# haoningwu3639/StoryGen

Measured on AMD Instinct MI355X. Metric: UNet denoising steps/sec @512x512, 3 prior-frame ctx, bs=1, higher is better.
Workload: dtype f16; 1 GPU; BASELINE configs[1]: StoryGen denoising loop, 512x512 (64x64x4 latent), R=3 prior frames, CFG batch 3, DDIM, SD-1.5 UNet + attn3 (909M params, synthetic fp16 weights); stage=multi-image-condition, samples_per_gpu=1, parallelism=dp1 (one sample per GPU, final all-gather), hipgraph=True, dedup_identical_reference_samples=True, overlap_ref_pass_of_next_step=True, ref_ahead=1, warmup_run=5, split_graphs=False, stream_priority=False, ref_pass_on_cus=0, ref_pass_eager=False, paired_gemm_launches=True, paired_text_image_attention=False, groupnorm_stats_from_epilogues=True, fp16_block_stream=False

## Files before the change

storygen_amd/csrc/gemm_conv.hip:

```cpp
#include "common.h"
#include <stdlib.h>
#include <type_traits>
#include <vector>

namespace {

constexpr int BK = 64;
constexpr int MAX_AUTO_SPLIT = 16;

struct FastDiv { unsigned mul, sh1, sh2; };

__host__ __device__ __forceinline__ unsigned fd_div(unsigned n, FastDiv f) {
#if defined(__HIP_DEVICE_COMPILE__)
    const unsigned t = __umulhi(n, f.mul);
#else
    const unsigned t = (unsigned)(((unsigned long long)n * f.mul) >> 32);
#endif
    return (t + ((n - t) >> f.sh1)) >> f.sh2;
}

FastDiv make_fastdiv(unsigned d) {
    if (d <= 1) return FastDiv{0u, 0u, 0u};
    unsigned l = 0;
    while ((1ull << l) < d) ++l;
    const unsigned long long m = (((1ull << l) - d) << 32) / d + 1;
    return FastDiv{(unsigned)m, 1u, l - 1};
}

struct MmaParams {
    const f16* A; long lda;
    const f16* W; long ldw;
    void* C; long ldc;
    f16* C2; long ldc2;
    int M, N, K, KT;
    int H, Wd, Ho, Wo, cpt , stride, ups, padded;
    int mode, flags;
    const f16* bias;
    const float* rowbias; long rowbias_ld; int rows_per_batch;
    const void* res1; long ldr1;
    const void* res2; long ldr2;
    float* ws; int splits; int kt_per_split; int tiles_m, tiles_n;
    int defer;
    float* stats; int stats_batch_rows;
    const float* ln_stats; int ln_parts; const float* ln_c; const float* ln_d; int ln_mode; float ln_eps;
    float* ln_out;
    unsigned* ln_guard;
    unsigned long long* prof;
    int group_m;
    FastDiv fd_splits, fd_group_w , fd_group_m, fd_hw, fd_wo, fd_rpb, fd_cpt;
};

__device__ __forceinline__ int lds_off(int row, int chunk) { return row * 128 + ((chunk ^ ((row >> 1) & 7)) << 4); }

__host__ __device__ __forceinline__ void tile_of_id(unsigned lid, int tiles_m, int tiles_n, int gm, FastDiv fd_w, FastDiv fd_gm,
                                                    unsigned& tm, unsigned& tn) {
    const unsigned width = (unsigned)gm * (unsigned)tiles_n;
    const unsigned group = fd_div(lid, fd_w), r = lid - group * width;
    const unsigned first = group * (unsigned)gm;
    const unsigned gsize = min((unsigned)tiles_m - first, (unsigned)gm);
    const unsigned q = gsize == (unsigned)gm ? fd_div(r, fd_gm) : r / gsize;
    tn = q;
    tm = first + (r - q * gsize);
}

__device__ __forceinline__ void decode_block(const MmaParams& p, int BM, int BN, int& m0, int& n0, int& z) {
    const unsigned lid2 = (unsigned)xcd_remap(blockIdx.x, p.tiles_m * p.tiles_n * p.splits);
    const unsigned lid = fd_div(lid2, p.fd_splits);
    z = (int)(lid2 - lid * p.splits);
    unsigned tm, tn;
    tile_of_id(lid, p.tiles_m, p.tiles_n, p.group_m, p.fd_group_w, p.fd_group_m, tm, tn);
    m0 = (int)tm * BM;
    n0 = (int)tn * BN;
}

constexpr int EPI_PITCH = 68;
constexpr int EPI_XTR = 64 * EPI_PITCH;
constexpr int EPI_WAVE_BYTES = 64 * EPI_PITCH * 4 + 1024;
constexpr int EPIQ_GROUP_BYTES = 64 * EPI_PITCH * 4 + 4 * 1024;

constexpr int LN_MAX_PARTS = 20;
typedef unsigned u32x2 __attribute__((ext_vector_type(2)));

__device__ __forceinline__ void st_stream(float* p, const f32x4& v) { *reinterpret_cast<f32x4*>(p) = v; }
__device__ __forceinline__ void st_stream(f16* p, const uint2& v) {
    const u32x2 w = {v.x, v.y};
    *reinterpret_cast<u32x2*>(p) = w;
}
__device__ __forceinline__ f32x4 ld_stream(const float* p) { return *reinterpret_cast<const f32x4*>(p); }

__device__ __forceinline__ bool epi_prefetches(const MmaParams& p) {
    return p.res1 != nullptr && (p.flags & SG_F_RES1_F32) && p.splits == 1 && p.mode == SG_EPI_LINEAR;
}

template <int NQ, int NPRE>
__device__ __forceinline__ void epi_prefetch(const MmaParams& p, int rowq, int cq, f32x4 (&pre)[NQ], u32x2& pbias) {
    static_assert(NPRE <= NQ, "prefetched row quads");
    if (p.splits > 1 || p.mode != SG_EPI_LINEAR) return;
    if (p.bias) pbias = *reinterpret_cast<const u32x2*>(p.bias + cq);
    if (NPRE == 0 || !epi_prefetches(p)) return;
    const float* r = reinterpret_cast<const float*>(p.res1) + cq;
    const int mlast = p.M - 1;
#pragma unroll
    for (int k = 0; k < NPRE; ++k) pre[k] = ld_stream(r + (long)min(rowq + 4 * k, mlast) * p.ldr1);
}

template <int NW, int WTM>
constexpr int epi_npre() { return WTM == 1 ? 4 : WTM == 4 ? 0 : NW >= 8 ? 8 : 16; }
template <int NW, int WTM>
constexpr int epi_kb() { return WTM == 1 ? 4 : (WTM == 4 || NW >= 8) ? 8 : 16; }

__device__ __forceinline__ float2 ln_token_coeffs(const MmaParams& p, int token) {
    const int pairs = (p.ln_parts + 1) >> 1;
    const f32x4* s = reinterpret_cast<const f32x4*>(p.ln_stats) + (long)token * pairs;
    f32x4 t[LN_MAX_PARTS / 2];
#pragma unroll
    for (int q = 0; q < LN_MAX_PARTS / 2; ++q) t[q] = s[min(q, pairs - 1)];
    float tot = 0.f;
#pragma unroll
    for (int q = 0; q < LN_MAX_PARTS; ++q) tot += q < p.ln_parts ? ((q & 1) ? t[q >> 1].z : t[q >> 1].x) : 0.f;
    const float n = 64.f * (float)p.ln_parts, mean = tot / n;
    float m2 = 0.f;
#pragma unroll
    for (int q = 0; q < LN_MAX_PARTS; ++q) {
        const float sq = (q & 1) ? t[q >> 1].z : t[q >> 1].x, mq = (q & 1) ? t[q >> 1].w : t[q >> 1].y;
        const float dm = sq * (1.f / 64.f) - mean;
        m2 += q < p.ln_parts ? fmaf(64.f * dm, dm, mq) : 0.f;
    }
    const float r = rsqrtf(m2 / n + p.ln_eps);
    if (p.ln_guard && fabsf(mean * r) > SG_LN_GUARD_RATIO) atomicOr(p.ln_guard, SG_LN_GUARD_OFFSET);
    return make_float2(mean * r, r);
}

union H4 { uint2 u; f16 h[4]; };


__device__ __forceinline__ void store_out4(const MmaParams& p, int gm, int gn, const float (&v)[4]) {
    const bool f32 = p.flags & SG_F_OUT_F32;
    if (f32) st_stream(reinterpret_cast<float*>(p.C) + (long)gm * p.ldc + gn, f32x4{v[0], v[1], v[2], v[3]});
    if (!f32 || p.C2) {
        H4 o;
#pragma unroll
        for (int e = 0; e < 4; ++e) o.h[e] = (f16)(f32 ? __builtin_amdgcn_fmed3f(v[e], -65504.f, 65504.f) : v[e]);
        if (!f32) st_stream(reinterpret_cast<f16*>(p.C) + (long)gm * p.ldc + gn, o.u);
        if (p.C2) st_stream(p.C2 + (long)gm * p.ldc2 + gn, o.u);
    }
}

__device__ __forceinline__ void epi_park_stats(float* xtr, int lr, int lc, float (&cs)[4], float (&cq2)[4]) {
#pragma unroll
    for (int e = 0; e < 4; ++e) {
        cs[e] += __shfl_xor(cs[e], 16, 64); cq2[e] += __shfl_xor(cq2[e], 16, 64);
        cs[e] += __shfl_xor(cs[e], 32, 64); cq2[e] += __shfl_xor(cq2[e], 32, 64);
    }
    if (lr == 0) {
#pragma unroll
        for (int e = 0; e < 4; ++e) {
            xtr[128 + (4 * lc + e) * 2 + 0] = cs[e];
            xtr[128 + (4 * lc + e) * 2 + 1] = cq2[e];
        }
    }
}

__device__ __forceinline__ void ln_out_store(const MmaParams& p, int gm, int blk, float sum, float m2) {
    const int nblk = ((p.N >> 6) + 1) & ~1;
    *reinterpret_cast<float2*>(p.ln_out + ((size_t)gm * nblk + blk) * 2) = make_float2(sum, m2);
    if (p.ln_guard && !(fabsf(sum * (1.f / 64.f)) + sqrtf(m2) < 65504.f)) atomicOr(p.ln_guard, SG_LN_GUARD_RANGE);
}

template <int WGM, int WGN, int WT = 2, int WTM = WT>
__device__ __forceinline__ void epi_finish(const MmaParams& p, char* smem, f32x16 (&acc)[WTM][WT], f32x4 (&pre)[WT == 2 ? 16 : 4], u32x2& pbias,
                                           int m0, int n0, int z, int wave, int wm0, int wn, int lane) {
    constexpr int BN = 32 * WT * WGN, NW = WGM * WGN, NT = 64 * NW, NH = WT == 2 ? WTM / 2 : 1, NQ = WT == 2 ? 16 : 4;
    const int lnm = p.ln_mode;
    const int l31 = lane & 31, hi = lane >> 5, lr = lane >> 4, lc = lane & 15;
    constexpr int GQ = WGN / 2;
    const int gmq = wm0 >> 1, gq = wn >> 1, wi = wm0 & 1, wj = wn & 1, q = wi * 2 + wj;
    char* grp = smem + (gmq * GQ + gq) * EPIQ_GROUP_BYTES;
    const int rbase = m0 + gmq * 64 + q * 16, cbase = n0 + gq * 64;
    float* stg = reinterpret_cast<float*>(WT == 2 ? smem + wave * EPI_WAVE_BYTES : grp);
    float* xtr = WT == 2 ? stg + EPI_XTR : reinterpret_cast<float*>(grp + 64 * EPI_PITCH * 4 + q * 1024);
    const int r0 = WT == 2 ? lr : q * 16 + lr;
    asm volatile("s_waitcnt lgkmcnt(0)" ::: "memory");
    __builtin_amdgcn_s_barrier();
    float cs[4] = {0, 0, 0, 0}, cq2[4] = {0, 0, 0, 0};
    const bool want_stats = p.stats != nullptr;
#pragma unroll
    for (int half = 0; half < NH; ++half) {
    const int wm = wm0 * NH + half;
    int rowq, colq;
    if constexpr (WT == 2) {
#pragma unroll
        for (int i = 0; i < 2; ++i)
#pragma unroll
            for (int j = 0; j < 2; ++j)
#pragma unroll
                for (int g = 0; g < 4; ++g)
                    *reinterpret_cast<float4*>(stg + (i * 32 + l31) * EPI_PITCH + j * 32 + 8 * g + 4 * hi) =
                        make_float4(acc[2 * half + i][j][4 * g], acc[2 * half + i][j][4 * g + 1], acc[2 * half + i][j][4 * g + 2],
                                    acc[2 * half + i][j][4 * g + 3]);
        rowq = m0 + wm * 64 + lr; colq = n0 + wn * 64 + 4 * lc;
        if (lnm) {
            *reinterpret_cast<float2*>(xtr + 2 * lane) =
                ln_token_coeffs(p, lnm == 1 ? min(m0 + wm * 64 + lane, p.M - 1) : min(n0 + wn * 64 + lane, p.N - 1));
            if (lnm == 2) {
                const int rr = min(m0 + wm * 64 + lane, p.M - 1);
                *reinterpret_cast<float2*>(xtr + 128 + 2 * lane) = make_float2(p.ln_c[rr], p.ln_d[rr]);
            }
        }
        if (p.mode == SG_EPI_GEGLU && p.splits == 1) {
            const int gr = lane >> 3, gc = (lane & 7) * 4;
            const int gv = n0 + wn * 64 + gc;
            if (gv >= p.N) continue;
            float bv[4] = {0, 0, 0, 0}, bg[4] = {0, 0, 0, 0};
            if (p.bias) {
                H4 a, b;
                a.u = *reinterpret_cast<const uint2*>(p.bias + gv); b.u = *reinterpret_cast<const uint2*>(p.bias + gv + 32);
#pragma unroll
                for (int e = 0; e < 4; ++e) { bv[e] = (float)a.h[e]; bg[e] = (float)b.h[e]; }
            }
            const int go = (gv >> 6) * 32 + (gv & 31);
            float cv[4] = {0, 0, 0, 0}, cg[4] = {0, 0, 0, 0};
            if (lnm == 1) {
                const f32x4 a = *reinterpret_cast<const f32x4*>(p.ln_c + gv), b = *reinterpret_cast<const f32x4*>(p.ln_c + gv + 32);
                const f32x4 c = *reinterpret_cast<const f32x4*>(p.ln_d + gv), d = *reinterpret_cast<const f32x4*>(p.ln_d + gv + 32);
                cv[0] = a.x; cv[1] = a.y; cv[2] = a.z; cv[3] = a.w; cg[0] = b.x; cg[1] = b.y; cg[2] = b.z; cg[3] = b.w;
                bv[0] += c.x; bv[1] += c.y; bv[2] += c.z; bv[3] += c.w; bg[0] += d.x; bg[1] += d.y; bg[2] += d.z; bg[3] += d.w;
            }
#pragma unroll
            for (int k = 0; k < 8; ++k) {
                const int row = 8 * k + gr, gm = m0 + wm * 64 + row;
                const float4 a = *reinterpret_cast<const float4*>(stg + row * EPI_PITCH + gc);
                const float4 b = *reinterpret_cast<const float4*>(stg + row * EPI_PITCH + 32 + gc);
                float2 mr = make_float2(0.f, 1.f);
                if (lnm == 1) mr = *reinterpret_cast<const float2*>(xtr + 2 * row);
                if (gm >= p.M) continue;
                const float va[4] = {a.x, a.y, a.z, a.w}, ga[4] = {b.x, b.y, b.z, b.w};
                float o[4];
#pragma unroll
                for (int e = 0; e < 4; ++e)
                    o[e] = (fmaf(mr.y, va[e], bv[e]) - mr.x * cv[e]) * gelu_erf_f(fmaf(mr.y, ga[e], bg[e]) - mr.x * cg[e]);
                store_out4(p, gm, go, o);
            }
            continue;
        }
    } else {
#pragma unroll
        for (int g = 0; g < 4; ++g)
            *reinterpret_cast<float4*>(stg + (wi * 32 + l31) * EPI_PITCH + wj * 32 + 8 * g + 4 * hi) =
                make_float4(acc[0][0][4 * g], acc[0][0][4 * g + 1], acc[0][0][4 * g + 2], acc[0][0][4 * g + 3]);
        if (lnm == 1) {
            const float2 c = ln_token_coeffs(p, min(rbase + lc, p.M - 1));
            if (lr == 0) *reinterpret_cast<float2*>(xtr + 2 * lc) = c;
        } else if (lnm == 2) {
            *reinterpret_cast<float2*>(xtr + 2 * lane) = ln_token_coeffs(p, min(cbase + lane, p.N - 1));
            const int rr = min(rbase + lc, p.M - 1);
            if (lr == 0) *reinterpret_cast<float2*>(xtr + 128 + 2 * lc) = make_float2(p.ln_c[rr], p.ln_d[rr]);
        }
        asm volatile("s_waitcnt lgkmcnt(0)" ::: "memory");
        __builtin_amdgcn_s_barrier();
        rowq = rbase + lr; colq = cbase + 4 * lc;
    }
    const bool col_ok = colq < p.N;
    if (p.splits > 1) {
        float* wsz = p.ws + (size_t)z * p.M * p.N + colq;
#pragma unroll
        for (int k = 0; k < NQ; ++k) {
            const int row = 4 * k + r0, gm = rowq + 4 * k;
            const float4 v = *reinterpret_cast<const float4*>(stg + row * EPI_PITCH + 4 * lc);
            if (gm < p.M && col_ok) st_stream(wsz + (size_t)gm * p.N, f32x4{v.x, v.y, v.z, v.w});
        }
        continue;
    }
    const bool r1f32 = p.flags & SG_F_RES1_F32, r2f32 = p.flags & SG_F_RES2_F32;
    const bool res2_same = p.res2 != nullptr && p.res2 == p.res1 && p.ldr2 == p.ldr1 && r1f32 == r2f32;
    const int cq = min(colq, p.N - 4), mlast = p.M - 1;
    float v[NQ][4];
    {
        float bias4[4] = {0, 0, 0, 0};
        if (p.bias) {
            H4 b; b.u = make_uint2(pbias.x, pbias.y);
#pragma unroll
            for (int e = 0; e < 4; ++e) bias4[e] = (float)b.h[e];
        }
        if (lnm == 1) {
            const f32x4 lc4 = *reinterpret_cast<const f32x4*>(p.ln_c + cq), ld4 = *reinterpret_cast<const f32x4*>(p.ln_d + cq);
            const float c4[4] = {lc4.x, lc4.y, lc4.z, lc4.w};
            const float d4[4] = {ld4.x + bias4[0], ld4.y + bias4[1], ld4.z + bias4[2], ld4.w + bias4[3]};
#pragma unroll
            for (int k = 0; k < NQ; ++k) {
                const float4 a = *reinterpret_cast<const float4*>(stg + (4 * k + r0) * EPI_PITCH + 4 * lc);
                const float2 mr = *reinterpret_cast<const float2*>(xtr + 2 * (4 * k + lr));
                const float av[4] = {a.x, a.y, a.z, a.w};
#pragma unroll
                for (int e = 0; e < 4; ++e) v[k][e] = fmaf(mr.y, av[e], d4[e]) - mr.x * c4[e];
            }
        } else if (lnm == 2) {
            float mrx[4], mry[4];
#pragma unroll
            for (int e = 0; e < 4; ++e) { const float2 t = *reinterpret_cast<const float2*>(xtr + 2 * (4 * lc + e)); mrx[e] = t.x; mry[e] = t.y; }
#pragma unroll
            for (int k = 0; k < NQ; ++k) {
                const float4 a = *reinterpret_cast<const float4*>(stg + (4 * k + r0) * EPI_PITCH + 4 * lc);
                const float2 cd = *reinterpret_cast<const float2*>(xtr + 128 + 2 * (4 * k + lr));
                const float av[4] = {a.x, a.y, a.z, a.w};
#pragma unroll
                for (int e = 0; e < 4; ++e) v[k][e] = fmaf(mry[e], av[e], cd.y + bias4[e]) - mrx[e] * cd.x;
            }
        } else {
#pragma unroll
            for (int k = 0; k < NQ; ++k) {
                const float4 a = *reinterpret_cast<const float4*>(stg + (4 * k + r0) * EPI_PITCH + 4 * lc);
                v[k][0] = a.x + bias4[0]; v[k][1] = a.y + bias4[1]; v[k][2] = a.z + bias4[2]; v[k][3] = a.w + bias4[3];
            }
        }
    }
    constexpr int KB = epi_kb<NW, WTM>();
    auto add_f32 = [&](const float* base, long ld) __attribute__((always_inline)) {
#pragma unroll
        for (int kb = 0; kb < NQ; kb += KB) {
            float4 t[KB];
#pragma unroll
            for (int k = 0; k < KB; ++k) t[k] = *reinterpret_cast<const float4*>(base + (long)min(rowq + 4 * (kb + k), mlast) * ld + cq);
#pragma unroll
            for (int k = 0; k < KB; ++k) { v[kb + k][0] += t[k].x; v[kb + k][1] += t[k].y; v[kb + k][2] += t[k].z; v[kb + k][3] += t[k].w; }
        }
    };
    auto add_f16 = [&](const f16* base, long ld) __attribute__((always_inline)) {
        uint2 t[NQ];
#pragma unroll
        for (int k = 0; k < NQ; ++k) t[k] = *reinterpret_cast<const uint2*>(base + (long)min(rowq + 4 * k, mlast) * ld + cq);
#pragma unroll
        for (int k = 0; k < NQ; ++k) {
            H4 h; h.u = t[k];
#pragma unroll
            for (int e = 0; e < 4; ++e) v[k][e] += (float)h.h[e];
        }
    };
    if (p.rowbias) {
#pragma unroll
        for (int kb = 0; kb < NQ; kb += KB) {
            float4 t[KB];
#pragma unroll
            for (int k = 0; k < KB; ++k)
                t[k] = *reinterpret_cast<const float4*>(p.rowbias + (long)fd_div((unsigned)min(rowq + 4 * (kb + k), mlast), p.fd_rpb) * p.rowbias_ld + cq);
#pragma unroll
            for (int k = 0; k < KB; ++k) { v[kb + k][0] += t[k].x; v[kb + k][1] += t[k].y; v[kb + k][2] += t[k].z; v[kb + k][3] += t[k].w; }
        }
    }
    if (p.res1) {
        if (r1f32) {
            const float w = res2_same ? 2.f : 1.f;
            if constexpr (NH > 1) {
                const float* r = reinterpret_cast<const float*>(p.res1) + cq;
#pragma unroll
                for (int kb = 0; kb < NQ; kb += 8) {
                    f32x4 t[8];
#pragma unroll
                    for (int k = 0; k < 8; ++k) t[k] = ld_stream(r + (long)min(rowq + 4 * (kb + k), mlast) * p.ldr1);
#pragma unroll
                    for (int k = 0; k < 8; ++k) {
                        v[kb + k][0] = fmaf(w, t[k].x, v[kb + k][0]); v[kb + k][1] = fmaf(w, t[k].y, v[kb + k][1]);
                        v[kb + k][2] = fmaf(w, t[k].z, v[kb + k][2]); v[kb + k][3] = fmaf(w, t[k].w, v[kb + k][3]);
                    }
                }
            } else {
                if constexpr (epi_npre<NW, WTM>() < NQ) {
                    const float* r = reinterpret_cast<const float*>(p.res1) + cq;
#pragma unroll
                    for (int k = epi_npre<NW, WTM>(); k < NQ; ++k) pre[k] = ld_stream(r + (long)min(rowq + 4 * k, mlast) * p.ldr1);
                }
#pragma unroll
                for (int k = 0; k < NQ; ++k) {
                    v[k][0] = fmaf(w, pre[k].x, v[k][0]); v[k][1] = fmaf(w, pre[k].y, v[k][1]);
                    v[k][2] = fmaf(w, pre[k].z, v[k][2]); v[k][3] = fmaf(w, pre[k].w, v[k][3]);
                }
            }
        } else {
            add_f16(reinterpret_cast<const f16*>(p.res1), p.ldr1);
            if (res2_same) add_f16(reinterpret_cast<const f16*>(p.res1), p.ldr1);
        }
    }
    if (p.res2 && !res2_same) {
        if (r2f32) add_f32(reinterpret_cast<const float*>(p.res2), p.ldr2);
        else add_f16(reinterpret_cast<const f16*>(p.res2), p.ldr2);
    }
#pragma unroll
    for (int k = 0; k < NQ; ++k) {
        const int gm = rowq + 4 * k;
        if (gm < p.M && col_ok) {
            store_out4(p, gm, colq, v[k]);
#pragma unroll
            for (int e = 0; e < 4; ++e) { cs[e] += v[k][e]; cq2[e] = fmaf(v[k][e], v[k][e], cq2[e]); }
        }
    }
    if (p.ln_out) {
        if constexpr (WT == 2) {
#pragma unroll
            for (int k = 0; k < 16; ++k)
                *reinterpret_cast<float4*>(stg + (4 * k + lr) * EPI_PITCH + 4 * lc) = make_float4(v[k][0], v[k][1], v[k][2], v[k][3]);
            float sum = 0.f, m2 = 0.f, mean = 0.f;
            if constexpr (NH > 1) {
#pragma unroll
                for (int pass = 0; pass < 2; ++pass) {
#pragma unroll
                    for (int qb = 0; qb < 16; qb += 8) {
                        float4 rv[8];
#pragma unroll
                        for (int q = 0; q < 8; ++q) rv[q] = *reinterpret_cast<const float4*>(stg + lane * EPI_PITCH + 4 * (qb + q));
#pragma unroll
                        for (int q = 0; q < 8; ++q) {
                            if (pass == 0) {
                                sum += (rv[q].x + rv[q].y) + (rv[q].z + rv[q].w);
                            } else {
                                const float a = rv[q].x - mean, b = rv[q].y - mean, c = rv[q].z - mean, d = rv[q].w - mean;
                                m2 = fmaf(a, a, m2); m2 = fmaf(b, b, m2); m2 = fmaf(c, c, m2); m2 = fmaf(d, d, m2);
                            }
                        }
                    }
                    if (pass == 0) mean = sum * (1.f / 64.f);
                }
            } else {
                float4 rv[16];
#pragma unroll
                for (int q = 0; q < 16; ++q) rv[q] = *reinterpret_cast<const float4*>(stg + lane * EPI_PITCH + 4 * q);
#pragma unroll
                for (int q = 0; q < 16; ++q) sum += (rv[q].x + rv[q].y) + (rv[q].z + rv[q].w);
                mean = sum * (1.f / 64.f);
#pragma unroll
                for (int q = 0; q < 16; ++q) {
                    const float a = rv[q].x - mean, b = rv[q].y - mean, c = rv[q].z - mean, d = rv[q].w - mean;
                    m2 = fmaf(a, a, m2); m2 = fmaf(b, b, m2); m2 = fmaf(c, c, m2); m2 = fmaf(d, d, m2);
                }
            }
            const int gm = m0 + wm * 64 + lane;
            if (gm < p.M && n0 + wn * 64 < p.N) {
                ln_out_store(p, gm, (n0 >> 6) + wn, sum, m2);
            }
        } else {
            float s4[4], m4[4];
#pragma unroll
            for (int k = 0; k < 4; ++k) s4[k] = (v[k][0] + v[k][1]) + (v[k][2] + v[k][3]);
#pragma unroll
            for (int o = 1; o < 16; o <<= 1)
#pragma unroll
                for (int k = 0; k < 4; ++k) s4[k] += __shfl_xor(s4[k], o, 64);
#pragma unroll
            for (int k = 0; k < 4; ++k) {
                const float mean = s4[k] * (1.f / 64.f);
                const float a = v[k][0] - mean, b = v[k][1] - mean, c = v[k][2] - mean, d = v[k][3] - mean;
                m4[k] = fmaf(a, a, fmaf(b, b, fmaf(c, c, d * d)));
            }
#pragma unroll
            for (int o = 1; o < 16; o <<= 1)
#pragma unroll
                for (int k = 0; k < 4; ++k) m4[k] += __shfl_xor(m4[k], o, 64);
            if (lc == 0 && cbase < p.N) {
#pragma unroll
                for (int k = 0; k < 4; ++k)
                    if (rowq + 4 * k < p.M) ln_out_store(p, rowq + 4 * k, (n0 >> 6) + gq, s4[k], m4[k]);
            }
        }
    }
    }
    if (want_stats && (WT == 1 || p.mode == SG_EPI_LINEAR) && p.splits == 1) {
        epi_park_stats(xtr, lr, lc, cs, cq2);
        __syncthreads();
        for (int idx = threadIdx.x; idx < BN * 2; idx += NT) {
            const int plane = idx / BN, col = idx - plane * BN;
            const int gn = n0 + col;
            if (gn < p.N) {
                float s = 0.f;
                if constexpr (WT == 2) {
#pragma unroll
                    for (int w = 0; w < WGM; ++w)
                        s += reinterpret_cast<const float*>(smem + (w * WGN + (col >> 6)) * EPI_WAVE_BYTES)[EPI_XTR + 128 + (col & 63) * 2 + plane];
                } else {
#pragma unroll
                    for (int g = 0; g < WGM / 2; ++g)
#pragma unroll
                        for (int w = 0; w < 4; ++w)
                            s += reinterpret_cast<const float*>(smem + (g * GQ + (col >> 6)) * EPIQ_GROUP_BYTES + 64 * EPI_PITCH * 4 + w * 1024)[128 + (col & 63) * 2 + plane];
                }
                p.stats[((size_t)(m0 / (32 * WTM * WGM)) * 2 + plane) * p.N + gn] = s;
            }
        }
    }
}

template <int BM, int BN, bool CONV>
__global__ __launch_bounds__(256) void mma_kernel(const MmaParams p) {
    constexpr int WM = BM / 2, WN = BN / 2, TM = WM / 32, TN = WN / 32;
    static_assert(TM == 2 && TN == 2, "epi_finish works on 64x64 wave tiles");
    constexpr int A_IT = BM / 32, B_IT = BN / 32;
    constexpr int A_BYTES = BM * 128, B_BYTES = BN * 128, STAGE = A_BYTES + B_BYTES;
    constexpr int EPI_BYTES = 4 * EPI_WAVE_BYTES;
    constexpr int SMEM = (2 * STAGE > EPI_BYTES) ? 2 * STAGE : EPI_BYTES;
    __shared__ __attribute__((aligned(16))) char smem[SMEM];

    const int t = threadIdx.x, lane = t & 63, wave = t >> 6;
    const int wm = wave >> 1, wn = wave & 1, l31 = lane & 31, hi = lane >> 5;
    int m0, n0, z;
    decode_block(p, BM, BN, m0, n0, z);
    const int kt0 = z * p.kt_per_split;
    const int kt1 = min(p.KT, kt0 + p.kt_per_split);

    const int c = t & 7, r0 = t >> 3;
    const f16* a_ptr[A_IT];
    int a_oy[A_IT], a_ox[A_IT];
    bool a_ok[A_IT];
    const int pad = p.padded ? 1 : 0;
    const int wrow = p.Wd + 2 * pad;
#pragma unroll
    for (int i = 0; i < A_IT; ++i) {
        const int gm = m0 + r0 + 32 * i;
        a_ok[i] = gm < p.M;
        if constexpr (CONV) {
            const int hw = p.Ho * p.Wo;
            const int b = gm / hw, rem = gm - b * hw;
            const int oy = rem / p.Wo, ox = rem - oy * p.Wo;
            a_oy[i] = a_ok[i] ? oy * p.stride - 1 : -(1 << 20);
            a_ox[i] = ox * p.stride - 1;
            a_ptr[i] = p.A + (long)b * (p.H + 2 * pad) * wrow * p.lda + c * 8;
        } else {
            a_oy[i] = a_ox[i] = 0;
            a_ptr[i] = p.A + (long)gm * p.lda + c * 8;
        }
    }
    const f16* w_ptr[B_IT];
    bool w_ok[B_IT];
#pragma unroll
    for (int i = 0; i < B_IT; ++i) {
        const int gn = n0 + r0 + 32 * i;
        w_ok[i] = gn < p.N;
        w_ptr[i] = p.W + (long)gn * p.ldw + c * 8;
    }
    const int hin = p.H << p.ups, win = p.Wd << p.ups;

    uint4 areg[A_IT], breg[B_IT];
    auto load_regs = [&](int kt) {
        const bool kok = kt * BK + c * 8 < p.K;
        if constexpr (CONV) {
            const int tap = kt / p.cpt, cc = kt - tap * p.cpt;
            const int ky = tap / 3, kx = tap - ky * 3;
#pragma unroll
            for (int i = 0; i < A_IT; ++i) {
                const int iy = a_oy[i] + ky, ix = a_ox[i] + kx;
                const bool ok = (unsigned)iy < (unsigned)hin && (unsigned)ix < (unsigned)win;
                const long pix = (long)((iy >> p.ups) + pad) * wrow + ((ix >> p.ups) + pad);
                areg[i] = ok ? ldg16(a_ptr[i] + pix * p.lda + cc * BK) : make_uint4(0, 0, 0, 0);
            }
        } else {
#pragma unroll
            for (int i = 0; i < A_IT; ++i)
                areg[i] = (a_ok[i] && kok) ? ldg16(a_ptr[i] + kt * BK) : make_uint4(0, 0, 0, 0);
        }
#pragma unroll
        for (int i = 0; i < B_IT; ++i)
            breg[i] = (w_ok[i] && kok) ? ldg16(w_ptr[i] + kt * BK) : make_uint4(0, 0, 0, 0);
    };
    auto store_lds = [&](int buf) {
        char* sA = smem + buf * STAGE;
        char* sB = sA + A_BYTES;
#pragma unroll
        for (int i = 0; i < A_IT; ++i) *reinterpret_cast<uint4*>(sA + lds_off(r0 + 32 * i, c)) = areg[i];
#pragma unroll
        for (int i = 0; i < B_IT; ++i) *reinterpret_cast<uint4*>(sB + lds_off(r0 + 32 * i, c)) = breg[i];
    };

    f32x16 acc[TM][TN];
#pragma unroll
    for (int i = 0; i < TM; ++i)
#pragma unroll
        for (int j = 0; j < TN; ++j)
#pragma unroll
            for (int r = 0; r < 16; ++r) acc[i][j][r] = 0.f;

    if (kt0 < kt1) {
        load_regs(kt0);
        store_lds(0);
    }
    __syncthreads();
    for (int kt = kt0; kt < kt1; ++kt) {
        const int buf = (kt - kt0) & 1;
        const bool more = kt + 1 < kt1;
        if (more) load_regs(kt + 1);
        const char* sA = smem + buf * STAGE;
        const char* sB = sA + A_BYTES;
#pragma unroll
        for (int ks = 0; ks < 4; ++ks) {
            f16x8 af[TM], bf[TN];
#pragma unroll
            for (int i = 0; i < TM; ++i)
                af[i] = *reinterpret_cast<const f16x8*>(sA + lds_off(wm * WM + i * 32 + l31, ks * 2 + hi));
#pragma unroll
            for (int j = 0; j < TN; ++j)
                bf[j] = *reinterpret_cast<const f16x8*>(sB + lds_off(wn * WN + j * 32 + l31, ks * 2 + hi));
#pragma unroll
            for (int i = 0; i < TM; ++i)
#pragma unroll
                for (int j = 0; j < TN; ++j)
                    acc[i][j] = __builtin_amdgcn_mfma_f32_32x32x16_f16(bf[j], af[i], acc[i][j], 0, 0, 0);
        }
        if (more) store_lds(buf ^ 1);
        __syncthreads();
    }
    f32x4 pre_f[16]; u32x2 pre_bias;
    epi_prefetch<16, 16>(p, m0 + wm * 64 + (lane >> 4), min(n0 + wn * 64 + 4 * (lane & 15), p.N - 4), pre_f, pre_bias);
    __syncthreads();
    epi_finish<2, 2>(p, smem, acc, pre_f, pre_bias, m0, n0, z, wave, wm, wn, lane);
}

struct LdsRef { char* p; unsigned a; };
__device__ __forceinline__ LdsRef operator+(LdsRef r, int d) { return LdsRef{r.p + d, r.a + (unsigned)d}; }
__device__ __forceinline__ LdsRef lds_ref(char* smem) {
    return LdsRef{smem, (unsigned)__builtin_amdgcn_readfirstlane((int)(unsigned long)((__attribute__((address_space(3))) char*)smem))};
}
__device__ __forceinline__ void glds16(const f16* base, unsigned offb, LdsRef dst) {
    __builtin_amdgcn_global_load_lds((const __attribute__((address_space(1))) void*)(reinterpret_cast<const char*>(base) + offb),
                                     (__attribute__((address_space(3))) void*)dst.p, 16, 0, 0);
}

template <int N>
__device__ __forceinline__ void wait_vmcnt() {
    asm volatile("s_waitcnt vmcnt(%0)" ::"n"(N) : "memory");
}

template <int WGM, int WGN, int S, int WT = 2, int WTM = WT>
constexpr int pipe_smem_bytes() {
    constexpr int ring = S * (32 * WTM * WGM + 32 * WT * WGN) * 128;
    constexpr int epi = WT == 2 ? WGM * WGN * EPI_WAVE_BYTES : (WGM / 2) * (WGN / 2) * EPIQ_GROUP_BYTES;
    return ring > epi ? ring : epi;
}

template <int ST, int S, int YS, class F>
__device__ __forceinline__ void slab_seq(F& slab, int it, int nsteady) {
    if constexpr (ST < S) {
        if (it + ST < nsteady) {
            slab(it + ST, std::false_type{}, std::integral_constant<int, YS>{}, std::integral_constant<int, ST>{});
            slab_seq<ST + 1, S, YS>(slab, it, nsteady);
        }
    }
}
template <int Y, int S, class F>
__device__ __forceinline__ void slab_tail(F& slab, int nt) {
    if (nt > Y) slab(nt - 1 - Y, std::integral_constant<bool, Y == 0>{}, std::integral_constant<int, Y>{}, (nt - 1 - Y) % S);
    if constexpr (Y > 0) slab_tail<Y - 1, S>(slab, nt);
}

template <int WGM, int WGN, bool CONV, bool PROF = false, int S = 3, int WT = 2, int WTMX = WT>
__device__ __forceinline__ void mma_pipe_body(const MmaParams& p, char* smem) {
    unsigned long long pf_acc[9] = {0, 0, 0, 0, 0, 0, 0, 0, 0};
    unsigned long long pf_t = 0, pf_entry = 0;
    auto stamp = [&](int slot) __attribute__((always_inline)) {
        if constexpr (PROF) {
            const unsigned long long now = __builtin_readcyclecounter();
            pf_acc[slot] += now - pf_t;
            pf_t = now;
        }
    };
    if constexpr (PROF) pf_entry = pf_t = __builtin_readcyclecounter();
    constexpr int WTM = WTMX, WTN = WT;
    static_assert(WTM == WT || (WT == 2 && WTM == 4), "wave tiles: 32x32, 64x64 or 128x64");
    constexpr int NW = WGM * WGN, WM = 32 * WTM, WN = 32 * WTN, BM = WM * WGM, BN = WN * WGN;
    constexpr int A_IT = BM / (8 * NW), B_IT = BN / (8 * NW), LPT = A_IT + B_IT;
    constexpr int A_BYTES = BM * 128, B_BYTES = BN * 128, STAGE = A_BYTES + B_BYTES;
    constexpr int ISTR = NW * 1024;
    constexpr bool SPREAD = (NW <= 4 || WT == 1) && !PROF, STAGGER = NW == 8 && WT == 2 && !PROF;
    static_assert(S >= 2 && S <= 8, "ring depth");
    static_assert(WT == 2 || (WGM % 2 == 0 && WGN % 2 == 0), "32x32 waves come in 2x2 groups (epi_finish, WT = 1)");
    static_assert((S - 1) * LPT < 64, "vmcnt is a 6-bit counter");
    static_assert(S * STAGE <= 160 * 1024, "the ring must fit the 160 KB of LDS");
    static_assert(S * STAGE <= pipe_smem_bytes<WGM, WGN, S, WT, WTM>(), "the LDS block covers the ring and the epilogue's staging regions");

    const int t = threadIdx.x, lane = t & 63;
    const int wave = __builtin_amdgcn_readfirstlane(t >> 6);
    const int wm = wave / WGN, wn = wave % WGN, l31 = lane & 31, hi = lane >> 5;
    int m0, n0, z;
    decode_block(p, BM, BN, m0, n0, z);
    const int kt0 = z * p.kt_per_split;
    const int nt = min(p.KT, kt0 + p.kt_per_split) - kt0;

    const int srow = wave * 8 + (lane >> 3);
    const int wp = p.Wd + 2;
    unsigned w_off[B_IT];
#pragma unroll
    for (int i = 0; i < B_IT; ++i) {
        const int row = srow + 8 * NW * i;
        const int lc = (lane & 7) ^ ((row >> 1) & 7);
        w_off[i] = 2u * (unsigned)((long)min(n0 + row, p.N - 1) * p.ldw + lc * 8);
    }
    auto w_koff = [&](int kt) __attribute__((always_inline)) -> long {
        if constexpr (CONV) {
            const int cc = (kt * 7282) >> 16, tap = kt - 9 * cc;
            return (long)tap * p.cpt * BK + (long)cc * BK;
        } else {
            return (long)kt * BK;
        }
    };
    const LdsRef lds = lds_ref(smem);
    auto issue_w = [&](long koff, int stage, int sel = -1) __attribute__((always_inline)) {
        const LdsRef sB = lds + (stage * STAGE + A_BYTES + wave * 1024);
        const f16* Wt = p.W + koff;
#pragma unroll
        for (int i = 0; i < B_IT; ++i)
            if (sel < 0 || ((A_IT + i) & 3) == sel) glds16(Wt, w_off[i], sB + i * ISTR);
    };
    if (nt > 0) issue_w(w_koff(kt0), 0);

    unsigned a_off[A_IT];
    unsigned a_par[A_IT];
#pragma unroll
    for (int i = 0; i < A_IT; ++i) {
        const int row = srow + 8 * NW * i;
        const int lc = (lane & 7) ^ ((row >> 1) & 7);
        const int gm = min(m0 + row, p.M - 1);
        if constexpr (CONV) {
            const int hw = p.Ho * p.Wo;
            const int b = (int)fd_div((unsigned)gm, p.fd_hw), rem = gm - b * hw;
            const int oy = (int)fd_div((unsigned)rem, p.fd_wo), ox = rem - oy * p.Wo;
            const long img = (long)b * (p.H + 2) * wp;
            if (!p.ups) {
                a_off[i] = 2u * (unsigned)((img + (long)(oy * p.stride) * wp + ox * p.stride) * p.lda + lc * 8);
                a_par[i] = 0;
            } else {
                a_off[i] = 2u * (unsigned)((img + (long)(((oy - 1) >> 1) + 1) * wp + ((ox - 1) >> 1) + 1) * p.lda + lc * 8);
                a_par[i] = (unsigned)(((oy - 1) & 1) | (((ox - 1) & 1) << 1));
            }
        } else {
            a_off[i] = 2u * (unsigned)((long)gm * p.lda + lc * 8);
            a_par[i] = 0;
        }
    }

    struct ABase { const f16* At; int ky, kx; long wk; };
    auto a_base = [&](int kt) __attribute__((always_inline)) {
        ABase r;
        r.ky = r.kx = 0;
        r.wk = w_koff(kt);
        if constexpr (CONV) {
            const int cc = (kt * 7282) >> 16, tap = kt - 9 * cc;
            const int ky = (tap * 11) >> 5, kx = tap - ky * 3;
            r.ky = ky; r.kx = kx;
            r.At = !p.ups ? p.A + ((long)(ky * wp + kx) * p.lda + cc * BK) : p.A + cc * BK;
        } else {
            r.At = p.A + kt * BK;
        }
        return r;
    };
    auto a_emit = [&](const ABase& ab, int stage, int sel) __attribute__((always_inline)) {
        const LdsRef sA = lds + (stage * STAGE + wave * 1024);
        if constexpr (CONV) {
            if (!p.ups) {
#pragma unroll
                for (int i = 0; i < A_IT; ++i)
                    if (sel < 0 || (i & 3) == sel) glds16(ab.At, a_off[i], sA + i * ISTR);
            } else {
                const unsigned rs = (unsigned)(wp * (int)p.lda), cs = (unsigned)p.lda;
#pragma unroll
                for (int i = 0; i < A_IT; ++i) {
                    if (!(sel < 0 || (i & 3) == sel)) continue;
                    const unsigned dy = ((unsigned)ab.ky + (a_par[i] & 1u)) >> 1, dx = ((unsigned)ab.kx + (a_par[i] >> 1)) >> 1;
                    glds16(ab.At, a_off[i] + 2u * (__umul24(dy, rs) + __umul24(dx, cs)), sA + i * ISTR);
                }
            }
        } else {
#pragma unroll
            for (int i = 0; i < A_IT; ++i)
                if (sel < 0 || (i & 3) == sel) glds16(ab.At, a_off[i], sA + i * ISTR);
        }
    };
    long it_off, it_wk;
    int it_kx = 0, it_ky = 0;
    {
        const ABase b0 = a_base(kt0);
        it_off = b0.At - p.A;
        it_wk = b0.wk;
        if constexpr (CONV) { it_ky = b0.ky; it_kx = b0.kx; }
    }
    const long it_px = CONV && !p.ups ? (long)p.lda : 0;
    const long it_dy = CONV && !p.ups ? (long)(wp - 3) * p.lda : 0;
    const long it_dc = CONV ? (p.ups ? 0 : -3L * wp * p.lda) + BK : 0;
    const long it_wtap = CONV ? (long)p.cpt * BK : BK, it_wdc = CONV ? BK - 9L * p.cpt * BK : 0;
    auto a_next = [&]() __attribute__((always_inline)) {
        ABase r;
        r.At = p.A + it_off; r.ky = it_ky; r.kx = it_kx; r.wk = it_wk;
        it_wk += it_wtap;
        if constexpr (CONV) {
            it_off += it_px;
            if (++it_kx == 3) {
                it_kx = 0; it_off += it_dy;
                if (++it_ky == 3) { it_ky = 0; it_off += it_dc; it_wk += it_wdc; }
            }
        } else {
            it_off += BK;
        }
        return r;
    };
    auto issue_aw = [&](int stage, bool with_w) __attribute__((always_inline)) {
        const ABase ab = a_next();
        a_emit(ab, stage, -1);
        if (with_w) issue_w(ab.wk, stage);
    };
    if (nt > 0) issue_aw(0, false);
#pragma unroll
    for (int st = 1; st < S - 1; ++st)
        if (nt > st) issue_aw(st, true);

    f32x16 acc[WTM][WTN];
#pragma unroll
    for (int i = 0; i < WTM; ++i)
#pragma unroll
        for (int j = 0; j < WTN; ++j)
#pragma unroll
            for (int r = 0; r < 16; ++r) acc[i][j][r] = 0.f;
    constexpr int NQ = WT == 2 ? 16 : 4;
    f32x4 pre_f[NQ]; u32x2 pre_bias;
    auto prefetch = [&]() __attribute__((always_inline)) {
        const int rowq = (WT == 2 ? m0 + wm * WM : m0 + (wm >> 1) * 64 + ((wm & 1) * 2 + (wn & 1)) * 16) + (lane >> 4);
        const int colq = n0 + (WT == 2 ? wn : wn >> 1) * 64 + 4 * (lane & 15);
        epi_prefetch<NQ, epi_npre<NW, WTM>()>(p, rowq, min(colq, p.N - 4), pre_f, pre_bias);
    };

    constexpr int SPB = WT == 2 ? 1 : ((65536 - 8192) / STAGE > 0 ? (65536 - 8192) / STAGE : 1);
    constexpr int NBASE = (S + SPB - 1) / SPB;
    unsigned fa_off[NBASE][4], fb_off[NBASE][4];
#pragma unroll
    for (int st = 0; st < NBASE; ++st)
#pragma unroll
        for (int ks = 0; ks < 4; ++ks) {
            fa_off[st][ks] = (unsigned)(st * SPB * STAGE + lds_off(wm * WM + l31, ks * 2 + hi));
            fb_off[st][ks] = (unsigned)(st * SPB * STAGE + A_BYTES + lds_off(wn * WN + l31, ks * 2 + hi));
            asm volatile("" : "+v"(fa_off[st][ks]), "+v"(fb_off[st][ks]));
        }
    stamp(7);
    auto slab = [&](int it, auto last_tag, auto young_tag, auto stage_c) __attribute__((always_inline)) {
        constexpr bool LAST = decltype(last_tag)::value;
        constexpr int YOUNG = decltype(young_tag)::value;
        const int stage = stage_c;
        wait_vmcnt<YOUNG * LPT>();
        stamp(1);
        __builtin_amdgcn_s_barrier();
        stamp(2);
        const char* sA = smem + stage * STAGE;
        const char* sB = sA + A_BYTES;
        f16x8 af[2][WTM], bf[2][WTN];
        auto load_frags = [&](int buf, int ks) __attribute__((always_inline)) {
            if constexpr (std::is_same<decltype(stage_c), int>::value) {
#pragma unroll
                for (int i = 0; i < WTM; ++i)
                    af[buf][i] = *reinterpret_cast<const f16x8*>(sA + lds_off(wm * WM + i * 32 + l31, ks * 2 + hi));
#pragma unroll
                for (int j = 0; j < WTN; ++j)
                    bf[buf][j] = *reinterpret_cast<const f16x8*>(sB + lds_off(wn * WN + j * 32 + l31, ks * 2 + hi));
            } else {
                constexpr int ST = decltype(stage_c)::value;
#pragma unroll
                for (int i = 0; i < WTM; ++i)
                    af[buf][i] = *reinterpret_cast<const f16x8*>(smem + fa_off[ST / SPB][ks] + (ST % SPB) * STAGE + i * 4096);
#pragma unroll
                for (int j = 0; j < WTN; ++j)
                    bf[buf][j] = *reinterpret_cast<const f16x8*>(smem + fb_off[ST / SPB][ks] + (ST % SPB) * STAGE + j * 4096);
            }
        };
        load_frags(0, 0);
        const bool refill = SPREAD && !LAST && it + S - 1 < nt;
        int rst = stage + S - 1;
        if (rst >= S) rst -= S;
        ABase ab = {nullptr, 0, 0, 0};
        if (refill) ab = a_next();
#pragma unroll
        for (int ks = 0; ks < 4; ++ks) {
            if (ks + 1 < 4) load_frags((ks + 1) & 1, ks + 1);
            if constexpr (SPREAD) {
                if constexpr (!LAST) {
                    if (refill) {
                        a_emit(ab, rst, ks);
                        issue_w(ab.wk, rst, ks);
                    }
                } else if (ks == 1) {
                    prefetch();
                }
            } else if (LAST || !STAGGER ? ks == 1 : ks == (wave < 4 ? 1 : 3)) {
                stamp(4);
                if constexpr (LAST) {
                    prefetch();
                } else if (it + S - 1 < nt) {
                    issue_aw(rst, true);
                }
                stamp(5);
            }
#pragma unroll
            for (int i = 0; i < WTM; ++i)
#pragma unroll
                for (int j = 0; j < WTN; ++j)
                    acc[i][j] = __builtin_amdgcn_mfma_f32_32x32x16_f16(bf[ks & 1][j], af[ks & 1][i], acc[i][j], 0, 0, 0);
            if (ks == 0) stamp(3);
        }
        stamp(6);
        if constexpr (PROF) pf_acc[0] += 1;
    };
    constexpr int TAIL = S > 2 ? S - 2 : 1, YS = S - 2;
    const int nsteady = nt > TAIL ? nt - TAIL : 0;
    for (int it = 0; it < nsteady; it += S) slab_seq<0, S, YS>(slab, it, nsteady);
    slab_tail<TAIL - 1, S>(slab, nt);
    if (nt <= 0) prefetch();
    epi_finish<WGM, WGN, WT, WTM>(p, smem, acc, pre_f, pre_bias, m0, n0, z, wave, wm, wn, lane);
    if constexpr (PROF) {
        asm volatile("s_waitcnt vmcnt(0)" ::: "memory");
        stamp(8);
        if (lane == 0 && p.prof) {
            unsigned long long* dst = p.prof + ((size_t)blockIdx.x * NW + wave) * 10;
#pragma unroll
            for (int k = 0; k < 9; ++k) dst[k] = pf_acc[k];
            dst[9] = pf_t - pf_entry;
        }
    }
}

template <int WGM, int WGN, bool CONV, int S = 3>
__global__ __launch_bounds__(64 * WGM * WGN) void mma_pipe_kernel(const MmaParams p) {
    __shared__ __attribute__((aligned(16))) char smem[pipe_smem_bytes<WGM, WGN, S>()];
    mma_pipe_body<WGM, WGN, CONV, false, S>(p, smem);
}

template <int WGM, int WGN, bool CONV>
__global__ __launch_bounds__(64 * WGM * WGN) void mma_fat_kernel(const MmaParams p) {
    __shared__ __attribute__((aligned(16))) char smem[pipe_smem_bytes<WGM, WGN, 2, 2, 4>()];
    mma_pipe_body<WGM, WGN, CONV, false, 2, 2, 4>(p, smem);
}

template <int WGM, int WGN, bool CONV, int S>
__global__ __launch_bounds__(64 * WGM * WGN) void mma_lat_kernel(const MmaParams p) {
    __shared__ __attribute__((aligned(16))) char smem[pipe_smem_bytes<WGM, WGN, S, 1>()];
    mma_pipe_body<WGM, WGN, CONV, false, S, 1>(p, smem);
}

#ifdef SG_BUILD_EXPERIMENTS
template <int WGM, int WGN, bool CONV>
__global__ __launch_bounds__(64 * WGM * WGN) void mma_pipe_prof_kernel(const MmaParams p) {
    __shared__ __attribute__((aligned(16))) char smem[pipe_smem_bytes<WGM, WGN, 3>()];
    mma_pipe_body<WGM, WGN, CONV, true>(p, smem);
}
#endif

struct MmaPair { MmaParams p0, p1; };

template <int WGM, int WGN>
__global__ __launch_bounds__(64 * WGM * WGN) void mma_pipe_pair_kernel(const MmaPair pp) {
    __shared__ __attribute__((aligned(16))) char smem[pipe_smem_bytes<WGM, WGN, 3>()];
    if (blockIdx.y == 0) {
        if ((int)blockIdx.x < pp.p0.tiles_m * pp.p0.tiles_n * pp.p0.splits) mma_pipe_body<WGM, WGN, false>(pp.p0, smem);
    } else {
        if ((int)blockIdx.x < pp.p1.tiles_m * pp.p1.tiles_n * pp.p1.splits) mma_pipe_body<WGM, WGN, false>(pp.p1, smem);
    }
}

template <int S>
__global__ __launch_bounds__(256) void mma_lat_pair_kernel(const MmaPair pp) {
    __shared__ __attribute__((aligned(16))) char smem[pipe_smem_bytes<2, 2, S, 1>()];
    if (blockIdx.y == 0) {
        if ((int)blockIdx.x < pp.p0.tiles_m * pp.p0.tiles_n * pp.p0.splits) mma_pipe_body<2, 2, false, false, S, 1>(pp.p0, smem);
    } else {
        if ((int)blockIdx.x < pp.p1.tiles_m * pp.p1.tiles_n * pp.p1.splits) mma_pipe_body<2, 2, false, false, S, 1>(pp.p1, smem);
    }
}

__device__ __forceinline__ void add8(float (&v)[8], const uint4& a, const uint4& b, bool f32) {
    if (f32) {
        v[0] += __uint_as_float(a.x); v[1] += __uint_as_float(a.y); v[2] += __uint_as_float(a.z); v[3] += __uint_as_float(a.w);
        v[4] += __uint_as_float(b.x); v[5] += __uint_as_float(b.y); v[6] += __uint_as_float(b.z); v[7] += __uint_as_float(b.w);
    } else {
        H8 h; h.u = a;
#pragma unroll
        for (int e = 0; e < 8; ++e) v[e] += (float)h.h[e];
    }
}

__device__ __forceinline__ void store_out8(const MmaParams& p, int gm, int gn, const float (&v)[8]) {
    const bool f32 = p.flags & SG_F_OUT_F32;
    if (f32) {
        float* o = reinterpret_cast<float*>(p.C) + (long)gm * p.ldc + gn;
        *reinterpret_cast<float4*>(o) = make_float4(v[0], v[1], v[2], v[3]);
        *reinterpret_cast<float4*>(o + 4) = make_float4(v[4], v[5], v[6], v[7]);
    }
    if (!f32 || p.C2) {
        H8 o;
#pragma unroll
        for (int e = 0; e < 8; ++e) o.h[e] = (f16)(f32 ? __builtin_amdgcn_fmed3f(v[e], -65504.f, 65504.f) : v[e]);
        if (!f32) stg16(reinterpret_cast<f16*>(p.C) + (long)gm * p.ldc + gn, o.u);
        if (p.C2) stg16(p.C2 + (long)gm * p.ldc2 + gn, o.u);
    }
}

__device__ __forceinline__ void add_res8(const void* res, long ld, bool f32, int gm, int gn, float (&v)[8]) {
    if (f32) {
        const float* r = reinterpret_cast<const float*>(res) + (long)gm * ld + gn;
        add8(v, ldg16(r), ldg16(r + 4), true);
    } else {
        add8(v, ldg16(reinterpret_cast<const f16*>(res) + (long)gm * ld + gn), make_uint4(0, 0, 0, 0), false);
    }
}

__device__ __forceinline__ void epi_linear8(const MmaParams& p, int gm, int gn, float (&v)[8]) {
    if (p.bias) {
        H8 b; b.u = ldg16(p.bias + gn);
#pragma unroll
        for (int j = 0; j < 8; ++j) v[j] += (float)b.h[j];
    }
    if (p.rowbias) {
        const float* rb = p.rowbias + (long)fd_div((unsigned)gm, p.fd_rpb) * p.rowbias_ld + gn;
        add8(v, ldg16(rb), ldg16(rb + 4), true);
    }
    if (p.res1) add_res8(p.res1, p.ldr1, p.flags & SG_F_RES1_F32, gm, gn, v);
    if (p.res2) add_res8(p.res2, p.ldr2, p.flags & SG_F_RES2_F32, gm, gn, v);
    store_out8(p, gm, gn, v);
    if (p.ln_out) {
        float s = ((v[0] + v[1]) + (v[2] + v[3])) + ((v[4] + v[5]) + (v[6] + v[7]));
        s += __shfl_xor(s, 1, 64); s += __shfl_xor(s, 2, 64); s += __shfl_xor(s, 4, 64);
        const float mean = s * (1.f / 64.f);
        float m2 = 0.f;
#pragma unroll
        for (int j = 0; j < 8; ++j) { const float d = v[j] - mean; m2 = fmaf(d, d, m2); }
        m2 += __shfl_xor(m2, 1, 64); m2 += __shfl_xor(m2, 2, 64); m2 += __shfl_xor(m2, 4, 64);
        if ((gn & 63) == 0) ln_out_store(p, gm, gn >> 6, s, m2);
    }
}

__device__ __forceinline__ void epi_geglu8(const MmaParams& p, int gm, int gv, float (&val)[8], float (&gate)[8]) {
    if (p.bias) {
        H8 bv, bg; bv.u = ldg16(p.bias + gv); bg.u = ldg16(p.bias + gv + 32);
#pragma unroll
        for (int j = 0; j < 8; ++j) { val[j] += (float)bv.h[j]; gate[j] += (float)bg.h[j]; }
    }
    float o[8];
#pragma unroll
    for (int j = 0; j < 8; ++j) o[j] = val[j] * gelu_erf_f(gate[j]);
    store_out8(p, gm, (gv >> 6) * 32 + (gv & 31), o);
}

__global__ __launch_bounds__(256) void splitk_reduce_kernel(const MmaParams p) {
    const size_t MN = (size_t)p.M * p.N;
    if (p.mode == SG_EPI_LINEAR) {
        const int nch = p.N / 8;
        const long total = (long)p.M * nch;
        for (long idx = (long)blockIdx.x * 256 + threadIdx.x; idx < total; idx += (long)gridDim.x * 256) {
            const int gm = (int)(idx / nch), gn = (int)(idx - (long)gm * nch) * 8;
            float v[8] = {0, 0, 0, 0, 0, 0, 0, 0};
            const float* s = p.ws + (size_t)gm * p.N + gn;
            for (int z0 = 0; z0 < p.splits; z0 += 4) {
                float4 a[4], b[4];
#pragma unroll
                for (int u = 0; u < 4; ++u) {
                    a[u] = b[u] = make_float4(0.f, 0.f, 0.f, 0.f);
                    if (z0 + u < p.splits) {
                        a[u] = *reinterpret_cast<const float4*>(s + (z0 + u) * MN);
                        b[u] = *reinterpret_cast<const float4*>(s + (z0 + u) * MN + 4);
                    }
                }
#pragma unroll
                for (int u = 0; u < 4; ++u) {
                    v[0] += a[u].x; v[1] += a[u].y; v[2] += a[u].z; v[3] += a[u].w;
                    v[4] += b[u].x; v[5] += b[u].y; v[6] += b[u].z; v[7] += b[u].w;
                }
            }
            epi_linear8(p, gm, gn, v);
        }
    } else {
        const int och = p.N / 16;
        const long total = (long)p.M * och;
        for (long idx = (long)blockIdx.x * 256 + threadIdx.x; idx < total; idx += (long)gridDim.x * 256) {
            const int gm = (int)(idx / och), j = (int)(idx - (long)gm * och);
            const int gv = (j >> 2) * 64 + (j & 3) * 8;
            float val[8] = {0, 0, 0, 0, 0, 0, 0, 0}, gate[8] = {0, 0, 0, 0, 0, 0, 0, 0};
            const float* s = p.ws + (size_t)gm * p.N + gv;
            for (int z0 = 0; z0 < p.splits; z0 += 2) {
                float4 q[2][4];
#pragma unroll
                for (int u = 0; u < 2; ++u) {
#pragma unroll
                    for (int k = 0; k < 4; ++k) q[u][k] = make_float4(0.f, 0.f, 0.f, 0.f);
                    if (z0 + u < p.splits) {
                        const float* src = s + (z0 + u) * MN;
                        q[u][0] = *reinterpret_cast<const float4*>(src);
                        q[u][1] = *reinterpret_cast<const float4*>(src + 4);
                        q[u][2] = *reinterpret_cast<const float4*>(src + 32);
                        q[u][3] = *reinterpret_cast<const float4*>(src + 36);
                    }
                }
#pragma unroll
                for (int u = 0; u < 2; ++u) {
                    val[0] += q[u][0].x; val[1] += q[u][0].y; val[2] += q[u][0].z; val[3] += q[u][0].w;
                    val[4] += q[u][1].x; val[5] += q[u][1].y; val[6] += q[u][1].z; val[7] += q[u][1].w;
                    gate[0] += q[u][2].x; gate[1] += q[u][2].y; gate[2] += q[u][2].z; gate[3] += q[u][2].w;
                    gate[4] += q[u][3].x; gate[5] += q[u][3].y; gate[6] += q[u][3].z; gate[7] += q[u][3].w;
                }
            }
            epi_geglu8(p, gm, gv, val, gate);
        }
    }
}

template <int RPT>
__global__ __launch_bounds__(256) void splitk_reduce_stats_kernel(const MmaParams p) {
    constexpr int RB = RPT < 4 ? RPT : 4;
    static_assert(RPT % RB == 0, "whole steps");
    __shared__ float s_acc[32][2][64];
    const int t = threadIdx.x, vc = t & 7, tr = t >> 3;
    const int nb = p.N >> 6;
    const int mt = blockIdx.x / nb, nt = blockIdx.x - mt * nb;
    const int gn = nt * 64 + vc * 8, gm0 = mt * (32 * RPT) + tr;
    const size_t MN = (size_t)p.M * p.N;
    const size_t hstep = (size_t)32 * p.N;
    float s1[8], s2[8];
#pragma unroll
    for (int j = 0; j < 8; ++j) s1[j] = s2[j] = 0.f;
#pragma unroll 1
    for (int h0 = 0; h0 < RPT; h0 += RB) {
        float v[RB][8];
#pragma unroll
        for (int h = 0; h < RB; ++h)
#pragma unroll
            for (int j = 0; j < 8; ++j) v[h][j] = 0.f;
        const float* s = p.ws + (size_t)(gm0 + 32 * h0) * p.N + gn;
        for (int z0 = 0; z0 < p.splits; z0 += 2) {
            float4 a[2][RB], b[2][RB];
#pragma unroll
            for (int u = 0; u < 2; ++u)
#pragma unroll
                for (int h = 0; h < RB; ++h) {
                    a[u][h] = b[u][h] = make_float4(0.f, 0.f, 0.f, 0.f);
                    if (z0 + u < p.splits) {
                        const float* src = s + (z0 + u) * MN + h * hstep;
                        a[u][h] = *reinterpret_cast<const float4*>(src);
                        b[u][h] = *reinterpret_cast<const float4*>(src + 4);
                    }
                }
#pragma unroll
            for (int u = 0; u < 2; ++u)
#pragma unroll
                for (int h = 0; h < RB; ++h) {
                    v[h][0] += a[u][h].x; v[h][1] += a[u][h].y; v[h][2] += a[u][h].z; v[h][3] += a[u][h].w;
                    v[h][4] += b[u][h].x; v[h][5] += b[u][h].y; v[h][6] += b[u][h].z; v[h][7] += b[u][h].w;
                }
        }
#pragma unroll
        for (int h = 0; h < RB; ++h) {
            epi_linear8(p, gm0 + 32 * (h0 + h), gn, v[h]);
#pragma unroll
            for (int j = 0; j < 8; ++j) { s1[j] += v[h][j]; s2[j] = fmaf(v[h][j], v[h][j], s2[j]); }
        }
    }
    *reinterpret_cast<float4*>(&s_acc[tr][0][vc * 8]) = make_float4(s1[0], s1[1], s1[2], s1[3]);
    *reinterpret_cast<float4*>(&s_acc[tr][0][vc * 8 + 4]) = make_float4(s1[4], s1[5], s1[6], s1[7]);
    *reinterpret_cast<float4*>(&s_acc[tr][1][vc * 8]) = make_float4(s2[0], s2[1], s2[2], s2[3]);
    *reinterpret_cast<float4*>(&s_acc[tr][1][vc * 8 + 4]) = make_float4(s2[4], s2[5], s2[6], s2[7]);
    __syncthreads();
    if (t < 128) {
        const int plane = t >> 6, ch = t & 63;
        float acc = 0.f;
#pragma unroll 8
        for (int r = 0; r < 32; ++r) acc += s_acc[r][plane][ch];
        p.stats[((size_t)mt * 2 + plane) * p.N + nt * 64 + ch] = acc;
    }
}

int reduce_stats_rows(const MmaParams& p) {
    if (p.mode != SG_EPI_LINEAR || p.N % 64 != 0 || p.stats_batch_rows <= 0 || p.M % p.stats_batch_rows != 0) return 0;
    int best = 0;
    for (int rows = 64; rows <= 256; rows *= 2)
        if (p.stats_batch_rows % rows == 0 && (best == 0 || (long)(p.M / rows) * (p.N / 64) >= 192)) best = rows;
    return best;
}

enum { FAM_GENERIC = 0, FAM_PIPE = 1, FAM_FAT = 2, FAM_LAT = 16 };

struct TileHint { int bm = 0, bn = 0, waves = 0; };
struct PlanRequest {
    int force_split = 0;
    TileHint hint;
    void* ws = nullptr;
    size_t ws_bytes = 0;
    const char* name = "";
    bool in_pair = false;
    bool stats_optional = false;
    unsigned long long* prof = nullptr;
};

struct Plan {
    int bm = 0, bn = 0, splits = 1;
    int family = FAM_GENERIC;
    int threads = 0, grid = 0;
    int stats_rows = 0;
    bool lat() const { return family >= FAM_LAT; }
    int ring() const { return family - FAM_LAT; }
};


Plan choose_plan(int M, int N, int KT, int force_split, int max_ws_split, bool pipe, int hint_bm, int hint_bn) {
    static const int cand_pipe[6][2] = {{256, 128}, {128, 128}, {256, 64}, {128, 64}, {64, 128}, {64, 64}};
    static const int cand_gen[1][2] = {{128, 128}};
    static const int split_opts[] = {1, 2, 3, 4, 5, 6, 8, 10, 12, 16};
    const SgOptions& o = sg_options();
    const int ncand = pipe ? 6 : 1, family = pipe ? FAM_PIPE : FAM_GENERIC;
    const double CUS = 256.0, BW = pipe ? 18.5 : 12.0;
    const int forced = force_split > 0 ? (force_split > KT ? KT : force_split) : 0;
    const int gen_bm = cand_gen[0][0], gen_bn = cand_gen[0][1];
    Plan best{pipe ? 64 : gen_bm, pipe ? 64 : gen_bn, forced ? forced : 1, family};
    double best_cost = 1e300;
    for (int ci = 0; ci < ncand; ++ci) {
        const int bm = pipe ? cand_pipe[ci][0] : cand_gen[ci][0], bn = pipe ? cand_pipe[ci][1] : cand_gen[ci][1];
        if (pipe && o.tile_m && (bm != o.tile_m || bn != o.tile_n)) continue;
        if (pipe && !o.tile_m && hint_bm && (bm != hint_bm || bn != hint_bn)) continue;
        const long tiles = (long)sg_cdiv(M, bm) * sg_cdiv(N, bn);
        const double waves_per_block = pipe ? (bm / 64) * (bn / 64) : 4.0;
        const double mfma_per_slab = pipe ? 512.0 : 512.0 * (bm / 64.0) * (bn / 64.0) / 4.0;
        for (int s : split_opts) {
            if (forced) s = forced;
            else if (s > 1 && (s > max_ws_split || KT / s < 2 || o.no_split)) continue;
            if (s > KT) continue;
            const double blocks = (double)tiles * s;
            const double slabs = sg_cdiv(KT, s);
            const double blocks_per_cu = sg_cdiv((long)blocks, (long)CUS);
            const double t_bw = blocks_per_cu * slabs * (bm + bn) * 128.0 / BW;
            const double waves_per_simd = sg_cdiv((long)(blocks * waves_per_block), (long)(CUS * 4));
            const double t_mfma = waves_per_simd * slabs * mfma_per_slab;
            double cost = (t_bw > t_mfma ? t_bw : t_mfma) + 2500.0 + blocks_per_cu * (bm * bn / 16.0);
            if (s > 1) cost += 5000.0 + (double)M * N * 4.0 * (s + 1) / 1500.0;
            if (cost < best_cost) { best_cost = cost; best = Plan{bm, bn, s, family}; }
            if (forced) break;
        }
    }
    return best;
}

int check_stats(MmaParams& p, Plan& pl, const PlanRequest& rq) {
    pl.stats_rows = 0;
    if (!p.stats) return SG_OK;
    const int rows = p.splits == 1 ? pl.bm : reduce_stats_rows(p);
    const bool ok = p.mode == SG_EPI_LINEAR && rows > 0 && p.stats_batch_rows > 0 && p.stats_batch_rows % rows == 0 &&
                    p.M % p.stats_batch_rows == 0;
    if (ok) { pl.stats_rows = rows; return SG_OK; }
    if (rq.stats_optional) { p.stats = nullptr; return SG_OK; }
    return sg_set_error(SG_EINVAL, "%s: epilogue statistics need the linear epilogue, a %d-row tile that divides the %d rows of an image "
                        "and, under split-K (here %d), N %% 64 == 0: query sg_*_stats_tile_rows first", rq.name, rows, p.stats_batch_rows,
                        p.splits);
}

template <bool CONV>
bool lat_plan(const MmaParams& p, bool pipe, int force_split, int max_ws_split, TileHint hint, bool in_pair, Plan& pl) {
    const SgOptions& o = sg_options();
    if (!pipe || p.mode != SG_EPI_LINEAR || p.prof || hint.waves < 0 || o.tile_m) return false;
    if (hint.waves == 0) {
        const int kind = (in_pair || p.ln_mode == 2) ? 1 : p.ln_mode ? 2 : p.stats ? 4 : p.ln_out ? 16 : 32;
        if (!(o.lat_mask & kind)) return false;
    }
    const bool hinted = hint.bm != 0 || hint.bn != 0 || hint.waves != 0;
    const bool ask_sq = hint.bm == 64 && hint.bn == 64 && hint.waves == 4, ask_wide = hint.bm == 64 && hint.bn == 128 && hint.waves == 8;
    if (hinted && !ask_sq && !ask_wide) return false;
    const long tiles_sq = (long)sg_cdiv(p.M, 64) * sg_cdiv(p.N, 64), tiles_wide = (long)sg_cdiv(p.M, 64) * sg_cdiv(p.N, 128);
    const bool wide = ask_wide || (!hinted && o.lat_wide && p.M <= o.lat_wide_m && p.N >= 256 && p.KT >= 40);
    const bool sq = !wide && (ask_sq || (!hinted && !CONV && tiles_sq <= o.lat_tiles && p.KT >= o.lat_min_kt &&
                                         (p.KT <= o.lat_max_kt || tiles_sq <= 128)));
    if (!wide && !sq) return false;
    const long tiles = wide ? tiles_wide : tiles_sq;
    const int min_slabs = wide ? 8 : 16;
    int sp = 1;
    if (force_split > 0) sp = force_split > p.KT ? p.KT : force_split;
    else if (tiles <= 128 && !o.no_split && (o.lat_mask & 8)) {
        sp = (int)(256 / tiles);
        if (sp > p.KT / min_slabs) sp = p.KT / min_slabs;
        if (sp > max_ws_split) sp = max_ws_split;
        if (sp > MAX_AUTO_SPLIT) sp = MAX_AUTO_SPLIT;
        if (sp < 1) sp = 1;
    }
    pl = Plan{64, wide ? 128 : 64, sp, FAM_LAT + (wide ? 6 : (o.lat_stages == 8 ? 8 : 4))};
    return true;
}

TileHint apply_big_m(TileHint hint, int M, bool pipe) {
    const SgOptions& o = sg_options();
    if (o.big_m > 0 && M >= o.big_m && hint.bm == 0 && hint.bn == 0 && hint.waves == 0 && pipe) { hint.bm = o.big_bm; hint.bn = o.big_bn; }
    return hint;
}

bool asks_fat(TileHint h) { return h.waves == 8 && ((h.bm == 512 && h.bn == 128) || (h.bm == 256 && h.bn == 256)); }
bool asks_lat(TileHint h) { return (h.waves == 4 && h.bm == 64 && h.bn == 64) || (h.waves == 8 && h.bm == 64 && h.bn == 128); }

template <bool CONV>
Plan choose_family(const MmaParams& p, const PlanRequest& rq, TileHint hint, bool pipe, int max_ws_split) {
    const SgOptions& o = sg_options();
    const bool fat_ok = pipe && !p.prof && !o.tile_m && rq.force_split <= 1 && (p.mode == SG_EPI_LINEAR || p.mode == SG_EPI_GEGLU);
    if (asks_fat(hint)) {
        if (fat_ok) return Plan{hint.bm, hint.bn, 1, FAM_FAT};
        hint = TileHint{};
    }
    else if (CONV && fat_ok && o.fat_m > 0 && p.M >= o.fat_m && hint.bm == 0 && hint.bn == 0 && hint.waves == 0) {
        const int rows = p.stats ? p.stats_batch_rows : 512;
        if (rows % 512 == 0) return Plan{512, 128, 1, FAM_FAT};
    }
    Plan pl;
    if (lat_plan<CONV>(p, pipe, rq.force_split, max_ws_split, hint, rq.in_pair, pl)) return pl;
    if (asks_lat(hint)) hint.bm = hint.bn = 0;
    return choose_plan(p.M, p.N, p.KT, rq.force_split, max_ws_split, pipe, hint.bm, hint.bn);
}

template <bool CONV>
int choose_group_m(const MmaParams& p, int splits) {
    const double a_bytes = CONV ? 2.0 * p.M * (p.K / 9) * (p.stride == 1 && !p.ups ? 1.0 : (p.ups ? 0.25 : 4.0)) : 2.0 * p.M * p.K;
    const double w_bytes = 2.0 * p.N * p.K;
    const double a_panel = a_bytes / p.tiles_m, w_panel = w_bytes / p.tiles_n;
    const int wave_tiles = splits >= 32 ? 1 : 32 / splits;
    int best = 1;
    double best_bytes = 1e300;
    const int cands[6] = {1, 2, 4, 8, 16, p.tiles_m};
    for (int c : cands) {
        const int gm = c < p.tiles_m ? c : p.tiles_m;
        const int width = gm * p.tiles_n;
        int rows, cols;
        if (width >= wave_tiles) {
            rows = gm < wave_tiles ? gm : wave_tiles;
            cols = (wave_tiles + rows - 1) / rows;
        } else {
            rows = gm * ((wave_tiles + width - 1) / width);
            if (rows > p.tiles_m) rows = p.tiles_m;
            cols = p.tiles_n;
        }
        const double bytes = rows * a_panel + cols * w_panel;
        if (bytes <= best_bytes) { best_bytes = bytes; best = gm; }
    }
    return sg_options().no_nmajor ? 1 : best;
}

template <bool CONV>
void fill_fastdiv(MmaParams& p) {
    p.fd_splits = make_fastdiv((unsigned)p.splits);
    p.fd_group_w = make_fastdiv((unsigned)(p.group_m * p.tiles_n));
    p.fd_group_m = make_fastdiv((unsigned)p.group_m);
    p.fd_rpb = make_fastdiv((unsigned)(p.rows_per_batch > 0 ? p.rows_per_batch : 1));
    if (CONV) {
        p.fd_hw = make_fastdiv((unsigned)(p.Ho * p.Wo));
        p.fd_wo = make_fastdiv((unsigned)p.Wo);
        p.fd_cpt = make_fastdiv((unsigned)p.cpt);
    }
}

int threads_of(const Plan& pl) {
    return pl.family == FAM_FAT ? 512 : pl.lat() ? 64 * (pl.bm / 32) * (pl.bn / 32) : pl.family == FAM_PIPE ? 64 * (pl.bm / 64) * (pl.bn / 64) : 256;
}

template <bool CONV>
int plan_mma(MmaParams& p, const PlanRequest& rq, Plan& pl) {
    p.KT = sg_cdiv(p.K, BK);
    p.prof = rq.prof;
    const bool pipe = (p.K % BK == 0) && (!CONV || p.padded) && !sg_options().no_pipe;
    const size_t per_split = (size_t)p.M * p.N * 4;
    const int max_ws_split = rq.ws ? (int)(rq.ws_bytes / per_split > 64 ? 64 : rq.ws_bytes / per_split) : 1;
    pl = choose_family<CONV>(p, rq, apply_big_m(rq.hint, p.M, pipe), pipe, max_ws_split);
    if (pl.splits > 1 && (rq.ws == nullptr || rq.ws_bytes < per_split * pl.splits))
        return sg_set_error(SG_EINVAL, "%s: split_k=%d needs %zu workspace bytes, got %zu", rq.name, pl.splits, per_split * pl.splits,
                            rq.ws_bytes);
    p.ws = reinterpret_cast<float*>(rq.ws);
    p.splits = pl.splits;
    p.kt_per_split = sg_cdiv(p.KT, pl.splits);
    p.tiles_m = sg_cdiv(p.M, pl.bm);
    p.tiles_n = sg_cdiv(p.N, pl.bn);
    p.group_m = choose_group_m<CONV>(p, pl.splits);
    fill_fastdiv<CONV>(p);
    pl.threads = threads_of(pl);
    pl.grid = p.tiles_m * p.tiles_n * pl.splits;
    return check_stats(p, pl, rq);
}

template <int WGM, int WGN, bool CONV>
void launch_pipe(const MmaParams& p, dim3 grid, dim3 block, hipStream_t st) {
#ifdef SG_BUILD_EXPERIMENTS
    if (p.prof) {
        hipLaunchKernelGGL((mma_pipe_prof_kernel<WGM, WGN, CONV>), grid, block, 0, st, p);
        return;
    }
#endif
    if constexpr ((WGM == 2 && WGN == 2) || (WGM == 4 && WGN == 1)) {
        if (sg_options().pipe_stages == 2) {
            hipLaunchKernelGGL((mma_pipe_kernel<WGM, WGN, CONV, 2>), grid, block, 0, st, p);
            return;
        }
    }
    hipLaunchKernelGGL((mma_pipe_kernel<WGM, WGN, CONV>), grid, block, 0, st, p);
}

int launch_reduce(const MmaParams& p, hipStream_t st) {
    if (p.splits <= 1) return SG_OK;
    if (p.stats) {
        const int rows = reduce_stats_rows(p);
        const dim3 grid((p.M / rows) * (p.N / 64));
        if (rows == 256) hipLaunchKernelGGL(splitk_reduce_stats_kernel<8>, grid, dim3(256), 0, st, p);
        else if (rows == 128) hipLaunchKernelGGL(splitk_reduce_stats_kernel<4>, grid, dim3(256), 0, st, p);
        else hipLaunchKernelGGL(splitk_reduce_stats_kernel<2>, grid, dim3(256), 0, st, p);
        SG_CHECK_LAUNCH("splitk_reduce_stats");
        return SG_OK;
    }
    const long items = (long)p.M * (p.N / (p.mode == SG_EPI_GEGLU ? 16 : 8));
    const int blocks = (int)min((long)4096, (items + 255) / 256);
    hipLaunchKernelGGL(splitk_reduce_kernel, dim3(blocks), dim3(256), 0, st, p);
    SG_CHECK_LAUNCH("splitk_reduce");
    return SG_OK;
}

template <bool CONV>
int launch_plan(const MmaParams& p, const Plan& pl, hipStream_t st, const char* name) {
    if (p.defer && pl.splits <= 1)
        return sg_set_error(SG_EINVAL, "%s: defer_reduce needs a split-K launch (query sg_conv3x3_planned_splits first)", name);
    const dim3 grid(pl.grid), block(pl.threads);
    if (pl.family == FAM_FAT) {
        if (pl.bm == 512) hipLaunchKernelGGL((mma_fat_kernel<4, 2, CONV>), grid, block, 0, st, p);
        else hipLaunchKernelGGL((mma_fat_kernel<2, 4, CONV>), grid, block, 0, st, p);
    } else if (pl.lat()) {
        if (pl.bn == 128) hipLaunchKernelGGL((mma_lat_kernel<2, 4, CONV, 6>), grid, block, 0, st, p);
        else if (pl.ring() == 8) hipLaunchKernelGGL((mma_lat_kernel<2, 2, CONV, 8>), grid, block, 0, st, p);
        else hipLaunchKernelGGL((mma_lat_kernel<2, 2, CONV, 4>), grid, block, 0, st, p);
    } else if (pl.family == FAM_PIPE) {
        if (pl.bm == 256 && pl.bn == 128) launch_pipe<4, 2, CONV>(p, grid, block, st);
        else if (pl.bm == 128 && pl.bn == 128) launch_pipe<2, 2, CONV>(p, grid, block, st);
        else if (pl.bm == 256 && pl.bn == 64) launch_pipe<4, 1, CONV>(p, grid, block, st);
        else if (pl.bm == 128 && pl.bn == 64) launch_pipe<2, 1, CONV>(p, grid, block, st);
        else if (pl.bm == 64 && pl.bn == 128) launch_pipe<1, 2, CONV>(p, grid, block, st);
        else launch_pipe<1, 1, CONV>(p, grid, block, st);
    } else {
        if (p.ln_mode) return sg_set_error(SG_EINVAL, "%s: a folded LayerNorm needs the LDS-DMA kernel (K %% 64 == 0)", name);
        if (pl.bm == 128 && pl.bn == 128) hipLaunchKernelGGL((mma_kernel<128, 128, CONV>), grid, block, 0, st, p);
        else return sg_set_error(SG_EINVAL, "%s: internal: the register-staged kernel has only the 128x128 tile", name);
    }
    SG_CHECK_LAUNCH(name);
    if (p.defer) return SG_OK;
    return launch_reduce(p, st);
}

void report_plan(const Plan& pl, int32_t* out) {
    out[0] = pl.bm; out[1] = pl.bn; out[2] = pl.splits; out[3] = pl.grid; out[4] = pl.threads; out[5] = pl.family;
}

int check_out_res(const char* who, int flags, const void* C, int64_t ldc, const void* C2, int64_t ldc2, const void* res1,
                  int64_t ldr1, const void* res2, int64_t ldr2, int n_out) {
    SG_REQUIRE((flags & ~(SG_F_OUT_F32 | SG_F_RES1_F32 | SG_F_RES2_F32)) == 0, "%s: unknown flag bits 0x%x", who, flags);
    SG_REQUIRE(sg_aligned16(C) && ldc % 8 == 0 && ldc >= n_out, "%s: output alignment / ld", who);
    SG_REQUIRE(!C2 || (sg_aligned16(C2) && ldc2 % 8 == 0 && ldc2 >= n_out), "%s: second output alignment / ld", who);
    SG_REQUIRE(!res1 || (sg_aligned16(res1) && ldr1 % 8 == 0), "%s: res1 alignment", who);
    SG_REQUIRE(!res2 || (sg_aligned16(res2) && ldr2 % 8 == 0), "%s: res2 alignment", who);
    return SG_OK;
}

int check_tile_hint(const char* who, int bm, int bn, int waves) {
    if ((bm == 64 && bn == 64 && waves == 4) || (bm == 64 && bn == 128 && waves == 8)) return SG_OK;
    if (bm == 0 && bn == 0 && waves == -1) return SG_OK;
    if (waves == 8 && ((bm == 512 && bn == 128) || (bm == 256 && bn == 256))) return SG_OK;
    if (waves != 0 && waves != (bm / 64) * (bn / 64))
        return sg_set_error(SG_EINVAL, "%s: tile_waves=%d is not available for tile %dx%d (64x64 per wave; 64x64 with 4 waves of 32x32)", who, waves, bm, bn);
    if (bm == 0 && bn == 0) return SG_OK;
    static const int ok[6][2] = {{256, 128}, {128, 128}, {256, 64}, {128, 64}, {64, 128}, {64, 64}};
    for (auto& t : ok)
        if (t[0] == bm && t[1] == bn) return SG_OK;
    return sg_set_error(SG_EINVAL, "%s: unsupported tile hint %dx%d", who, bm, bn);
}

}

extern "C" size_t sg_gemm_workspace_bytes(int32_t M, int32_t N, int32_t split_k) {
    const int s = split_k > 0 ? split_k : MAX_AUTO_SPLIT;
    return s > 1 ? (size_t)M * (size_t)N * 4u * (size_t)s : 0;
}

namespace {
int gemm_params(const sg_gemm_desc* d, MmaParams& p, const char* who) {
    SG_REQUIRE(d != nullptr, "%s: null descriptor", who);
    SG_REQUIRE(d->A && d->W && d->C, "%s: null A/W/C", who);
    SG_REQUIRE(d->M > 0 && d->N > 0 && d->K > 0, "%s: bad shape M=%d N=%d K=%d", who, d->M, d->N, d->K);
    SG_REQUIRE(d->K % 8 == 0 && d->N % 8 == 0, "%s: K (%d) and N (%d) must be multiples of 8", who, d->K, d->N);
    SG_REQUIRE(d->lda % 8 == 0 && d->ldw % 8 == 0, "%s: lda/ldw must be multiples of 8", who);
    SG_REQUIRE(d->lda >= d->K && d->ldw >= d->K, "%s: lda/ldw smaller than K", who);
    SG_REQUIRE(sg_aligned16(d->A) && sg_aligned16(d->W), "%s: A/W must be 16-byte aligned", who);
    SG_REQUIRE(d->epilogue == SG_EPI_LINEAR || d->epilogue == SG_EPI_GEGLU, "%s: unknown epilogue %d", who, d->epilogue);
    int n_out = d->N;
    if (d->epilogue == SG_EPI_GEGLU) {
        SG_REQUIRE(d->N % 64 == 0, "%s: GEGLU needs N %% 64 == 0 (got %d)", who, d->N);
        SG_REQUIRE(!d->rowbias && !d->res1 && !d->res2, "%s: GEGLU epilogue takes bias only", who);
        n_out = d->N / 2;
    }
    if (int rc = check_out_res(who, d->flags, d->C, d->ldc, d->C2, d->ldc2, d->res1, d->ldr1, d->res2, d->ldr2, n_out))
        return rc;
    SG_REQUIRE(!d->bias || sg_aligned16(d->bias), "%s: bias must be 16-byte aligned", who);
    SG_REQUIRE(!d->rowbias || (sg_aligned16(d->rowbias) && d->rowbias_ld % 4 == 0 && d->rows_per_batch >= 1),
               "%s: rowbias alignment / rows_per_batch", who);
    SG_REQUIRE(d->split_k >= 0 && d->split_k <= 64, "%s: split_k %d is outside the supported range [0, 64] (0 = auto, 1 = none)", who, d->split_k);
    SG_REQUIRE(!d->workspace || (sg_aligned16(d->workspace)), "%s: workspace alignment", who);
    const long long lim = 1ll << 31;
    const long long a_span = (long long)(d->M - 1) * d->lda + d->K, w_span = (long long)(d->N - 1) * d->ldw + d->K;
    SG_REQUIRE(d->lda <= lim && a_span <= lim,
               "%s: operand A spans %lld elements ((M - 1) * lda + K); the bound is 2^31 elements (4 GiB: 32-bit LDS-DMA byte offsets)", who, a_span);
    SG_REQUIRE(d->ldw <= lim && w_span <= lim,
               "%s: operand W spans %lld elements ((N - 1) * ldw + K); the bound is 2^31 elements (4 GiB: 32-bit LDS-DMA byte offsets)", who, w_span);
    p = MmaParams{};
    p.A = reinterpret_cast<const f16*>(d->A); p.lda = d->lda;
    p.W = reinterpret_cast<const f16*>(d->W); p.ldw = d->ldw;
    p.C = d->C; p.ldc = d->ldc;
    p.C2 = reinterpret_cast<f16*>(d->C2); p.ldc2 = d->ldc2;
    p.M = d->M; p.N = d->N; p.K = d->K;
    p.mode = d->epilogue; p.flags = d->flags;
    p.bias = reinterpret_cast<const f16*>(d->bias);
    p.rowbias = d->rowbias; p.rowbias_ld = d->rowbias_ld; p.rows_per_batch = d->rows_per_batch > 0 ? d->rows_per_batch : 1;
    p.res1 = d->res1; p.ldr1 = d->ldr1;
    p.res2 = d->res2; p.ldr2 = d->ldr2;
    SG_REQUIRE(!d->stats || (sg_aligned16(d->stats) && d->stats_batch_rows > 0), "%s: stats alignment / stats_batch_rows", who);
    p.stats = d->stats; p.stats_batch_rows = d->stats_batch_rows;
    SG_REQUIRE(d->ln_mode >= 0 && d->ln_mode <= 2, "%s: ln_mode must be 0, 1 or 2", who);
    if (d->ln_mode) {
        SG_REQUIRE(d->ln_stats && d->ln_c && d->ln_d, "%s: ln_mode needs ln_stats, ln_c and ln_d", who);
        SG_REQUIRE(d->ln_parts >= 1 && d->ln_parts <= LN_MAX_PARTS && d->K == 64 * d->ln_parts,
                   "%s: ln_parts (%d) must be K / 64 (K = %d) and at most %d", who, d->ln_parts, d->K, LN_MAX_PARTS);
        SG_REQUIRE(sg_aligned16(d->ln_c) && sg_aligned16(d->ln_d) && sg_aligned16(d->ln_stats), "%s: ln_c / ln_d / ln_stats alignment", who);
        SG_REQUIRE(d->split_k <= 1, "%s: a GEMM with a folded LayerNorm does not split K (its epilogue is not linear in the partials)", who);
        SG_REQUIRE(!d->stats && !d->rowbias && !d->res1 && !d->res2, "%s: ln_mode excludes stats, rowbias and residuals", who);
        SG_REQUIRE(d->ln_mode == 1 || d->epilogue == SG_EPI_LINEAR, "%s: ln_mode 2 needs the linear epilogue", who);
        SG_REQUIRE(d->ln_eps > 0.f, "%s: ln_eps must be positive", who);
    }
    if (d->ln_stats_out) {
        SG_REQUIRE(d->epilogue == SG_EPI_LINEAR && d->N % 64 == 0 && sg_aligned16(d->ln_stats_out),
                   "%s: ln_stats_out needs the linear epilogue, N %% 64 == 0 and a 16-byte aligned buffer", who);
    }
    p.ln_stats = d->ln_stats; p.ln_parts = d->ln_parts; p.ln_c = d->ln_c; p.ln_d = d->ln_d; p.ln_mode = d->ln_mode; p.ln_eps = d->ln_eps;
    p.ln_out = d->ln_stats_out;
    SG_REQUIRE(!d->ln_guard || (reinterpret_cast<uintptr_t>(d->ln_guard) & 3u) == 0, "%s: ln_guard must be 4-byte aligned", who);
    p.ln_guard = (d->ln_mode || d->ln_stats_out) ? reinterpret_cast<unsigned*>(d->ln_guard) : nullptr;
    return check_tile_hint(who, d->tile_m, d->tile_n, d->tile_waves);
}

int conv_params(const sg_conv3x3_desc* d, MmaParams& p, const char* who) {
    SG_REQUIRE(d != nullptr, "%s: null descriptor", who);
    SG_REQUIRE(d->x && d->w && d->y, "%s: null x/w/y", who);
    SG_REQUIRE(d->B > 0 && d->H > 0 && d->W > 0 && d->Cin > 0 && d->Cout > 0, "%s: bad shape", who);
    SG_REQUIRE(d->Cin % 64 == 0, "%s: Cin (%d) must be a multiple of 64", who, d->Cin);
    SG_REQUIRE(d->Cout % 8 == 0, "%s: Cout (%d) must be a multiple of 8", who, d->Cout);
    SG_REQUIRE(d->stride == 1 || d->stride == 2, "%s: stride must be 1 or 2", who);
    SG_REQUIRE(d->upsample2x == 0 || (d->upsample2x == 1 && d->stride == 1), "%s: upsample2x needs stride 1", who);
    SG_REQUIRE(d->x_padded == 0 || d->x_padded == 1, "%s: x_padded must be 0 or 1", who);
    SG_REQUIRE(d->ldx % 8 == 0 && d->ldx >= d->Cin, "%s: bad ldx", who);
    SG_REQUIRE(sg_aligned16(d->x) && sg_aligned16(d->w), "%s: x/w must be 16-byte aligned", who);
    if (int rc = check_out_res(who, d->flags, d->y, d->ldy, nullptr, 0, d->res1, d->ldr1, nullptr, 0, d->Cout)) return rc;
    SG_REQUIRE(!d->bias || sg_aligned16(d->bias), "%s: bias alignment", who);
    SG_REQUIRE(!d->rowbias || (sg_aligned16(d->rowbias) && d->rowbias_ld % 4 == 0), "%s: rowbias alignment", who);
    SG_REQUIRE(d->split_k >= 0 && d->split_k <= 64, "%s: split_k %d is outside the supported range [0, 64] (0 = auto, 1 = none)", who, d->split_k);
    SG_REQUIRE(!d->workspace || sg_aligned16(d->workspace), "%s: workspace alignment", who);
    SG_REQUIRE((int64_t)(d->W + 2) * d->ldx < (1 << 24), "%s: input row pitch must be below 2^24 elements", who);
    {
        const long long lim = 1ll << 31;
        const int bord = d->x_padded ? 2 : 0;
        const long long rows = (long long)d->B * (d->H + bord), pixels = rows <= lim ? rows * (d->W + bord) : lim + 1;
        const long long x_span = pixels <= lim ? (pixels - 1) * (long long)d->ldx + d->Cin : lim + 1;
        const long long w_span = (long long)d->Cout * 9 * d->Cin;
        SG_REQUIRE(x_span <= lim,
                   "%s: input x spans %s%lld elements ((pixels - 1) * ldx + Cin%s); the bound is 2^31 elements (4 GiB: 32-bit LDS-DMA byte offsets)",
                   who, pixels <= lim ? "" : "more than ", x_span, d->x_padded ? ", zero border included" : "");
        SG_REQUIRE(w_span <= lim,
                   "%s: weights w span %lld elements (Cout * 9 * Cin); the bound is 2^31 elements (4 GiB: 32-bit LDS-DMA byte offsets)", who, w_span);
    }
    SG_REQUIRE(9 * (d->Cin / 64) < 3000, "%s: Cin (%d) too large for the slab decode (kt / 9 by multiply-shift, kt < 3000)", who, d->Cin);
    const int hin = d->H << d->upsample2x, win = d->W << d->upsample2x;
    const int Ho = (hin + 2 - 3) / d->stride + 1, Wo = (win + 2 - 3) / d->stride + 1;
    p = MmaParams{};
    p.A = reinterpret_cast<const f16*>(d->x); p.lda = d->ldx;
    p.W = reinterpret_cast<const f16*>(d->w); p.ldw = 9L * d->Cin;
    p.C = d->y; p.ldc = d->ldy;
    p.M = d->B * Ho * Wo; p.N = d->Cout; p.K = 9 * d->Cin;
    p.H = d->H; p.Wd = d->W; p.Ho = Ho; p.Wo = Wo; p.cpt = d->Cin / 64; p.stride = d->stride; p.ups = d->upsample2x;
    p.padded = d->x_padded;
    p.mode = SG_EPI_LINEAR; p.flags = d->flags;
    p.bias = reinterpret_cast<const f16*>(d->bias);
    p.rowbias = d->rowbias; p.rowbias_ld = d->rowbias_ld; p.rows_per_batch = Ho * Wo;
    p.res1 = d->res1; p.ldr1 = d->ldr1;
    SG_REQUIRE(!d->stats || sg_aligned16(d->stats), "%s: stats alignment", who);
    p.stats = d->stats; p.stats_batch_rows = Ho * Wo;
    SG_REQUIRE(d->defer_reduce == 0 || (d->defer_reduce == 1 && !d->stats), "%s: defer_reduce is 0 or 1 and excludes stats", who);
    p.defer = d->defer_reduce;
    return check_tile_hint(who, d->tile_m, d->tile_n, d->tile_waves);
}

PlanRequest gemm_request(const sg_gemm_desc* d, const char* name) {
    return PlanRequest{d->ln_mode ? 1 : d->split_k, TileHint{d->tile_m, d->tile_n, d->tile_waves}, d->workspace, d->workspace_bytes, name};
}

int plan_gemm(const sg_gemm_desc* d, MmaParams& p, Plan& pl, bool stats_optional = false, void* prof = nullptr) {
    if (int rc = gemm_params(d, p, "sg_gemm_f16")) return rc;
    PlanRequest rq = gemm_request(d, "sg_gemm_f16");
    rq.stats_optional = stats_optional;
    rq.prof = reinterpret_cast<unsigned long long*>(prof);
    return plan_mma<false>(p, rq, pl);
}

int plan_conv(const sg_conv3x3_desc* d, MmaParams& p, Plan& pl, bool stats_optional = false, void* prof = nullptr) {
    if (int rc = conv_params(d, p, "sg_conv3x3")) return rc;
    PlanRequest rq{d->split_k, TileHint{d->tile_m, d->tile_n, d->tile_waves}, d->workspace, d->workspace_bytes, "sg_conv3x3_nhwc_f16"};
    rq.stats_optional = stats_optional;
    rq.prof = reinterpret_cast<unsigned long long*>(prof);
    return plan_mma<true>(p, rq, pl);
}

int plan_conv_undeferred(const sg_conv3x3_desc* d, Plan& pl) {
    sg_conv3x3_desc q = *d;
    q.defer_reduce = 0;
    MmaParams p;
    return plan_conv(&q, p, pl);
}

struct PairPlan {
    Plan pl0, pl1;
    bool paired = false;
    int grid = 0;
};

int plan_pair(const sg_gemm_desc* d0, const sg_gemm_desc* d1, MmaPair& pp, PairPlan& out) {
    if (int rc = gemm_params(d0, pp.p0, "sg_gemm_pair_f16[0]")) return rc;
    if (int rc = gemm_params(d1, pp.p1, "sg_gemm_pair_f16[1]")) return rc;
    SG_REQUIRE(!(d0->workspace && d1->workspace) ||
               (reinterpret_cast<char*>(d0->workspace) + d0->workspace_bytes <= reinterpret_cast<char*>(d1->workspace) ||
                reinterpret_cast<char*>(d1->workspace) + d1->workspace_bytes <= reinterpret_cast<char*>(d0->workspace)),
               "sg_gemm_pair_f16: the two problems run concurrently and need disjoint workspaces");
    PlanRequest rq0 = gemm_request(d0, "sg_gemm_pair_f16[0]"), rq1 = gemm_request(d1, "sg_gemm_pair_f16[1]");
    rq0.in_pair = rq1.in_pair = true;
    Plan &pl0 = out.pl0, &pl1 = out.pl1;
    if (int rc = plan_mma<false>(pp.p0, rq0, pl0)) return rc;
    PlanRequest on_tile0 = rq1;
    on_tile0.hint = TileHint{pl0.bm, pl0.bn, pl0.lat() ? (pl0.bn == 128 ? 8 : 4) : -1};
    if (int rc = plan_mma<false>(pp.p1, on_tile0, pl1)) return rc;
    out.paired = pl0.family != FAM_GENERIC && pl1.family != FAM_GENERIC && pl1.bm == pl0.bm && pl1.bn == pl0.bn && pl0.lat() == pl1.lat() &&
                 !(pl0.lat() && pl0.bn == 128);
    if (!out.paired) {
        out.grid = 0;
        return plan_mma<false>(pp.p1, rq1, pl1);
    }
    out.grid = (((pl0.grid > pl1.grid ? pl0.grid : pl1.grid) + 7) & ~7) * 2;
    return SG_OK;
}

template <int WGM, int WGN>
void launch_pair(const MmaPair& pp, dim3 grid, dim3 block, hipStream_t st) {
    hipLaunchKernelGGL((mma_pipe_pair_kernel<WGM, WGN>), grid, block, 0, st, pp);
}

int launch_pair_plan(const MmaPair& pp, const PairPlan& pr, hipStream_t st) {
    const Plan& pl0 = pr.pl0;
    const dim3 grid(pr.grid / 2, 2), block(pl0.threads);
    if (pl0.lat()) {
        if (pl0.ring() == 8) hipLaunchKernelGGL(mma_lat_pair_kernel<8>, grid, block, 0, st, pp);
        else hipLaunchKernelGGL(mma_lat_pair_kernel<4>, grid, block, 0, st, pp);
    }
    else if (pl0.bm == 256 && pl0.bn == 128) launch_pair<4, 2>(pp, grid, block, st);
    else if (pl0.bm == 128 && pl0.bn == 128) launch_pair<2, 2>(pp, grid, block, st);
    else if (pl0.bm == 256 && pl0.bn == 64) launch_pair<4, 1>(pp, grid, block, st);
    else if (pl0.bm == 128 && pl0.bn == 64) launch_pair<2, 1>(pp, grid, block, st);
    else if (pl0.bm == 64 && pl0.bn == 128) launch_pair<1, 2>(pp, grid, block, st);
    else launch_pair<1, 1>(pp, grid, block, st);
    SG_CHECK_LAUNCH("sg_gemm_pair_f16");
    if (int rc = launch_reduce(pp.p0, st)) return rc;
    return launch_reduce(pp.p1, st);
}
}

extern "C" int sg_gemm_f16(const sg_gemm_desc* d, sg_stream_t stream) {
    MmaParams p;
    Plan pl;
    if (int rc = plan_gemm(d, p, pl)) return rc;
    return launch_plan<false>(p, pl, (hipStream_t)stream, "sg_gemm_f16");
}

extern "C" int sg_gemm_pair_f16(const sg_gemm_desc* d0, const sg_gemm_desc* d1, sg_stream_t stream) {
    MmaPair pp;
    PairPlan pr;
    if (int rc = plan_pair(d0, d1, pp, pr)) return rc;
    hipStream_t st = (hipStream_t)stream;
    if (pr.paired) return launch_pair_plan(pp, pr, st);
    if (int rc = launch_plan<false>(pp.p0, pr.pl0, st, "sg_gemm_pair_f16[0]")) return rc;
    return launch_plan<false>(pp.p1, pr.pl1, st, "sg_gemm_pair_f16[1]");
}

extern "C" int sg_conv3x3_nhwc_f16(const sg_conv3x3_desc* d, sg_stream_t stream) {
    MmaParams p;
    Plan pl;
    if (int rc = plan_conv(d, p, pl)) return rc;
    return launch_plan<true>(p, pl, (hipStream_t)stream, "sg_conv3x3_nhwc_f16");
}

extern "C" int sg_gemm_stats_tile_rows(const sg_gemm_desc* d) {
    SG_REQUIRE(d && d->stats, "sg_gemm_stats_tile_rows: descriptor with a stats buffer required");
    MmaParams p;
    Plan pl;
    const int rc = plan_gemm(d, p, pl, true);
    return rc ? rc : pl.stats_rows;
}

extern "C" int sg_conv3x3_stats_tile_rows(const sg_conv3x3_desc* d) {
    SG_REQUIRE(d && d->stats, "sg_conv3x3_stats_tile_rows: descriptor with a stats buffer required");
    MmaParams p;
    Plan pl;
    const int rc = plan_conv(d, p, pl, true);
    return rc ? rc : pl.stats_rows;
}

extern "C" int sg_conv3x3_planned_splits(const sg_conv3x3_desc* d) {
    SG_REQUIRE(d != nullptr, "sg_conv3x3_planned_splits: null descriptor");
    Plan pl;
    const int rc = plan_conv_undeferred(d, pl);
    return rc ? rc : pl.splits;
}

extern "C" int sg_gemm_launch_plan(const sg_gemm_desc* d, int32_t* out) {
    SG_REQUIRE(d && out, "sg_gemm_launch_plan: null argument");
    MmaParams p;
    Plan pl;
    if (int rc = plan_gemm(d, p, pl)) return rc;
    report_plan(pl, out);
    return SG_OK;
}

extern "C" int sg_conv3x3_launch_plan(const sg_conv3x3_desc* d, int32_t* out) {
    SG_REQUIRE(d && out, "sg_conv3x3_launch_plan: null argument");
    Plan pl;
    if (int rc = plan_conv_undeferred(d, pl)) return rc;
    report_plan(pl, out);
    return SG_OK;
}

extern "C" int sg_gemm_pair_launch_plan(const sg_gemm_desc* d0, const sg_gemm_desc* d1, int32_t* out) {
    SG_REQUIRE(out, "sg_gemm_pair_launch_plan: null argument");
    MmaPair pp;
// ... 115 lines not shown
```

storygen_amd/engine.py:

```python
from __future__ import annotations

import math
from typing import Dict, List, NamedTuple, Optional

import torch

from . import ops
from .arch import BlockSpec, ResnetSpec, UNetArch, XfSpec, feature_shapes
from .repack import conv1x1_nk, conv3x3_krsc, conv_in_kn, ff_fused_pack, fold_layernorm, interleave_geglu

F16 = torch.float16
GN_EPILOGUE_STATS = True
FP16_BLOCK_STREAM = False
FP16_RESNET_STREAM = False
PAIR_GEMMS = True
LN_FOLD = True
ATTN_PAIR = False
SPLITK_IN_GN = True
FF_FUSED = True
FF_SPLIT_MAX_TOKENS = 16384
FF_PROJ_MERGE = True
LN_EPS = 1e-5


def _pair(first, second):
    if PAIR_GEMMS:
        ops.gemm_pair(first, second)
    else:
        for args, kw in (first, second):
            ops.gemm(*args, **{**kw, "tile": (0, 0, -1)})


class _Resnet:
    __slots__ = ("spec", "n1g", "n1b", "w1", "n2g", "n2b", "w2", "b2", "wsc", "bsc", "temb_off")


class _Xf:
    __slots__ = ("spec", "ng", "nb", "w_in", "b_in", "w_out", "b_out", "ln", "w_qk1", "w_v1", "w_o1", "b_o1", "w_q2", "w_k2",
                 "w_v2", "w_o2", "b_o2", "w_q3", "w_k3", "w_v3", "w_o3", "b_o3", "w_o23", "b_o23", "w_ff1", "b_ff1", "w_ff2", "b_ff2",
                 "w_qk1f", "c_qk1", "d_qk1", "w_v1f", "c_v1", "d_v1", "w_q2f", "c_q2", "d_q2", "w_q3f", "c_q3", "d_q3",
                 "w_ff1f", "c_ff1", "d_ff1",
                 "ff_pack",
                 "w_out2",
                 "w_ffo", "b_ffo")


class EngineWeights:

    def __init__(self, arch: UNetArch, state_dict: Dict[str, torch.Tensor], device):
        self.arch, self.dev, self.cfg = arch, torch.device(device), arch.config
        self.version = 0
        self._load_weights(state_dict)

    def _w(self, sd, key) -> torch.Tensor:
        return sd[key].detach().to(device=self.dev, dtype=F16).contiguous()

    def _load_weights(self, sd):
        dev, arch = self.dev, self.arch
        g = lambda k: self._w(sd, k)
        self.w_conv_in = conv_in_kn(g("conv_in.weight"))
        self.b_conv_in = g("conv_in.bias")
        self.w_t1, self.b_t1 = g("time_embedding.linear_1.weight"), g("time_embedding.linear_1.bias")
        self.w_t2, self.b_t2 = g("time_embedding.linear_2.weight"), g("time_embedding.linear_2.bias")
        half = cfg_half = self.cfg["block_out_channels"][0] // 2
        self.freqs = torch.exp(-math.log(10000.0) * torch.arange(half, dtype=torch.float32)
                               / (cfg_half - self.cfg["freq_shift"])).to(dev)
        self.resnets: Dict[str, _Resnet] = {}
        temb_w, temb_b, off = [], [], 0
        for r in arch.resnets:
            p = r.prefix
            o = _Resnet()
            o.spec = r
            o.n1g, o.n1b = g(f"{p}.norm1.weight"), g(f"{p}.norm1.bias")
            o.w1 = conv3x3_krsc(g(f"{p}.conv1.weight"))
            o.n2g, o.n2b = g(f"{p}.norm2.weight"), g(f"{p}.norm2.bias")
            o.w2, o.b2 = conv3x3_krsc(g(f"{p}.conv2.weight")), g(f"{p}.conv2.bias")
            if r.has_shortcut:
                o.wsc, o.bsc = conv1x1_nk(g(f"{p}.conv_shortcut.weight")), g(f"{p}.conv_shortcut.bias")
            else:
                o.wsc = o.bsc = None
            temb_w.append(g(f"{p}.time_emb_proj.weight"))
            temb_b.append((sd[f"{p}.time_emb_proj.bias"].float() + sd[f"{p}.conv1.bias"].float()).to(dev, F16))
            o.temb_off = off
            off += r.cout
            self.resnets[p] = o
        self.w_temb = torch.cat(temb_w, 0).contiguous()
        self.b_temb = torch.cat(temb_b, 0).contiguous()
        self.temb_total = off
        self.xfs: Dict[str, _Xf] = {}
        for blk in arch.blocks:
            for a in blk.attns:
                if a is None:
                    continue
                p, t = a.prefix, f"{a.prefix}.transformer_blocks.0"
                o = _Xf()
                o.spec = a
                o.ng, o.nb = g(f"{p}.norm.weight"), g(f"{p}.norm.bias")
                o.w_in, o.b_in = conv1x1_nk(g(f"{p}.proj_in.weight")), g(f"{p}.proj_in.bias")
                o.w_out, o.b_out = conv1x1_nk(g(f"{p}.proj_out.weight")), g(f"{p}.proj_out.bias")
                o.ln = {n: (g(f"{t}.{n}.weight"), g(f"{t}.{n}.bias")) for n in ("norm1", "norm2", "norm3", "norm4")}
                o.w_qk1 = torch.cat([g(f"{t}.attn1.to_q.weight"), g(f"{t}.attn1.to_k.weight")], 0).contiguous()
                o.w_v1 = g(f"{t}.attn1.to_v.weight")
                o.w_o1, o.b_o1 = g(f"{t}.attn1.to_out.0.weight"), g(f"{t}.attn1.to_out.0.bias")
                o.w_q2 = g(f"{t}.attn2.to_q.weight")
                o.w_k2, o.w_v2 = g(f"{t}.attn2.to_k.weight"), g(f"{t}.attn2.to_v.weight")
                o.w_o2, o.b_o2 = g(f"{t}.attn2.to_out.0.weight"), g(f"{t}.attn2.to_out.0.bias")
                o.w_q3 = g(f"{t}.attn3.to_q.weight")
                o.w_k3, o.w_v3 = g(f"{t}.attn3.to_k.weight"), g(f"{t}.attn3.to_v.weight")
                o.w_o3, o.b_o3 = g(f"{t}.attn3.to_out.0.weight"), g(f"{t}.attn3.to_out.0.bias")
                o.w_o23 = torch.cat([o.w_o2, o.w_o3], dim=1).contiguous()
                o.b_o23 = (sd[f"{t}.attn2.to_out.0.bias"].float() + sd[f"{t}.attn3.to_out.0.bias"].float()).to(dev, F16)
                o.w_ff1, o.b_ff1 = interleave_geglu(g(f"{t}.ff.net.0.proj.weight"), g(f"{t}.ff.net.0.proj.bias"))
                o.w_ff2, o.b_ff2 = g(f"{t}.ff.net.2.weight"), g(f"{t}.ff.net.2.bias")
                for name, val in self._pack_folds(o).items():
                    setattr(o, name, val)
                o.ff_pack = ff_fused_pack(o.w_ff1f, o.d_ff1, o.w_ff2) if (ops.ff_fused_supported(a.channels) and dev.type == "cuda") else None
                o.w_out2 = torch.cat([o.w_out, o.w_out], dim=1).contiguous() if o.ff_pack is not None else None
                if o.ff_pack is None:
                    wo32 = o.w_out.float()
                    o.w_ffo = torch.cat([(wo32 @ o.w_ff2.float()).to(F16), o.w_out], dim=1).contiguous()
                    o.b_ffo = (wo32 @ o.b_ff2.float() + o.b_out.float()).to(F16).contiguous()
                else:
                    o.w_ffo = o.b_ffo = None
                self.xfs[p] = o
        self.samplers = {}
        for blk in arch.down + arch.up:
            if blk.sampler_prefix:
                self.samplers[blk.sampler_prefix] = (conv3x3_krsc(g(f"{blk.sampler_prefix}.weight")),
                                                     g(f"{blk.sampler_prefix}.bias"))
        self.gn_out = (g("conv_norm_out.weight"), g("conv_norm_out.bias"))
        self.w_conv_out = conv3x3_krsc(g("conv_out.weight"))
        self.b_conv_out = g("conv_out.bias")

    @staticmethod
    def _pack_folds(xf: "_Xf", which=("qk1", "v1", "q2", "q3", "ff1")) -> Dict[str, torch.Tensor]:
        src = {"qk1": (xf.w_qk1, None, "norm1"), "v1": (xf.w_v1, None, "norm1"), "q2": (xf.w_q2, None, "norm2"),
               "q3": (xf.w_q3, None, "norm4"), "ff1": (xf.w_ff1, xf.b_ff1, "norm3")}
        out = {}
        for k in which:
            w, b, n = src[k]
            wf, c, d = fold_layernorm(w, b, *xf.ln[n])
            out[f"w_{k}f"], out[f"c_{k}"], out[f"d_{k}"] = wf.contiguous(), c.contiguous(), d.contiguous()
        return out

    def _pack_attn3(self, sd, xf: "_Xf") -> Dict[str, torch.Tensor]:
        t = f"{xf.spec.prefix}.transformer_blocks.0"
        g = lambda k: self._w(sd, k)
        w_o3 = g(f"{t}.attn3.to_out.0.weight")
        return {"w_q3": g(f"{t}.attn3.to_q.weight"), "w_k3": g(f"{t}.attn3.to_k.weight"), "w_v3": g(f"{t}.attn3.to_v.weight"),
                "w_o3": w_o3, "b_o3": g(f"{t}.attn3.to_out.0.bias"), "w_o23": torch.cat([xf.w_o2, w_o3], dim=1),
                "b_o23": (sd[f"{t}.attn2.to_out.0.bias"].float() + sd[f"{t}.attn3.to_out.0.bias"].float()).to(self.dev, F16)}

    def refresh_attn3_(self, sd, prefixes=None):
        for p, xf in self.xfs.items():
            if prefixes is None or p in prefixes:
                for name, val in self._pack_attn3(sd, xf).items():
                    getattr(xf, name).copy_(val)
                for name, val in self._pack_folds(xf, ("q3",)).items():
                    getattr(xf, name).copy_(val)

    def _pack_attn1(self, sd, xf: "_Xf") -> Dict[str, torch.Tensor]:
        t = f"{xf.spec.prefix}.transformer_blocks.0"
        g = lambda k: self._w(sd, k)
        return {"w_qk1": torch.cat([g(f"{t}.attn1.to_q.weight"), g(f"{t}.attn1.to_k.weight")], 0), "w_v1": g(f"{t}.attn1.to_v.weight"),
                "w_o1": g(f"{t}.attn1.to_out.0.weight"), "b_o1": g(f"{t}.attn1.to_out.0.bias")}

    def refresh_attn1_(self, sd, prefixes=None):
        for p, xf in self.xfs.items():
            if prefixes is None or p in prefixes:
                for name, val in self._pack_attn1(sd, xf).items():
                    getattr(xf, name).copy_(val)
                for name, val in self._pack_folds(xf, ("qk1", "v1")).items():
                    getattr(xf, name).copy_(val)

    def reload_(self, sd):
        fresh = EngineWeights.__new__(EngineWeights)
        fresh.arch, fresh.dev, fresh.cfg = self.arch, self.dev, self.cfg
        fresh._load_weights(sd)

        def walk(old, new):
            if torch.is_tensor(old):
                old.copy_(new)
            elif isinstance(old, dict):
                for k in old:
                    walk(old[k], new[k])
            elif isinstance(old, (tuple, list)):
                for a, b in zip(old, new):
                    walk(a, b)
            elif isinstance(old, (_Resnet, _Xf)):
                for k in old.__slots__:
                    if k != "spec" and getattr(old, k, None) is not None:
                        walk(getattr(old, k), getattr(new, k))
        for k, v in self.__dict__.items():
            if k not in ("arch", "dev", "cfg", "version"):
                walk(v, getattr(fresh, k))
        self.version += 1


class HarvestPlan:

    def __init__(self, ctx: Dict[str, torch.Tensor], ops_: List[tuple], kv: Optional[Dict[str, tuple]] = None,
                 src_offset: int = 0, short: int = 0, slots_per_row: Optional[int] = None, direct: bool = False,
                 identity: bool = False):
        self.ctx, self.ops, self.kv, self.src_offset = ctx, list(ops_), kv, int(src_offset)
        self.short, self.slots_per_row, self.direct = int(short), slots_per_row, bool(direct) or bool(identity)
        self.identity = bool(identity)
        if self.identity and (self.ops or self.src_offset):
            raise ValueError("an identity harvest plan has no copy ops and no source offset")

    def flat_slot(self, row: int, slot: int, R: int) -> int:
        return row if row < self.short else self.short + (row - self.short) * R + slot

    def is_direct(self, n_samples: int, R: int) -> bool:
        if self.identity:
            return all(c.dim() == 2 and c.shape[0] % n_samples == 0 for c in self.ctx.values())
        if not self.direct or self.src_offset:
            return False
        seen = {}
        for src, step, row, slot, cnt in self.ops:
            for j in range(cnt):
                seen[self.flat_slot(row, slot + j, R)] = src + j * step
        return seen == {u: u for u in range(n_samples)}


class _GnFeed(NamedTuple):
    pstats: Optional[list] = None
    split: Optional[dict] = None

    @staticmethod
    def concat(h: "_GnFeed", skip: "_GnFeed", channels: int) -> "_GnFeed":
        if h.pstats and skip.pstats and h.pstats[0][2] + skip.pstats[0][2] == channels:
            return _GnFeed(pstats=h.pstats + skip.pstats)
        return _NO_FEED


_NO_FEED = _GnFeed()


class _XfPass:

    def __init__(self, eng: "UNetEngine", xf: _Xf, x: torch.Tensor, x_gn: _GnFeed, out: Optional[torch.Tensor], lvl: int, consume: bool):
        L = self.L = eng.lv[lvl]
        self.xf, self.x, self.x_gn, self.out, self.lvl, self.consume, self.guard = xf, x, x_gn, out, lvl, consume, eng.ln_guard
        self.B, self.hw, self.M, self.C, self.heads = eng.B, eng.hw[lvl], x.shape[0], xf.spec.channels, xf.spec.heads
        self.scale = xf.spec.dim_head ** -0.5
        self.fold = LN_FOLD and self.C % 64 == 0 and self.C // 64 <= 20
        self.ff1 = FF_FUSED and xf.ff_pack is not None and L["h3"].dtype != F16
        self.merge = FF_PROJ_MERGE and self.fold and not self.ff1 and xf.w_ffo is not None and L["h3"].dtype != F16 and out is not None
        self.h0r, self.h1r = self.raw(L["h0"], L["ln"]), self.raw(L["h1"], L["ln4"])
        self.h3raw = L["ffo"][:self.M, 4 * self.C:5 * self.C] if self.merge else L["ln"]

    @staticmethod
    def raw(t: torch.Tensor, buf: torch.Tensor) -> torch.Tensor:
        return t if t.dtype == F16 else buf

    def prod(self, t: torch.Tensor, buf: torch.Tensor, st: torch.Tensor) -> dict:
        return dict(out2=None if t.dtype == F16 else buf, ln_out=st, guard=self.guard) if self.fold else {}

    def prod3(self, h3: torch.Tensor) -> dict:
        return {} if self.ff1 else self.prod(h3, self.h3raw, self.L["lnst3"])


class UNetEngine:
    def __init__(self, arch: UNetArch, state_dict: Optional[Dict[str, torch.Tensor]], device, batch: int, height: int,
                 width: int, n_ref: int = 0, seq_len: int = 77, splitk_workspace_mb: int = 96,
                 weights: Optional[EngineWeights] = None, ctx_rows: Optional[int] = None,
                 attn3_groups: Optional[List[tuple]] = None, fp8_attention: bool = False, ctx_short: int = 0,
                 cfg_shared_head: bool = False, fp16_stream: Optional[tuple] = None):
        self.arch, self.dev = arch, torch.device(device)
        self.B, self.H, self.W, self.R, self.S = batch, height, width, n_ref, seq_len
        cfg = arch.config
        self.cfg = cfg
        nlev = len(cfg["block_out_channels"])
        if height % (1 << (nlev - 1)) or width % (1 << (nlev - 1)):
            raise ValueError(f"latent size {height}x{width} must be divisible by {1 << (nlev - 1)}")
        self.groups, self.eps = cfg["norm_num_groups"], cfg["norm_eps"]
        self.cad = cfg["cross_attention_dim"]
        self.hw = [(height >> l) * (width >> l) for l in range(nlev)]
        self.Sp = (seq_len + 7) & ~7
        for k, lv in arch.feature_level.items():
            if self.hw[lv] % 8:
                raise ValueError(f"latent {height}x{width} leaves {self.hw[lv]} tokens at attention block {k}; the V^T layout "
# ... 261 lines not shown
        plans = () if harvest is None else (tuple(harvest) if isinstance(harvest, (list, tuple)) else (harvest,))
        self._xf_entry(st)
        self._self_projections(st, st.L["h0"], st.h0r, st.L["qk"], st.L["vt"])
        self._xf_harvest(st, plans, self._xf_self_attention(st, plans))

    def _xf_back(self, st: _XfPass, text_cache: bool, shared: bool = False) -> _GnFeed:
        h3 = self._xf_cross_consume(st, text_cache, shared) if st.consume else self._xf_cross_text(st, text_cache)
        return self._xf_feed_forward(st, h3)

    def _xf_entry(self, st: _XfPass):
        L, xf, x = st.L, st.xf, st.x
        ops.groupnorm(x.unflatten(0, (st.B, st.hw)), xf.ng, xf.nb, L["gn"].unflatten(0, (st.B, st.hw)), self.groups, 1e-6, False,
                      self.ws_gn, pstats=st.x_gn.pstats, split=st.x_gn.split)
        ops.gemm(L["gn"], xf.w_in, L["h0"], bias=xf.b_in, workspace=self.ws_split, **st.prod(L["h0"], L["ln"], L["lnst0"]))

    def _self_projections(self, st: _XfPass, h0: torch.Tensor, h0r: torch.Tensor, qk: torch.Tensor, vt: torch.Tensor):
        xf, L = st.xf, st.L
        if st.fold:
            _pair(((h0r, xf.w_qk1f, qk), dict(ln=(1, L["lnst0"], xf.c_qk1, xf.d_qk1, LN_EPS), guard=st.guard)),
                  ((xf.w_v1f, h0r, vt), dict(ln=(2, L["lnst0"], xf.c_v1, xf.d_v1, LN_EPS), guard=st.guard)))
        else:
            ops.layernorm(h0, *xf.ln["norm1"], L["ln"])
            _pair(((L["ln"], xf.w_qk1, qk), dict(workspace=self.ws_split)), ((xf.w_v1, L["ln"], vt), dict(workspace=self.ws_pair)))

    def _xf_self_attention(self, st: _XfPass, plans: tuple) -> Optional[torch.Tensor]:
        xf, L, B, hw, C = st.xf, st.L, st.B, st.hw, st.C
        qk3 = L["qk"].view(B, hw, 2 * C)
        self._attention(qk3[:, :, :C], qk3[:, :, C:], L["vt"].view(C, B, hw).permute(1, 0, 2), L["att"].view(B, hw, C), st.heads, st.scale)
        direct = None
        if len(plans) == 1 and plans[0].is_direct(B, plans[0].slots_per_row or self.R):
            c = plans[0].ctx[xf.spec.feature_key]
            direct = c if c.dim() == 2 else c.view(-1, C)
            assert direct.shape[0] == st.M, (direct.shape, st.M)
        kw1 = st.prod(L["h1"], L["ln4"], L["lnst1"])
        if direct is not None:
            kw1["out2"] = st.h1r = direct
        ops.gemm(L["att"], xf.w_o1, L["h1"], bias=xf.b_o1, res1=L["h0"], workspace=self.ws_split, **kw1)
        return direct

    def _xf_harvest(self, st: _XfPass, plans: tuple, direct: Optional[torch.Tensor]):
        xf, hw, C = st.xf, st.hw, st.C
        h1b = st.L["h1"].view(st.B, hw, C)
        for plan in plans:
            ctx = plan.ctx[xf.spec.feature_key]
            c2d = ctx if ctx.dim() == 2 else ctx.view(-1, C)
            if direct is None:
                Rp = plan.slots_per_row or (ctx.shape[1] // hw)
                for src, step, row, slot, cnt in plan.ops:
                    t0 = plan.flat_slot(row, slot, Rp) * hw
                    dst = c2d[t0:t0 + cnt * hw].view(cnt, hw, C)
                    ops.copy_rows(dst, h1b[plan.src_offset + src:].as_strided((cnt, hw, C), (step * hw * C, C, 1)))
            if plan.kv is not None:
                ki, vti = plan.kv[xf.spec.feature_key]
                _pair(((c2d, xf.w_k3, ki), dict(workspace=self.ws_split)), ((xf.w_v3, c2d, vti), dict(workspace=self.ws_pair)))

    def _xf_queries(self, st: _XfPass):
        xf, L, h1, h1r, gd, ws = st.xf, st.L, st.L["h1"], st.h1r, st.guard, self.ws_split
        if st.consume and st.fold:
            _pair(((h1r, xf.w_q2f, L["q2"]), dict(ln=(1, L["lnst1"], xf.c_q2, xf.d_q2, LN_EPS), guard=gd)),
                  ((h1r, xf.w_q3f, L["q"]), dict(ln=(1, L["lnst1"], xf.c_q3, xf.d_q3, LN_EPS), guard=gd)))
        elif st.consume:
            ops.layernorm(h1, *xf.ln["norm2"], L["ln"], 1e-5, *xf.ln["norm4"], L["ln4"])
            _pair(((L["ln"], xf.w_q2, L["q2"]), dict(workspace=ws)), ((L["ln4"], xf.w_q3, L["q"]), dict(workspace=self.ws_pair)))
        elif st.fold:
            ops.gemm(h1r, xf.w_q2f, L["q"], ln=(1, L["lnst1"], xf.c_q2, xf.d_q2, LN_EPS), guard=gd)
        else:
            ops.layernorm(h1, *xf.ln["norm2"], L["ln"])
            ops.gemm(L["ln"], xf.w_q2, L["q"], workspace=ws)

    def _ctx_kv(self, st: _XfPass):
        xf, L, hw, C = st.xf, st.L, st.hw, st.C
        if self.kv_ext is not None:
            ki, vti = self.kv_ext[xf.spec.feature_key]
        else:
            ctx = self.ctx[xf.spec.feature_key]
            c2d = ctx if ctx.dim() == 2 else ctx.view(-1, C)
            ki, vti = L["ki"], L["vti"]
            _pair(((c2d, xf.w_k3, ki), dict(workspace=self.ws_split)), ((xf.w_v3, c2d, vti), dict(workspace=self.ws_pair)))
        ns, rows, nk = self.ctx_short, self.ctx_rows, self.R * hw
        short = (ki[: ns * hw].view(ns, hw, C), vti[:, : ns * hw].unflatten(1, (ns, hw)).permute(1, 0, 2)) if ns else None
        return ki[ns * hw:].view(rows - ns, nk, C), vti[:, ns * hw:].unflatten(1, (rows - ns, nk)).permute(1, 0, 2), short

    def _xf_cross_consume(self, st: _XfPass, text_cache: bool, shared: bool) -> torch.Tensor:
        xf, L, B, hw, C, heads, scale, S = st.xf, st.L, st.B, st.hw, st.C, st.heads, st.scale, self.S
        kt3, vtt3 = self._text_kv(xf, st.lvl, text_cache)
        att23, h1, h3 = L["att23"], L["h1"], L["h3"]
        a2v, a3v = att23[:, :C].unflatten(0, (B, hw)), att23[:, C:].unflatten(0, (B, hw))
        if shared:
            q2q = L["q2"][:hw].view(1, hw, C).expand(2, hw, C)
            q3 = L["q"][:hw].view(1, hw, C).expand(2, hw, C)
            kt3, vtt3, a2o, a3o = kt3[::2], vtt3[::2], a2v[::2], a3v[:2]
        else:
            q2q, q3, a2o, a3o = L["q2"].view(B, hw, C), L["q"].view(B, hw, C), a2v, a3v
        paired = (ATTN_PAIR and self.attn3_share is not None and not self.ctx_short and not shared
                  and not (self.fp8_attention and C == heads * 40))
        forked = False if paired else self._fork()
        if forked:
            with torch.cuda.stream(self.side):
                ops.attention(q2q, kt3, vtt3, a2o, heads, scale, nk=S)
        elif not paired:
            ops.attention(q2q, kt3, vtt3, a2o, heads, scale, nk=S)
        ki3, vti3, short = self._ctx_kv(st)
        if paired:
            ops.attention_pair((q3, ki3, vti3, a3v, None), (q2q, kt3, vtt3, a2v, S), heads, scale)
        elif self.attn3_share is not None:
            self._attention(q3, ki3, vti3, a3o, heads, scale, short=short)
        else:
            for q0, n, c0 in self.attn3_groups:
                self._attention(q3[q0:q0 + n], ki3[c0:c0 + n], vti3[c0:c0 + n], a3v[q0:q0 + n], heads, scale)
        if forked:
            self._join()
        if shared:
            ops.copy_rows(a2v[1:2], a2v[0:1])
            ops.copy_rows(a3v[2:3], a3v[1:2])
        ops.gemm(att23, xf.w_o23, h3, bias=xf.b_o23, res1=h1, res2=h1, workspace=self.ws_split, **st.prod3(h3))
        return h3

    def _xf_cross_text(self, st: _XfPass, text_cache: bool) -> torch.Tensor:
        xf, L, B, hw, C = st.xf, st.L, st.B, st.hw, st.C
        kt3, vtt3 = self._text_kv(xf, st.lvl, text_cache)
        ops.attention(L["q"].view(B, hw, C), kt3, vtt3, L["att"].view(B, hw, C), st.heads, st.scale, nk=self.S)
        h3 = L["h2"]
        ops.gemm(L["att"], xf.w_o2, h3, bias=xf.b_o2, res1=L["h1"], workspace=self.ws_split, **st.prod3(h3))
        return h3

    def _xf_feed_forward(self, st: _XfPass, h3: torch.Tensor) -> _GnFeed:
        xf, L, M, C, gd, ws, x, out = st.xf, st.L, st.M, st.C, st.guard, self.ws_split, st.x, st.out
        h4, w_out = L["h4"], xf.w_out
        if st.ff1 and M <= FF_SPLIT_MAX_TOKENS:
            h4, w_out = L["att23"], xf.w_out2
            ops.ff_fused(h3, xf.ff_pack, xf.b_ff2, h4, LN_EPS, split=True)
        elif st.ff1:
            ops.ff_fused(h3, xf.ff_pack, xf.b_ff2, L["h4"], LN_EPS)
        elif st.merge:
            ops.gemm(st.h3raw, xf.w_ff1f, L["ffo"][:M, :4 * C], epilogue=ops.EPI_GEGLU, ln=(1, L["lnst3"], xf.c_ff1, xf.d_ff1, LN_EPS), guard=gd)
            h4, w_out = L["ffo"][:M], xf.w_ffo
        elif st.fold:
            ops.gemm(st.raw(h3, L["ln"]), xf.w_ff1f, L["ffi"], epilogue=ops.EPI_GEGLU, ln=(1, L["lnst3"], xf.c_ff1, xf.d_ff1, LN_EPS), guard=gd)
        else:
            ops.layernorm(h3, *xf.ln["norm3"], L["ln"])
            ops.gemm(L["ln"], xf.w_ff1, L["ffi"], bias=xf.b_ff1, epilogue=ops.EPI_GEGLU, workspace=ws)
        if not st.ff1 and not st.merge:
            ops.gemm(L["ffi"], xf.w_ff2, L["h4"], bias=xf.b_ff2, res1=h3, workspace=ws)
        kwo = dict(bias=xf.b_ffo if st.merge else xf.b_out, res1=x, workspace=ws)
        return self._produce(xf.spec.prefix + ".proj_out", st.lvl, C,
                             lambda s: ops.gemm(h4, w_out, out, stats=None if s is None else (s, st.hw), **kwo),
                             lambda buf: ops.gemm_stats_rows(h4, w_out, out, stats=(buf, st.hw), **kwo))

    def _sampler_conv(self, prefix: str, h: torch.Tensor, out: torch.Tensor, lvl: int, out_lvl: int, down: bool) -> _GnFeed:
        w, b = self.samplers[prefix]
        pbuf = self.padded[(lvl, h.shape[1])]
        ops.pad_cast(self._img(h, lvl), pbuf)
        kw = dict(stride=2 if down else 1, upsample2x=not down, bias=b, workspace=self.ws_split, x_padded=True)
        return self._produce(prefix, out_lvl, out.shape[1], lambda s: ops.conv3x3(pbuf, w, self._img(out, out_lvl), stats=s, **kw),
                             lambda buf: ops.conv3x3_stats_rows(pbuf, w, self._img(out, out_lvl), stats=buf, **kw))

    def forward(self, harvest_slot: Optional[int] = None, consume: bool = False, harvest: Optional[HarvestPlan] = None,
                harvest_only: bool = False, text_cache: bool = False,
                side: Optional[torch.cuda.Stream] = None) -> Optional[torch.Tensor]:
        if harvest_slot is not None:
            if harvest is not None or self.ctx_rows != self.B:
                raise ValueError("harvest_slot needs one context row per sample and no explicit plan")
            if not self.R:
                raise ValueError("engine was built without context buffers (n_ref=0)")
            if self.ctx_short:
                raise ValueError("harvest_slot: this engine's context rows have different slot counts (ctx_short); pass a HarvestPlan")
            harvest = HarvestPlan(self.ctx, [(b, 0, b, harvest_slot, 1) for b in range(self.B)])
        if harvest is not None and consume:
            raise ValueError("a pass either harvests features or consumes them")
        if consume and not self.R:
            raise ValueError("engine was built without context buffers (n_ref=0)")
        if harvest_only and harvest is None:
            raise ValueError("harvest_only needs a harvest plan")
        self.side = side
        arch, text, skips = self.arch, self.text_in, self.skips
        steps = list(zip(arch.schedule, arch.schedule[1:] + [None]))
        last_xf = [s.xf for s in arch.schedule if s.xf is not None][-1].prefix if harvest_only else None
        tk = dict(text_cache=text_cache)
        skip_gn: List[_GnFeed] = [_NO_FEED]
        if self.time_table is not None and self.time_table_on:
            ops.lookup_rows(self.t_in, self.time_table[0], self.time_table[1], self.tproj)
        else:
            self._time_chain(self.t_in, self.temb0, self.temb1, self.temb2, self.tproj)
        shared = self.cfg_shared_head and consume
        if shared and not self._head_checked and not torch.cuda.is_current_stream_capturing():
            self._head_checked = True
            if not (torch.equal(self.x_in[0], self.x_in[1]) and torch.equal(self.x_in[0], self.x_in[2])
                    and bool((self.t_in == self.t_in[0]).all()) and torch.equal(self.text_in[0], self.text_in[1])):
                raise ValueError("cfg_shared_head: the three samples must be the same latent at the same timestep with text rows "
                                 "[uncond, uncond, text] (the CFG main pass of one story frame, pipeline.py:448-453)")
        if shared:
            blk0 = arch.down[0]
            r0, xf0 = self.resnets[blk0.resnets[0].prefix], self.xfs[blk0.attns[0].prefix]
            ops.conv_in(self.x_in, self.w_conv_in, self.b_conv_in, self._img(skips[0], 0))
            saved = self._enter_head(1)
            try:
                sk0 = skips[0][: self.hw[0]]
                r_gn = self._resnet(r0, sk0, _NO_FEED, self.lv[0]["r"], 0, defer_out=True)
                st = _XfPass(self, xf0, self.lv[0]["r"], r_gn, None, 0, True)
                self._xf_to_harvest(st, None)
                self._xf_queries(st)
            finally:
                self._leave_head(saved)
            for t2d in (self.lv[0]["r"], self.lv[0]["h1"]):
                self._spread(t2d, 1, 2)
            h_gn = self._xf_back(_XfPass(self, xf0, self.lv[0]["r"], r_gn, skips[1], 0, True), text_cache, shared=True)
            skip_gn.append(h_gn)
            h, steps = skips[1], steps[1:]
        else:
            ops.conv_in(self.x_in, self.w_conv_in, self.b_conv_in, self._img(skips[0], 0))
            h, h_gn = skips[0], _NO_FEED
        for s, nxt in steps:
            lvl, L = s.level, self.lv[s.level]
            if s.push is not None:
                out = skips[s.push]
            elif nxt is not None and nxt.pop is not None:
                out = self.up_cats[-1 - nxt.pop][:, : nxt.resnet.cin - nxt.skip]
            else:
                out = L["t_out"]
            if s.resnet is None:
                h_gn = self._sampler_conv(s.sampler, h, out, lvl, s.out_level, down=s.out_level > lvl)
            else:
                rn = self.resnets[s.resnet.prefix]
                if s.pop is not None:
                    h, h_gn = self.up_cats[-1 - s.pop], _GnFeed.concat(h_gn, skip_gn[s.pop], s.resnet.cin)
                if s.xf is None:
                    h_gn = self._resnet(rn, h, h_gn, out, lvl)
                else:
                    r_gn = self._resnet(rn, h, h_gn, L["r"], lvl, defer_out=True)
                    if s.xf.prefix == last_xf:
                        self._xf_to_harvest(_XfPass(self, self.xfs[s.xf.prefix], L["r"], r_gn, None, lvl, consume), harvest)
                        return None
                    h_gn = self._transformer(self.xfs[s.xf.prefix], L["r"], r_gn, out, lvl, text, harvest, consume, **tk)
            if s.push is not None:
                skip_gn.append(h_gn)
            h = out
        L = self.lv[0]
        ops.groupnorm(h.unflatten(0, (self.B, self.hw[0])), *self.gn_out, L["gn"].unflatten(0, (self.B, self.hw[0])),
                      self.groups, self.eps, True, self.ws_gn, pstats=h_gn.pstats)
        ops.conv_out(self._img(L["gn"], 0), self.w_conv_out, self.b_conv_out, self.eps_out)
        return self.eps_out

    def check_ln_guard(self, clear: bool = True) -> int:
        flags = int(self.ln_guard.item())
        if clear and flags:
            self.ln_guard.zero_()
        if flags:
            why = []
            if flags & ops.LN_GUARD_RANGE:
                why.append("a stream tensor reached |x| >= 65504 (its fp16 copy was saturated)")
            if flags & ops.LN_GUARD_OFFSET:
                why.append(f"a token had |mean| / sigma > {ops.LN_GUARD_RATIO:g} (fp16 rounding of the raw copy no longer negligible)")
            raise FloatingPointError("LayerNorm fold outside its range: " + "; ".join(why) + " — rerun with storygen_amd.engine.LN_FOLD = False")
        return flags

    def _time_chain(self, t, e0, e1, e2, out):
        ops.timestep_embed(t, self.freqs, e0, self.cfg["flip_sin_to_cos"])
        ops.linear_rows(e0, self.w_t1, self.b_t1, e1, act_out=True)
        ops.linear_rows(e1, self.w_t2, self.b_t2, e2, act_out=True)
        ops.linear_rows(e2, self.w_temb, self.b_temb, out)

    def build_time_table(self, timesteps, capacity: int = 256) -> bool:
        self.time_table_on = True
        if timesteps is None:
            had = self.time_table is not None
            self.time_table = None
            self._time_keys = None
            return had
        keys = sorted({float(t) for t in timesteps})
        if not keys:
            raise ValueError("build_time_table: no timesteps")
        tag = (keys, getattr(self.wts, "version", 0))
        if self.time_table is not None and getattr(self, "_time_keys", None) == tag:
            return False
        F32, dev, T = torch.float32, self.dev, len(keys)
        fresh = self.time_table is None or self.time_table[0].numel() < T
        if fresh:
            cap = max(int(capacity), T)
            self.time_table = (torch.empty(cap, dtype=F32, device=dev), torch.empty(cap, self.temb_total, dtype=F32, device=dev))
        tk, tab = self.time_table
        tk.fill_(float("nan"))
        tk[:T].copy_(torch.tensor(keys, dtype=F32))
        e0 = torch.empty(4, self.temb0.shape[1], dtype=F32, device=dev)
        e1, e2 = (torch.empty(4, self.arch.temb_dim, dtype=F32, device=dev) for _ in range(2))
        for i in range(0, T, 4):
            n = min(4, T - i)
            self._time_chain(tk[i:i + n], e0[:n], e1[:n], e2[:n], tab[i:i + n])
        self._time_keys = tag
        return fresh

    def set_inputs(self, sample: torch.Tensor, timestep, text: torch.Tensor):
        self.x_in.copy_(sample.to(self.dev, torch.float32))
        self.time_table_on = False
        t = timestep if torch.is_tensor(timestep) else torch.tensor([float(timestep)])
        self.t_in.copy_(t.to(self.dev, torch.float32).reshape(-1).expand(self.B))
        self.text_in.copy_(text.to(self.dev, F16))

    def features(self, slot: int = 0) -> Dict[str, torch.Tensor]:
        if self.ctx_short:
            raise ValueError("features(): this engine's context rows have different slot counts (ctx_short)")
        out = {}
        for k, (n, _) in feature_shapes(self.arch, self.H, self.W).items():
            out[k] = self.ctx[k][:, slot * n:(slot + 1) * n, :]
        return out
```

storygen_amd/ops.py:

```python
from __future__ import annotations

import ctypes as C
from typing import Optional

import torch

from . import _lib
from ._lib import AttnDesc, AttnPairPlan, AttnPlan, ConvDesc, FfDesc, GemmDesc, GnPlan, GroupNormDesc, check

lib = _lib.load()

EPI_LINEAR = 0
EPI_GEGLU = 1
F_OUT_F32, F_RES1_F32, F_RES2_F32 = 1, 2, 4

TILE_TABLE = {}
TUNE_SINK = None


def _apply_tile(d, tile, split_k, sig, mn):
    if tile is not None:
        d.tile_m, d.tile_n = tile[0], tile[1]
        if len(tile) > 2:
            d.tile_waves = tile[2]
    elif split_k == 0 and sig in TILE_TABLE:
        e = TILE_TABLE[sig]
        d.tile_m, d.tile_n = e[0], e[1]
        d.split_k = e[2] if e[2] <= 1 or d.workspace_bytes >= e[2] * mn * 4 else 0
        if len(e) > 3:
            d.tile_waves = e[3]


def load_tile_table(path: Optional[str] = None) -> int:
    import json
    import os
    path = path or os.path.join(os.path.dirname(os.path.abspath(__file__)), "tuning", "mi355x_tiles.json")
    TILE_TABLE.clear()
    if os.path.exists(path) and path != "none":
        with open(path) as f:
            TILE_TABLE.update({k: tuple(v) for k, v in json.load(f)["tiles"].items()})
    return len(TILE_TABLE)


PROFILE_SINK = None
LN_GUARD_RANGE, LN_GUARD_OFFSET, LN_GUARD_RATIO = 1, 2, 16.0
PLAN_SINK = None
AUX_SINK = None


class _timed:
    __slots__ = ("family", "flops", "start", "shape", "aux")

    def __init__(self, family: str, flops: float, shape: str = "", aux: bool = False):
        self.family, self.flops, self.shape, self.aux = family, flops, shape, aux

    def __enter__(self):
        if (AUX_SINK if self.aux else PROFILE_SINK) is not None:
            self.start = torch.cuda.Event(enable_timing=True)
            self.start.record(torch.cuda.current_stream())
        return self

    def __exit__(self, *exc):
        sink = AUX_SINK if self.aux else PROFILE_SINK
        if sink is not None and exc[0] is None:
            end = torch.cuda.Event(enable_timing=True)
            end.record(torch.cuda.current_stream())
            sink.append((self.family, self.flops, self.start, end, self.shape))
        return False


load_tile_table()


def _stream() -> int:
    return torch.cuda.current_stream().cuda_stream


def _p(t: Optional[torch.Tensor]):
    return None if t is None else t.data_ptr()


def _f16(t: torch.Tensor, name: str):
    if t.dtype != torch.float16 or not t.is_cuda:
        raise TypeError(f"{name}: expected a CUDA/HIP float16 tensor, got {t.dtype} on {t.device}")


def _act(t: torch.Tensor, name: str) -> bool:
    if t.dtype not in (torch.float16, torch.float32) or not t.is_cuda:
        raise TypeError(f"{name}: expected a CUDA/HIP float16/float32 tensor, got {t.dtype} on {t.device}")
    return t.dtype == torch.float32


def _f32(t: torch.Tensor, name: str):
    if t.dtype != torch.float32 or not t.is_cuda:
        raise TypeError(f"{name}: expected a CUDA/HIP float32 tensor, got {t.dtype} on {t.device}")


def _row_stride(t: torch.Tensor, name: str) -> int:
    if t.stride(-1) != 1:
        raise ValueError(f"{name}: innermost dimension must be contiguous")
    return t.stride(-2)


def _view3(t: torch.Tensor) -> tuple:
    return t.data_ptr(), t.stride(1), t.stride(0)


def device_arch() -> int:
    return lib.sg_device_arch()


def gemm_workspace_bytes(M: int, N: int, split_k: int = 0) -> int:
    return lib.sg_gemm_workspace_bytes(M, N, split_k)


ANATOMY: Optional[torch.Tensor] = None


def new_workspace(nbytes: int, device) -> torch.Tensor:
    return torch.empty((int(nbytes) + 15) & ~15, dtype=torch.uint8, device=device)


DEFAULT_WORKSPACE: Optional[torch.Tensor] = None


class default_workspace:
    def __init__(self, ws: Optional[torch.Tensor]):
        self.ws, self.prev = ws, None

    def __enter__(self):
        global DEFAULT_WORKSPACE
        self.prev, DEFAULT_WORKSPACE = DEFAULT_WORKSPACE, self.ws
        return self.ws

    def __exit__(self, *exc):
        global DEFAULT_WORKSPACE
        DEFAULT_WORKSPACE = self.prev
        return False


def _ws(workspace: Optional[torch.Tensor], d):
    if workspace is None:
        workspace = DEFAULT_WORKSPACE
    if workspace is not None:
        d.workspace, d.workspace_bytes = workspace.data_ptr(), workspace.numel() * workspace.element_size()


def _gemm_desc(a: torch.Tensor, w: torch.Tensor, out: torch.Tensor, *, bias: Optional[torch.Tensor] = None,
               rowbias: Optional[torch.Tensor] = None, rows_per_batch: int = 1, res1: Optional[torch.Tensor] = None,
               res2: Optional[torch.Tensor] = None, epilogue: int = EPI_LINEAR, split_k: int = 0,
               workspace: Optional[torch.Tensor] = None, out2: Optional[torch.Tensor] = None,
               tile: Optional[tuple] = None, use_table: bool = True, stats: Optional[tuple] = None,
               ln: Optional[tuple] = None, ln_out: Optional[torch.Tensor] = None, guard: Optional[torch.Tensor] = None):
    _f16(a, "a"), _f16(w, "w")
    flags = F_OUT_F32 if _act(out, "out") else 0
    M, K = a.shape
    N = w.shape[0]
    if w.shape[1] != K:
        raise ValueError(f"gemm: a is [{M},{K}] but w is {tuple(w.shape)}")
    n_out = N // 2 if epilogue == EPI_GEGLU else N
    if tuple(out.shape) != (M, n_out):
        raise ValueError(f"gemm: out must be [{M},{n_out}], got {tuple(out.shape)}")
    d = GemmDesc()
    d.A, d.lda = a.data_ptr(), _row_stride(a, "a")
    d.W, d.ldw = w.data_ptr(), _row_stride(w, "w")
    d.C, d.ldc = out.data_ptr(), _row_stride(out, "out")
    d.M, d.N, d.K = M, N, K
    d.epilogue = epilogue
    d.bias = _p(bias)
    if bias is not None:
        _f16(bias, "bias")
    if rowbias is not None:
        _f32(rowbias, "rowbias")
        d.rowbias, d.rowbias_ld = rowbias.data_ptr(), _row_stride(rowbias, "rowbias")
    d.rows_per_batch = rows_per_batch
    d.split_k = split_k
    if res1 is not None:
        flags |= F_RES1_F32 if _act(res1, "res1") else 0
        d.res1, d.ldr1 = res1.data_ptr(), _row_stride(res1, "res1")
    if res2 is not None:
        flags |= F_RES2_F32 if _act(res2, "res2") else 0
        d.res2, d.ldr2 = res2.data_ptr(), _row_stride(res2, "res2")
    if out2 is not None:
        _f16(out2, "out2")
        d.C2, d.ldc2 = out2.data_ptr(), _row_stride(out2, "out2")
    d.flags = flags
    _ws(workspace, d)
    if stats is not None:
        _f32(stats[0], "stats")
        d.stats, d.stats_batch_rows = stats[0].data_ptr(), int(stats[1])
    if ln is not None:
        mode, lst, lc, ld_, eps = ln
        _f32(lst, "ln stats"), _f32(lc, "ln c"), _f32(ld_, "ln d")
        tokens = M if mode == 1 else N
        if tuple(lst.shape) != (tokens, (K // 64 + 1) & ~1, 2) or not lst.is_contiguous() or lc.numel() != (N if mode == 1 else M) or ld_.numel() != lc.numel():
            raise ValueError(f"gemm: ln operands do not match mode {mode}, {tokens} tokens, K = {K}")
        d.ln_mode, d.ln_parts, d.ln_eps = int(mode), K // 64, float(eps)
        d.ln_stats, d.ln_c, d.ln_d = lst.data_ptr(), lc.data_ptr(), ld_.data_ptr()
    if ln_out is not None:
        _f32(ln_out, "ln_out")
        if ln_out.numel() != M * ((N // 64 + 1) & ~1) * 2 or not ln_out.is_contiguous():
            raise ValueError(f"gemm: ln_out must hold [{M}, {(N // 64 + 1) & ~1}, 2] floats (N / 64 blocks rounded up to even)")
        d.ln_stats_out = ln_out.data_ptr()
    if guard is not None:
        if guard.dtype != torch.int32 or not guard.is_cuda or guard.numel() < 1:
            raise TypeError("gemm: guard must be a CUDA int32 tensor")
        d.ln_guard = guard.data_ptr()
    sig = f"g:{M}:{N}:{K}:{epilogue}:{flags}:{int(bias is not None)}{int(rowbias is not None)}{int(res1 is not None)}{int(res2 is not None)}{int(out2 is not None)}"
    if ln is not None:
        sig += f":ln{ln[0]}"
    if ln_out is not None:
        sig += ":lo"
    if use_table or tile is not None:
        _apply_tile(d, tile, split_k, sig, M * N)
    if TUNE_SINK is not None and use_table:
        TUNE_SINK.append((sig, dict(kind="gemm", M=M, N=N, K=K, epilogue=epilogue, out_f32=bool(flags & F_OUT_F32), bias=bias is not None,
                                    rowbias=rowbias is not None, rows_per_batch=rows_per_batch, out2=out2 is not None,
                                    res1=None if res1 is None else str(res1.dtype), res2=None if res2 is None else str(res2.dtype),
                                    ln=0 if ln is None else int(ln[0]), ln_out=ln_out is not None)))
    return d, 2.0 * M * N * K, f"M{M} N{N} K{K}{' geglu' if epilogue else ''}"


def _gemm_bytes(d) -> float:
    n_out = d.N // 2 if d.epilogue == EPI_GEGLU else d.N
    osz = 4 if d.flags & F_OUT_F32 else 2
    b = 2.0 * d.M * d.K + 2.0 * d.N * d.K + osz * d.M * n_out
    if d.res1:
        b += (4 if d.flags & F_RES1_F32 else 2) * d.M * n_out
    if d.res2:
        b += (4 if d.flags & F_RES2_F32 else 2) * d.M * n_out
    if d.C2:
        b += 2.0 * d.M * n_out
    return b


def _plan_of(fn, d):
    out = (C.c_int32 * 6)()
    check(fn(C.byref(d), out), "launch plan")
    return list(out)


def _kernel_name(bm: int, bn: int, pipe: int, conv: bool) -> str:
    c = "true" if conv else "false"
    if pipe == 2:
        return f"mma_fat_kernel<{bm // 128}, {bn // 64}, {c}>"
    if pipe >= 16:
        return f"mma_lat_kernel<{bm // 32}, {bn // 32}, {c}, {pipe - 16}>"
    return f"mma_pipe_kernel<{bm // 64}, {bn // 64}, {c}, 3>" if pipe else f"mma_kernel<{bm}, {bn}, {c}>"


def _report_plan(kind: str, d, nbytes: float, family: str, shape: str, second=None):
    if second is not None:
        d1, b1 = second
        out = (C.c_int32 * 14)()
        check(lib.sg_gemm_pair_launch_plan(C.byref(d), C.byref(d1), out), "launch plan")
        (bm, bn, _, wgs, threads, pipe), (bm1, bn1, _, wgs1, threads1, pipe1) = out[1:7], out[7:13]
        if out[0]:
            name = f"mma_lat_pair_kernel<{pipe - 16}>" if pipe >= 16 else f"mma_pipe_pair_kernel<{bm // 64}, {bn // 64}>"
            PLAN_SINK.append((name, out[13] * threads, nbytes + b1, family, shape))
            return
        PLAN_SINK.append((_kernel_name(bm1, bn1, pipe1, False), wgs1 * threads1, b1, family, shape + " [2nd]"))
    else:
        bm, bn, _, wgs, threads, pipe = _plan_of(lib.sg_conv3x3_launch_plan if kind == "conv" else lib.sg_gemm_launch_plan, d)
    PLAN_SINK.append((_kernel_name(bm, bn, pipe, kind == "conv"), wgs * threads, nbytes, family, shape))


def gemm(a: torch.Tensor, w: torch.Tensor, out: torch.Tensor, **kw) -> torch.Tensor:
    d, flops, shape = _gemm_desc(a, w, out, **kw)
    if PLAN_SINK is not None:
        _report_plan("gemm", d, _gemm_bytes(d), "gemm", shape)
    with _timed("gemm", flops, shape):
        if ANATOMY is not None:
            check(lib.sg_debug_gemm_anatomy(C.byref(d), ANATOMY.data_ptr(), ANATOMY.numel() * ANATOMY.element_size(), _stream()),
                  "sg_debug_gemm_anatomy")
        else:
            check(lib.sg_gemm_f16(C.byref(d), _stream()), "sg_gemm_f16")
    return out


def ff_fused_supported(Cc: int) -> bool:
    return lib.sg_ff_fused_pack_bytes(int(Cc)) != 0


def ff_fused(x: torch.Tensor, wpack: torch.Tensor, b2: torch.Tensor, out: torch.Tensor, eps: float = 1e-5, split: bool = False) -> torch.Tensor:
    _f32(x, "x"), _f16(b2, "b2"), _f16(out, "out")
    M, Cc = x.shape
    if tuple(out.shape) != (M, 2 * Cc if split else Cc) or b2.numel() != Cc or wpack.dtype != torch.uint8 or not wpack.is_cuda or not wpack.is_contiguous():
        raise ValueError("ff_fused: out must be [M, C] fp16 ([M, 2C] with split), b2 [C], wpack a contiguous CUDA uint8 tensor")
    d = FfDesc()
    d.x, d.ldx = x.data_ptr(), _row_stride(x, "x")
    d.wpack, d.wpack_bytes = wpack.data_ptr(), wpack.numel()
    d.b2 = b2.data_ptr()
    d.y, d.ldy = out.data_ptr(), _row_stride(out, "out")
    d.M, d.C, d.eps = M, Cc, float(eps)
    d.hidden_split = 2 if split else 0
    with _timed("ff_fused", 24.0 * M * Cc * Cc, f"M{M} C{Cc}" + (" split" if split else "")):
        if ANATOMY is not None:
            check(lib.sg_debug_ff_anatomy(C.byref(d), ANATOMY.data_ptr(), ANATOMY.numel() * ANATOMY.element_size(), _stream()), "sg_debug_ff_anatomy")
        else:
            check(lib.sg_ff_geglu_fused_f16(C.byref(d), _stream()), "sg_ff_geglu_fused_f16")
    return out


def gemm_stats_rows(a: torch.Tensor, w: torch.Tensor, out: torch.Tensor, **kw) -> int:
    d, _, _ = _gemm_desc(a, w, out, **kw)
    rc = lib.sg_gemm_stats_tile_rows(C.byref(d))
    if rc < 0:
        check(rc, "sg_gemm_stats_tile_rows")
    return rc


def gemm_launch_plan(a: torch.Tensor, w: torch.Tensor, out: torch.Tensor, **kw) -> tuple:
    d, _, _ = _gemm_desc(a, w, out, **kw)
    return tuple(_plan_of(lib.sg_gemm_launch_plan, d))


def gemm_pair(first: tuple, second: tuple) -> None:
    (a0, kw0), (a1, kw1) = first, second
    d0, f0, s0 = _gemm_desc(*a0, use_table=False, **kw0)
    d1, f1, s1 = _gemm_desc(*a1, use_table=False, **kw1)
    if PLAN_SINK is not None:
        _report_plan("gemm", d0, _gemm_bytes(d0), "gemm", f"{s0} + {s1}", second=(d1, _gemm_bytes(d1)))
    with _timed("gemm", f0 + f1, f"{s0} + {s1}"):
        check(lib.sg_gemm_pair_f16(C.byref(d0), C.byref(d1), _stream()), "sg_gemm_pair_f16")


def gemm_pair_launch_plan(first: tuple, second: tuple) -> tuple:
    (a0, kw0), (a1, kw1) = first, second
    d0, _, _ = _gemm_desc(*a0, use_table=False, **kw0)
    d1, _, _ = _gemm_desc(*a1, use_table=False, **kw1)
    out = (C.c_int32 * 14)()
    check(lib.sg_gemm_pair_launch_plan(C.byref(d0), C.byref(d1), out), "sg_gemm_pair_launch_plan")
    return tuple(out)


def _conv_desc(x: torch.Tensor, w_krsc: torch.Tensor, out: torch.Tensor, *, stride: int = 1, upsample2x: bool = False,
               bias: Optional[torch.Tensor] = None, rowbias: Optional[torch.Tensor] = None,
               res1: Optional[torch.Tensor] = None, split_k: int = 0, workspace: Optional[torch.Tensor] = None,
               x_padded: bool = False, tile: Optional[tuple] = None, stats: Optional[torch.Tensor] = None,
               defer_reduce: bool = False):
    _f16(x, "x"), _f16(w_krsc, "w")
    flags = F_OUT_F32 if _act(out, "out") else 0
    B, H, W, Cin = x.shape
    if x_padded:
        H, W = H - 2, W - 2
    Cout = w_krsc.shape[0]
    if tuple(w_krsc.shape) != (Cout, 3, 3, Cin) or not w_krsc.is_contiguous():
        raise ValueError(f"conv3x3: w must be contiguous [Cout,3,3,{Cin}], got {tuple(w_krsc.shape)}")
    hin, win = (H * 2, W * 2) if upsample2x else (H, W)
    Ho, Wo = (hin - 1) // stride + 1, (win - 1) // stride + 1
    if tuple(out.shape) != (B, Ho, Wo, Cout):
        raise ValueError(f"conv3x3: out must be {(B, Ho, Wo, Cout)}, got {tuple(out.shape)}")

    def pix_stride(t, name):
        if t.stride(-1) != 1 or t.stride(1) != t.shape[2] * t.stride(2) or t.stride(0) != t.shape[1] * t.stride(1):
            raise ValueError(f"{name}: must be [B,H,W,C] with a single pixel stride")
        return t.stride(2)

    d = ConvDesc()
    d.x, d.ldx = x.data_ptr(), pix_stride(x, "x")
    d.w = w_krsc.data_ptr()
    d.y, d.ldy = out.data_ptr(), pix_stride(out, "out")
    d.B, d.H, d.W, d.Cin, d.Cout = B, H, W, Cin, Cout
    d.stride, d.upsample2x, d.x_padded = stride, int(upsample2x), int(x_padded)
    if bias is not None:
        _f16(bias, "bias")
        d.bias = bias.data_ptr()
    if rowbias is not None:
        _f32(rowbias, "rowbias")
        d.rowbias, d.rowbias_ld = rowbias.data_ptr(), _row_stride(rowbias, "rowbias")
    if res1 is not None:
        flags |= F_RES1_F32 if _act(res1, "res1") else 0
        d.res1, d.ldr1 = res1.data_ptr(), pix_stride(res1, "res1")
    d.flags = flags
    d.split_k = split_k
    _ws(workspace, d)
    if stats is not None:
        _f32(stats, "stats")
        d.stats = stats.data_ptr()
    d.defer_reduce = int(bool(defer_reduce))
    sig = f"c:{B}:{H}:{W}:{Cin}:{Cout}:{stride}:{int(upsample2x)}:{int(x_padded)}:{flags}:{int(bias is not None)}{int(rowbias is not None)}{int(res1 is not None)}"
    _apply_tile(d, tile, split_k, sig, B * Ho * Wo * Cout)
    if TUNE_SINK is not None:
        TUNE_SINK.append((sig, dict(kind="conv", B=B, H=H, W=W, Cin=Cin, Cout=Cout, stride=stride, ups=bool(upsample2x), padded=bool(x_padded),
                                    out_f32=bool(flags & F_OUT_F32), bias=bias is not None, rowbias=rowbias is not None,
                                    res1=None if res1 is None else str(res1.dtype))))
    return d, 2.0 * B * Ho * Wo * Cout * 9 * Cin, f"B{B} {Ho}x{Wo} {Cin}->{Cout} s{stride}{' up' if upsample2x else ''}"


def conv3x3(x: torch.Tensor, w_krsc: torch.Tensor, out: torch.Tensor, **kw) -> torch.Tensor:
    d, flops, shape = _conv_desc(x, w_krsc, out, **kw)
    if PLAN_SINK is not None:
        Ho, Wo = out.shape[1], out.shape[2]
        nb = 2.0 * d.B * d.H * d.W * d.Cin + 2.0 * d.Cout * 9 * d.Cin + (4 if d.flags & F_OUT_F32 else 2) * d.B * Ho * Wo * d.Cout
        if d.res1:
            nb += (4 if d.flags & F_RES1_F32 else 2) * d.B * Ho * Wo * d.Cout
        _report_plan("conv", d, nb, "conv3x3", shape)
    with _timed("conv3x3", flops, shape):
        if ANATOMY is not None:
            check(lib.sg_debug_conv_anatomy(C.byref(d), ANATOMY.data_ptr(), ANATOMY.numel() * ANATOMY.element_size(), _stream()),
                  "sg_debug_conv_anatomy")
        else:
            check(lib.sg_conv3x3_nhwc_f16(C.byref(d), _stream()), "sg_conv3x3_nhwc_f16")
    return out


def conv3x3_planned_splits(x: torch.Tensor, w_krsc: torch.Tensor, out: torch.Tensor, **kw) -> int:
    d, _, _ = _conv_desc(x, w_krsc, out, **kw)
    rc = lib.sg_conv3x3_planned_splits(C.byref(d))
    if rc < 0:
        check(rc, "sg_conv3x3_planned_splits")
    return rc


def conv3x3_launch_plan(x: torch.Tensor, w_krsc: torch.Tensor, out: torch.Tensor, **kw) -> tuple:
    d, _, _ = _conv_desc(x, w_krsc, out, **kw)
    return tuple(_plan_of(lib.sg_conv3x3_launch_plan, d))


def conv3x3_stats_rows(x: torch.Tensor, w_krsc: torch.Tensor, out: torch.Tensor, **kw) -> int:
    d, _, _ = _conv_desc(x, w_krsc, out, **kw)
    rc = lib.sg_conv3x3_stats_tile_rows(C.byref(d))
    if rc < 0:
        check(rc, "sg_conv3x3_stats_tile_rows")
    return rc


def conv_in(x_nchw: torch.Tensor, w_kn: torch.Tensor, bias: torch.Tensor, out: torch.Tensor) -> torch.Tensor:
    _f32(x_nchw, "x"), _f16(w_kn, "w"), _f16(bias, "bias")
    y_f32 = _act(out, "out")
    B, Cin, H, W = x_nchw.shape
    Cout = w_kn.shape[1]
    if not x_nchw.is_contiguous() or tuple(w_kn.shape) != (9 * Cin, Cout) or tuple(out.shape) != (B, H, W, Cout):
        raise ValueError("conv_in: bad shapes")
    check(lib.sg_conv_in_f16(x_nchw.data_ptr(), w_kn.data_ptr(), bias.data_ptr(), out.data_ptr(), out.stride(2), int(y_f32),
                             B, H, W, Cin, Cout, _stream()), "sg_conv_in_f16")
    return out


def conv_out(x: torch.Tensor, w_krsc: torch.Tensor, bias: torch.Tensor, out_nchw: torch.Tensor) -> torch.Tensor:
    _f16(x, "x"), _f16(w_krsc, "w"), _f16(bias, "bias"), _f32(out_nchw, "out")
    B, H, W, Cin = x.shape
    Cout = w_krsc.shape[0]
    if tuple(out_nchw.shape) != (B, Cout, H, W) or not out_nchw.is_contiguous() or not w_krsc.is_contiguous():
        raise ValueError("conv_out: bad shapes")
    check(lib.sg_conv_out_f16(x.data_ptr(), x.stride(2), w_krsc.data_ptr(), bias.data_ptr(), out_nchw.data_ptr(), B, H, W,
                              Cin, Cout, _stream()), "sg_conv_out_f16")
    return out_nchw


def _attn_fwd_desc(q: torch.Tensor, k: torch.Tensor, vt: torch.Tensor, out: torch.Tensor, heads: int, scale: float, nk: Optional[int],
                   short: Optional[tuple] = None):
    for n, t in (("q", q), ("k", k), ("vt", vt), ("out", out)):
        _f16(t, n)
        if t.dim() != 3 or t.stride(-1) != 1:
            raise ValueError(f"attention: {n} must be 3-D with a contiguous last dimension")
    B, Nq, Cq = q.shape
    Bk = k.shape[0]
    Nk = k.shape[1] if nk is None else nk
    D = Cq // heads
    if vt.shape[0] != Bk or vt.shape[1] != Cq or k.shape[2] != Cq or Nk > k.shape[1] or vt.shape[2] < ((Nk + 7) & ~7):
        raise ValueError(f"attention: k {tuple(k.shape)} / vt {tuple(vt.shape)} do not match q {tuple(q.shape)}, nk={Nk}")
    d = AttnDesc()
    d.q, d.ldq, d.bsq = q.data_ptr(), q.stride(1), q.stride(0)
    d.k, d.ldk, d.bsk = k.data_ptr(), k.stride(1), k.stride(0)
    d.vt, d.ldvt, d.bsvt = vt.data_ptr(), vt.stride(1), vt.stride(0)
    d.o, d.ldo, d.bso = out.data_ptr(), out.stride(1), out.stride(0)
    d.B, d.H, d.Nq, d.Nk, d.D = B, heads, Nq, Nk, D
    d.kv_batches = Bk
    d.scale = scale
    keys = [Nk] * B
    if short is not None:
        k2, vt2 = short
        _f16(k2, "k2"), _f16(vt2, "vt2")
        n2, Nk2 = k2.shape[0], k2.shape[1]
        if (k2.dim() != 3 or vt2.dim() != 3 or k2.shape[2] != Cq or tuple(vt2.shape[:2]) != (n2, Cq) or vt2.shape[2] < ((Nk2 + 7) & ~7)
                or k2.stride(-1) != 1 or vt2.stride(-1) != 1 or k2.stride(1) != k.stride(1) or vt2.stride(1) != vt.stride(1)):
            raise ValueError("attention: short rows must be [n, Nk2, H*D] / [n, H*D, Nk2] views with the token / row strides of k / vt")
        d.k2, d.bsk2, d.vt2, d.bsvt2 = k2.data_ptr(), k2.stride(0), vt2.data_ptr(), vt2.stride(0)
        d.Nk2, d.kv2_batches = Nk2, n2
        d.kv_batches = Bk = Bk + n2
        keys = [Nk2 if (b if b < Bk else b - (B - Bk)) < n2 else Nk for b in range(B)]
    if d.kv_batches > B:
        raise ValueError(f"attention: {d.kv_batches} K/V rows for {B} query batches")
    shape = f"B{B} H{heads} Nq{Nq} Nk{Nk}" + (f" ({d.kv2_batches}x Nk{d.Nk2})" if short is not None else "")
    return d, 4.0 * heads * Nq * D * float(sum(keys)), shape


def attention(q: torch.Tensor, k: torch.Tensor, vt: torch.Tensor, out: torch.Tensor, heads: int, scale: float,
              nk: Optional[int] = None, short: Optional[tuple] = None) -> torch.Tensor:
    d, flops, shape = _attn_fwd_desc(q, k, vt, out, heads, scale, nk, short)
    with _timed(f"attention_d{d.D}", flops, shape):
        check(lib.sg_attn_fwd_f16(C.byref(d), _stream()), "sg_attn_fwd_f16")
    return out


def attention_pair(a: tuple, b: tuple, heads: int, scale: float) -> None:
    da, fa, sa = _attn_fwd_desc(*a[:4], heads, scale, *a[4:])
    db, fb, sb = _attn_fwd_desc(*b[:4], heads, scale, *b[4:])
    with _timed(f"attention_d{da.D}", fa + fb, f"{sa} + {sb}"):
        check(lib.sg_attn_fwd_pair_f16(C.byref(da), C.byref(db), _stream()), "sg_attn_fwd_pair_f16")


ATTN_FAMILIES = ("d40_loop", "shared_body", "general", "lean", "ksplit", "lse", "f8")


def _attn_plan_tuple(pl) -> tuple:
    return (ATTN_FAMILIES[pl.family], pl.waves, pl.stages, pl.workgroups)


def attention_plan(q: torch.Tensor, k: torch.Tensor, vt: torch.Tensor, out: torch.Tensor, heads: int, scale: float,
                   nk: Optional[int] = None, short: Optional[tuple] = None, lse: bool = False) -> tuple:
    d, _, _ = _attn_fwd_desc(q, k, vt, out, heads, scale, nk, short)
    pl = AttnPlan()
    check(lib.sg_attn_fwd_plan(C.byref(d), int(lse), C.byref(pl)), "sg_attn_fwd_plan")
    return _attn_plan_tuple(pl)


def attention_pair_plan(a: tuple, b: tuple, heads: int, scale: float) -> tuple:
    da, _, _ = _attn_fwd_desc(*a[:4], heads, scale, *a[4:])
    db, _, _ = _attn_fwd_desc(*b[:4], heads, scale, *b[4:])
    pr = AttnPairPlan()
    check(lib.sg_attn_fwd_pair_plan(C.byref(da), C.byref(db), C.byref(pr)), "sg_attn_fwd_pair_plan")
    return (bool(pr.shared), pr.first, _attn_plan_tuple(pr.p0), _attn_plan_tuple(pr.p1), pr.workgroups)


def attention_f8_plan(B: int, heads: int, Nq: int) -> tuple:
    pl = AttnPlan()
    check(lib.sg_attn_fwd_f8_plan(B, heads, Nq, C.byref(pl)), "sg_attn_fwd_f8_plan")
    return _attn_plan_tuple(pl)


def attention_f8_bytes(B: int, heads: int, N: int, transposed: bool) -> int:
    return lib.sg_attn_f8_bytes(B, heads, N, int(transposed))


def attention_f8(q: torch.Tensor, k: torch.Tensor, vt: torch.Tensor, out: torch.Tensor, heads: int, scale: float,
                 scratch: torch.Tensor, nk: Optional[int] = None) -> torch.Tensor:
    for n, t in (("q", q), ("k", k), ("vt", vt), ("out", out)):
        _f16(t, n)
        if t.dim() != 3 or t.stride(-1) != 1:
            raise ValueError(f"attention_f8: {n} must be 3-D with a contiguous last dimension")
    B, Nq, Cq = q.shape
    Bk = k.shape[0]
    Nk = k.shape[1] if nk is None else nk
    if Cq != heads * 40:
        raise ValueError("attention_f8: head dim must be 40")
    if vt.shape[0] != Bk or vt.shape[1] != Cq or k.shape[2] != Cq or Nk > k.shape[1] or vt.shape[2] < ((Nk + 7) & ~7):
        raise ValueError(f"attention_f8: k {tuple(k.shape)} / vt {tuple(vt.shape)} do not match q {tuple(q.shape)}, nk={Nk}")
    nq8, nk8, nv8 = attention_f8_bytes(B, heads, Nq, False), attention_f8_bytes(Bk, heads, Nk, False), attention_f8_bytes(Bk, heads, Nk, True)
    if scratch.dtype != torch.uint8 or not scratch.is_cuda or scratch.numel() < nq8 + nk8 + nv8 + 512:
        raise ValueError(f"attention_f8: scratch must be a CUDA uint8 tensor of at least {nq8 + nk8 + nv8 + 512} bytes")
    base = (scratch.data_ptr() + 255) & ~255
    q8, k8, v8 = base, base + ((nq8 + 255) & ~255), base + ((nq8 + 255) & ~255) + ((nk8 + 255) & ~255)
    if v8 + nv8 > scratch.data_ptr() + scratch.numel():
        raise ValueError("attention_f8: scratch too small after alignment")
    st = _stream()
# ... 970 lines not shown
```

storygen_amd/repack.py:

```python
from __future__ import annotations

from typing import Optional, Tuple

import torch


def conv3x3_krsc(w: torch.Tensor) -> torch.Tensor:
    return w.permute(0, 2, 3, 1).contiguous()


def conv_in_kn(w: torch.Tensor) -> torch.Tensor:
    cout, cin = w.shape[:2]
    return w.permute(2, 3, 1, 0).reshape(9 * cin, cout).contiguous()


def conv1x1_nk(w: torch.Tensor) -> torch.Tensor:
    return w.reshape(w.shape[0], w.shape[1]).contiguous()


def interleave_geglu(w: torch.Tensor, b: Optional[torch.Tensor]) -> Tuple[torch.Tensor, Optional[torch.Tensor]]:
    inner = w.shape[0] // 2
    assert inner % 32 == 0
    wi = torch.stack([w[:inner].reshape(inner // 32, 32, -1), w[inner:].reshape(inner // 32, 32, -1)], dim=1)
    wi = wi.reshape(2 * inner, -1).contiguous()
    bi = None
    if b is not None:
        bi = torch.stack([b[:inner].reshape(inner // 32, 32), b[inner:].reshape(inner // 32, 32)], dim=1).reshape(-1).contiguous()
    return wi, bi


def fold_layernorm(w: torch.Tensor, b: Optional[torch.Tensor], gamma: torch.Tensor, beta: torch.Tensor
                   ) -> Tuple[torch.Tensor, torch.Tensor, torch.Tensor]:
    w32, g32, be32 = w.float(), gamma.float(), beta.float()
    wf = (w32 * g32[None]).to(torch.float16)
    c = wf.float().sum(dim=1)
    d = w32 @ be32 + (0.0 if b is None else b.float())
    return wf, c, d


FF_CHUNK_HIDDEN = 32


def _pi32(i: int) -> int:
    return (i & ~12) | ((i & 4) << 1) | ((i & 8) >> 1)


def ff_fused_layout(C: int) -> dict:
    assert C % 64 == 0 and (C * 64) % 1024 == 0, "the fused feed-forward kernel is built for C = 320"
    w1_img = (C // 64) * 64 * 128
    w1_part = w1_img + 64 * 32
    return dict(C=C, chunks=4 * C // FF_CHUNK_HIDDEN, w1_img=w1_img, w1_part=w1_part, w2_part=C * 64, chunk=w1_part + C * 64)


def ff_fused_pack(w1f: torch.Tensor, d1: torch.Tensor, w2: torch.Tensor) -> torch.Tensor:
    C = w2.shape[0]
    L = ff_fused_layout(C)
    assert tuple(w1f.shape) == (8 * C, C) and tuple(w2.shape) == (C, 4 * C) and d1.numel() == 8 * C
    dev = w1f.device
    nch, ks = L["chunks"], C // 64
    w1f = w1f.to(torch.float16).contiguous()
    w2 = (w2.to(torch.float16) * 0.5).contiguous()
    pi = torch.tensor([t * 32 + _pi32(i) for t in range(2) for i in range(32)], device=dev)
    a = w1f.view(nch, 64, ks, 8, 8)[:, pi]
    r = torch.arange(64, device=dev)
    logical = torch.arange(8, device=dev)[None, :] ^ ((r[:, None] >> 1) & 7)
    a = a.permute(0, 2, 1, 3, 4)
    a = torch.gather(a, 3, logical[None, None, :, :, None].expand(nch, ks, 64, 8, 8))
    w1_img = a.reshape(nch, L["w1_img"] // 2)
    b = w2.view(C, nch, 4, 8).permute(1, 0, 2, 3)
    n = torch.arange(C, device=dev)
    logical2 = torch.arange(4, device=dev)[None, :] ^ ((n[:, None] >> 2) & 3)
    b = torch.gather(b, 2, logical2[None, :, :, None].expand(nch, C, 4, 8))
    w2_img = b.reshape(nch, C * 32)
    out = torch.zeros(nch, L["chunk"], dtype=torch.uint8, device=dev)
    out[:, : L["w1_img"]] = w1_img.contiguous().view(torch.uint8).view(nch, -1)
    dd = d1.to(device=dev, dtype=torch.float32).contiguous().view(nch, 64)[:, pi]
    hi = dd.to(torch.float16)
    if not bool(torch.isfinite(hi).all()):
        raise ValueError(f"ff_fused_pack: d1 = W1 beta + b1 must be finite in fp16 (|d1| < 65520), got max |d1| = {float(dd.abs().max()):.6g}")
    lo =(dd - hi.float()).to(torch.float16)
    dimg = torch.zeros(nch, 64, 16, dtype=torch.float16, device=dev)
    dimg[:, :, 0], dimg[:, :, 1] = hi, lo
    out[:, L["w1_img"]: L["w1_part"]] = dimg.view(torch.uint8).view(nch, -1)
    out[:, L["w1_part"]:] = w2_img.contiguous().view(torch.uint8).view(nch, -1)
    return out.reshape(-1)
```

Measured before the change: 78.67 denoising steps/s.

## Compute nearest-upsample 3x3 conv as four 2x2 phase convolutions

Adds a phase-decomposed form of the upsample-then-3x3 convolution. The 3x3 taps are pre-summed into four 2x2 kernels, one per output parity, so each output pixel does 4 taps on the low-resolution input instead of 9 taps on the upsampled one. A new mma_phase_kernel handles this: it selects weights by phase, gathers directly from the padded low-res input, and scatters output rows to their interleaved positions. The engine uses it for up-block samplers with at least 1024 output rows and falls back when no suitable tile exists. In exchange, the pre-summed weights are rounded to fp16 in a different order, which changes numerics slightly, and the output stores are scattered.

```diff
diff --git a/storygen_amd/csrc/gemm_conv.hip b/storygen_amd/csrc/gemm_conv.hip
--- a/storygen_amd/csrc/gemm_conv.hip
+++ b/storygen_amd/csrc/gemm_conv.hip
@@ -34,6 +34,7 @@
     f16* C2; long ldc2;
     int M, N, K, KT;
     int H, Wd, Ho, Wo, cpt , stride, ups, padded;
+    int phase;
     int mode, flags;
     const f16* bias;
     const float* rowbias; long rowbias_ld; int rows_per_batch;
@@ -167,7 +168,16 @@
     if (p.ln_guard && !(fabsf(sum * (1.f / 64.f)) + sqrtf(m2) < 65504.f)) atomicOr(p.ln_guard, SG_LN_GUARD_RANGE);
 }
 
-template <int WGM, int WGN, int WT = 2, int WTM = WT>
+template <bool PH>
+__device__ __forceinline__ int epi_out_row(const MmaParams& p, int gm) {
+    if constexpr (!PH) return gm;
+    const int hw = p.Ho * p.Wo;
+    const int sp = (int)fd_div((unsigned)gm, p.fd_hw), q = gm - sp * hw;
+    const int i = (int)fd_div((unsigned)q, p.fd_wo);
+    return (sp >> 2) * 4 * hw + ((sp >> 1) & 1) * 2 * p.Wo + (sp & 1) + 2 * q + 2 * i * p.Wo;
+}
+
+template <int WGM, int WGN, int WT = 2, int WTM = WT, bool PH = false>
 __device__ __forceinline__ void epi_finish(const MmaParams& p, char* smem, f32x16 (&acc)[WTM][WT], f32x4 (&pre)[WT == 2 ? 16 : 4], u32x2& pbias,
                                            int m0, int n0, int z, int wave, int wm0, int wn, int lane) {
     constexpr int BN = 32 * WT * WGN, NW = WGM * WGN, NT = 64 * NW, NH = WT == 2 ? WTM / 2 : 1, NQ = WT == 2 ? 16 : 4;
@@ -267,7 +277,7 @@
         for (int k = 0; k < NQ; ++k) {
             const int row = 4 * k + r0, gm = rowq + 4 * k;
             const float4 v = *reinterpret_cast<const float4*>(stg + row * EPI_PITCH + 4 * lc);
-            if (gm < p.M && col_ok) st_stream(wsz + (size_t)gm * p.N, f32x4{v.x, v.y, v.z, v.w});
+            if (gm < p.M && col_ok) st_stream(wsz + (size_t)epi_out_row<PH>(p, gm) * p.N, f32x4{v.x, v.y, v.z, v.w});
         }
         continue;
     }
@@ -388,7 +398,7 @@
     for (int k = 0; k < NQ; ++k) {
         const int gm = rowq + 4 * k;
         if (gm < p.M && col_ok) {
-            store_out4(p, gm, colq, v[k]);
+            store_out4(p, epi_out_row<PH>(p, gm), colq, v[k]);
 #pragma unroll
             for (int e = 0; e < 4; ++e) { cs[e] += v[k][e]; cq2[e] = fmaf(v[k][e], v[k][e], cq2[e]); }
         }
@@ -647,8 +657,10 @@
     if constexpr (Y > 0) slab_tail<Y - 1, S>(slab, nt);
 }
 
-template <int WGM, int WGN, bool CONV, bool PROF = false, int S = 3, int WT = 2, int WTMX = WT>
+template <int WGM, int WGN, bool CONV, bool PROF = false, int S = 3, int WT = 2, int WTMX = WT, bool PH = false>
 __device__ __forceinline__ void mma_pipe_body(const MmaParams& p, char* smem) {
+    static_assert(!PH || (CONV && !PROF), "the phase form is a convolution");
+    constexpr int TAPS = PH ? 2 : 3;
     unsigned long long pf_acc[9] = {0, 0, 0, 0, 0, 0, 0, 0, 0};
     unsigned long long pf_t = 0, pf_entry = 0;
     auto stamp = [&](int slot) __attribute__((always_inline)) {
@@ -690,7 +702,9 @@
         w_off[i] = 2u * (unsigned)((long)min(n0 + row, p.N - 1) * p.ldw + lc * 8);
     }
     auto w_koff = [&](int kt) __attribute__((always_inline)) -> long {
-        if constexpr (CONV) {
+        if constexpr (PH) {
+            return (long)(kt & 3) * p.cpt * BK + (long)(kt >> 2) * BK;
+        } else if constexpr (CONV) {
             const int cc = (kt * 7282) >> 16, tap = kt - 9 * cc;
             return (long)tap * p.cpt * BK + (long)cc * BK;
         } else {
@@ -698,9 +712,10 @@
         }
     };
     const LdsRef lds = lds_ref(smem);
+    const f16* const Wb = PH ? p.W + (long)(fd_div((unsigned)m0, p.fd_hw) & 3u) * p.N * p.ldw : p.W;
     auto issue_w = [&](long koff, int stage, int sel = -1) __attribute__((always_inline)) {
         const LdsRef sB = lds + (stage * STAGE + A_BYTES + wave * 1024);
-        const f16* Wt = p.W + koff;
+        const f16* Wt = Wb + koff;
 #pragma unroll
         for (int i = 0; i < B_IT; ++i)
             if (sel < 0 || ((A_IT + i) & 3) == sel) glds16(Wt, w_off[i], sB + i * ISTR);
@@ -719,7 +734,11 @@
             const int b = (int)fd_div((unsigned)gm, p.fd_hw), rem = gm - b * hw;
             const int oy = (int)fd_div((unsigned)rem, p.fd_wo), ox = rem - oy * p.Wo;
             const long img = (long)b * (p.H + 2) * wp;
-            if (!p.ups) {
+            if constexpr (PH) {
+                const long simg = (long)(b >> 2) * (p.H + 2) * wp;
+                a_off[i] = 2u * (unsigned)((simg + (long)(oy + ((b >> 1) & 1)) * wp + ox + (b & 1)) * p.lda + lc * 8);
+                a_par[i] = 0;
+            } else if (!p.ups) {
                 a_off[i] = 2u * (unsigned)((img + (long)(oy * p.stride) * wp + ox * p.stride) * p.lda + lc * 8);
                 a_par[i] = 0;
             } else {
@@ -737,7 +756,11 @@
         ABase r;
         r.ky = r.kx = 0;
         r.wk = w_koff(kt);
-        if constexpr (CONV) {
+        if constexpr (PH) {
+            const int cc = kt >> 2, ky = (kt >> 1) & 1, kx = kt & 1;
+            r.ky = ky; r.kx = kx;
+            r.At = p.A + ((long)(ky * wp + kx) * p.lda + cc * BK);
+        } else if constexpr (CONV) {
             const int cc = (kt * 7282) >> 16, tap = kt - 9 * cc;
             const int ky = (tap * 11) >> 5, kx = tap - ky * 3;
             r.ky = ky; r.kx = kx;
@@ -750,7 +773,7 @@
     auto a_emit = [&](const ABase& ab, int stage, int sel) __attribute__((always_inline)) {
         const LdsRef sA = lds + (stage * STAGE + wave * 1024);
         if constexpr (CONV) {
-            if (!p.ups) {
+            if (PH || !p.ups) {
 #pragma unroll
                 for (int i = 0; i < A_IT; ++i)
                     if (sel < 0 || (i & 3) == sel) glds16(ab.At, a_off[i], sA + i * ISTR);
@@ -778,18 +801,18 @@
         if constexpr (CONV) { it_ky = b0.ky; it_kx = b0.kx; }
     }
     const long it_px = CONV && !p.ups ? (long)p.lda : 0;
-    const long it_dy = CONV && !p.ups ? (long)(wp - 3) * p.lda : 0;
-    const long it_dc = CONV ? (p.ups ? 0 : -3L * wp * p.lda) + BK : 0;
-    const long it_wtap = CONV ? (long)p.cpt * BK : BK, it_wdc = CONV ? BK - 9L * p.cpt * BK : 0;
+    const long it_dy = CONV && !p.ups ? (long)(wp - TAPS) * p.lda : 0;
+    const long it_dc = CONV ? (p.ups ? 0 : -(long)TAPS * wp * p.lda) + BK : 0;
+    const long it_wtap = CONV ? (long)p.cpt * BK : BK, it_wdc = CONV ? BK - (long)(TAPS * TAPS) * p.cpt * BK : 0;
     auto a_next = [&]() __attribute__((always_inline)) {
         ABase r;
         r.At = p.A + it_off; r.ky = it_ky; r.kx = it_kx; r.wk = it_wk;
         it_wk += it_wtap;
         if constexpr (CONV) {
             it_off += it_px;
-            if (++it_kx == 3) {
+            if (++it_kx == TAPS) {
                 it_kx = 0; it_off += it_dy;
-                if (++it_ky == 3) { it_ky = 0; it_off += it_dc; it_wk += it_wdc; }
+                if (++it_ky == TAPS) { it_ky = 0; it_off += it_dc; it_wk += it_wdc; }
             }
         } else {
             it_off += BK;
@@ -904,7 +927,7 @@
     for (int it = 0; it < nsteady; it += S) slab_seq<0, S, YS>(slab, it, nsteady);
     slab_tail<TAIL - 1, S>(slab, nt);
     if (nt <= 0) prefetch();
-    epi_finish<WGM, WGN, WT, WTM>(p, smem, acc, pre_f, pre_bias, m0, n0, z, wave, wm, wn, lane);
+    epi_finish<WGM, WGN, WT, WTM, PH>(p, smem, acc, pre_f, pre_bias, m0, n0, z, wave, wm, wn, lane);
     if constexpr (PROF) {
         asm volatile("s_waitcnt vmcnt(0)" ::: "memory");
         stamp(8);
@@ -921,6 +944,12 @@
 __global__ __launch_bounds__(64 * WGM * WGN) void mma_pipe_kernel(const MmaParams p) {
     __shared__ __attribute__((aligned(16))) char smem[pipe_smem_bytes<WGM, WGN, S>()];
     mma_pipe_body<WGM, WGN, CONV, false, S>(p, smem);
+}
+
+template <int WGM, int WGN>
+__global__ __launch_bounds__(64 * WGM * WGN) void mma_phase_kernel(const MmaParams p) {
+    __shared__ __attribute__((aligned(16))) char smem[pipe_smem_bytes<WGM, WGN, 3>()];
+    mma_pipe_body<WGM, WGN, true, false, 3, 2, 2, true>(p, smem);
 }
 
 template <int WGM, int WGN, bool CONV>
@@ -1196,7 +1225,9 @@
 };
 
 
-Plan choose_plan(int M, int N, int KT, int force_split, int max_ws_split, bool pipe, int hint_bm, int hint_bn) {
+bool phase_tile_ok(int bm, int bn) { return (bm == 256 && bn == 128) || (bm == 128 && bn == 128) || (bm == 64 && (bn == 128 || bn == 64)); }
+
+Plan choose_plan(int M, int N, int KT, int force_split, int max_ws_split, bool pipe, int hint_bm, int hint_bn, int row_div = 0) {
     static const int cand_pipe[6][2] = {{256, 128}, {128, 128}, {256, 64}, {128, 64}, {64, 128}, {64, 64}};
     static const int cand_gen[1][2] = {{128, 128}};
     static const int split_opts[] = {1, 2, 3, 4, 5, 6, 8, 10, 12, 16};
@@ -1211,6 +1242,7 @@
         const int bm = pipe ? cand_pipe[ci][0] : cand_gen[ci][0], bn = pipe ? cand_pipe[ci][1] : cand_gen[ci][1];
         if (pipe && o.tile_m && (bm != o.tile_m || bn != o.tile_n)) continue;
         if (pipe && !o.tile_m && hint_bm && (bm != hint_bm || bn != hint_bn)) continue;
+        if (row_div > 0 && (row_div % bm != 0 || !phase_tile_ok(bm, bn))) continue;
         const long tiles = (long)sg_cdiv(M, bm) * sg_cdiv(N, bn);
         const double waves_per_block = pipe ? (bm / 64) * (bn / 64) : 4.0;
         const double mfma_per_slab = pipe ? 512.0 : 512.0 * (bm / 64.0) * (bn / 64.0) / 4.0;
@@ -1230,6 +1262,7 @@
             if (forced) break;
         }
     }
+    if (row_div > 0 && best_cost == 1e300) best.bm = best.bn = 0;
     return best;
 }
 
@@ -1289,6 +1322,10 @@
 template <bool CONV>
 Plan choose_family(const MmaParams& p, const PlanRequest& rq, TileHint hint, bool pipe, int max_ws_split) {
     const SgOptions& o = sg_options();
+    if (CONV && p.phase) {
+        if (!pipe || o.tile_m || p.prof || asks_fat(hint) || asks_lat(hint)) return Plan{0, 0, 1, FAM_PIPE};
+        return choose_plan(p.M, p.N, p.KT, rq.force_split, max_ws_split, true, hint.bm, hint.bn, p.Ho * p.Wo);
+    }
     const bool fat_ok = pipe && !p.prof && !o.tile_m && rq.force_split <= 1 && (p.mode == SG_EPI_LINEAR || p.mode == SG_EPI_GEGLU);
     if (asks_fat(hint)) {
         if (fat_ok) return Plan{hint.bm, hint.bn, 1, FAM_FAT};
@@ -1306,9 +1343,11 @@
 
 template <bool CONV>
 int choose_group_m(const MmaParams& p, int splits) {
-    const double a_bytes = CONV ? 2.0 * p.M * (p.K / 9) * (p.stride == 1 && !p.ups ? 1.0 : (p.ups ? 0.25 : 4.0)) : 2.0 * p.M * p.K;
+    const double a_bytes = CONV ? (p.phase ? 2.0 * p.M * (p.K / 4) * 0.25
+                                           : 2.0 * p.M * (p.K / 9) * (p.stride == 1 && !p.ups ? 1.0 : (p.ups ? 0.25 : 4.0))) : 2.0 * p.M * p.K;
     const double w_bytes = 2.0 * p.N * p.K;
     const double a_panel = a_bytes / p.tiles_m, w_panel = w_bytes / p.tiles_n;
+    const int tiles_per_phase = CONV && p.phase ? (int)((long)p.tiles_m * p.Ho * p.Wo / p.M) : 0;
     const int wave_tiles = splits >= 32 ? 1 : 32 / splits;
     int best = 1;
     double best_bytes = 1e300;
@@ -1325,7 +1364,8 @@
             if (rows > p.tiles_m) rows = p.tiles_m;
             cols = p.tiles_n;
         }
-        const double bytes = rows * a_panel + cols * w_panel;
+        const int panels = tiles_per_phase > 0 ? (rows + tiles_per_phase - 1) / tiles_per_phase : 1;
+        const double bytes = rows * a_panel + cols * w_panel * panels;
         if (bytes <= best_bytes) { best_bytes = bytes; best = gm; }
     }
     return sg_options().no_nmajor ? 1 : best;
@@ -1356,6 +1396,10 @@
     const size_t per_split = (size_t)p.M * p.N * 4;
     const int max_ws_split = rq.ws ? (int)(rq.ws_bytes / per_split > 64 ? 64 : rq.ws_bytes / per_split) : 1;
     pl = choose_family<CONV>(p, rq, apply_big_m(rq.hint, p.M, pipe), pipe, max_ws_split);
+    if (CONV && p.phase && (pl.bm == 0 || (p.Ho * p.Wo) % pl.bm != 0 || !phase_tile_ok(pl.bm, pl.bn)))
+        return sg_set_error(SG_EUNSUP, "%s: no phase-form launch for this descriptor (a row tile of the LDS-DMA kernels must divide the "
+                            "%d pixels of the %dx%d input, and be one mma_phase_kernel is built for): use upsample2x = 1", rq.name,
+                            p.Ho * p.Wo, p.H, p.Wd);
     if (pl.splits > 1 && (rq.ws == nullptr || rq.ws_bytes < per_split * pl.splits))
         return sg_set_error(SG_EINVAL, "%s: split_k=%d needs %zu workspace bytes, got %zu", rq.name, pl.splits, per_split * pl.splits,
                             rq.ws_bytes);
@@ -1411,7 +1455,12 @@
     if (p.defer && pl.splits <= 1)
         return sg_set_error(SG_EINVAL, "%s: defer_reduce needs a split-K launch (query sg_conv3x3_planned_splits first)", name);
     const dim3 grid(pl.grid), block(pl.threads);
-    if (pl.family == FAM_FAT) {
+    if (CONV && p.phase) {
+        if (pl.bm == 256) hipLaunchKernelGGL((mma_phase_kernel<4, 2>), grid, block, 0, st, p);
+        else if (pl.bm == 128) hipLaunchKernelGGL((mma_phase_kernel<2, 2>), grid, block, 0, st, p);
+        else if (pl.bn == 128) hipLaunchKernelGGL((mma_phase_kernel<1, 2>), grid, block, 0, st, p);
+        else hipLaunchKernelGGL((mma_phase_kernel<1, 1>), grid, block, 0, st, p);
+    } else if (pl.family == FAM_FAT) {
         if (pl.bm == 512) hipLaunchKernelGGL((mma_fat_kernel<4, 2, CONV>), grid, block, 0, st, p);
         else hipLaunchKernelGGL((mma_fat_kernel<2, 4, CONV>), grid, block, 0, st, p);
     } else if (pl.lat()) {
@@ -1540,7 +1589,11 @@
     SG_REQUIRE(d->Cin % 64 == 0, "%s: Cin (%d) must be a multiple of 64", who, d->Cin);
     SG_REQUIRE(d->Cout % 8 == 0, "%s: Cout (%d) must be a multiple of 8", who, d->Cout);
     SG_REQUIRE(d->stride == 1 || d->stride == 2, "%s: stride must be 1 or 2", who);
-    SG_REQUIRE(d->upsample2x == 0 || (d->upsample2x == 1 && d->stride == 1), "%s: upsample2x needs stride 1", who);
+    SG_REQUIRE(d->upsample2x >= 0 && d->upsample2x <= 2, "%s: upsample2x must be 0, 1 or 2", who);
+    SG_REQUIRE(d->upsample2x == 0 || d->stride == 1, "%s: upsample2x needs stride 1", who);
+    const bool ph = d->upsample2x == 2;
+    SG_REQUIRE(!ph || d->x_padded == 1, "%s: upsample2x = 2 (phase form) needs the zero-bordered input (x_padded = 1)", who);
+    SG_REQUIRE(!ph || (!d->res1 && !d->rowbias), "%s: upsample2x = 2 (phase form) takes bias only (no res1, no rowbias)", who);
     SG_REQUIRE(d->x_padded == 0 || d->x_padded == 1, "%s: x_padded must be 0 or 1", who);
     SG_REQUIRE(d->ldx % 8 == 0 && d->ldx >= d->Cin, "%s: bad ldx", who);
     SG_REQUIRE(sg_aligned16(d->x) && sg_aligned16(d->w), "%s: x/w must be 16-byte aligned", who);
@@ -1555,29 +1608,31 @@
         const int bord = d->x_padded ? 2 : 0;
         const long long rows = (long long)d->B * (d->H + bord), pixels = rows <= lim ? rows * (d->W + bord) : lim + 1;
         const long long x_span = pixels <= lim ? (pixels - 1) * (long long)d->ldx + d->Cin : lim + 1;
-        const long long w_span = (long long)d->Cout * 9 * d->Cin;
+        const long long w_span = (long long)d->Cout * (ph ? 16 : 9) * d->Cin;
         SG_REQUIRE(x_span <= lim,
                    "%s: input x spans %s%lld elements ((pixels - 1) * ldx + Cin%s); the bound is 2^31 elements (4 GiB: 32-bit LDS-DMA byte offsets)",
                    who, pixels <= lim ? "" : "more than ", x_span, d->x_padded ? ", zero border included" : "");
         SG_REQUIRE(w_span <= lim,
-                   "%s: weights w span %lld elements (Cout * 9 * Cin); the bound is 2^31 elements (4 GiB: 32-bit LDS-DMA byte offsets)", who, w_span);
+                   "%s: weights w span %lld elements (Cout * 9 * Cin; 16 in the phase form); the bound is 2^31 elements (4 GiB: 32-bit LDS-DMA byte offsets)", who, w_span);
     }
     SG_REQUIRE(9 * (d->Cin / 64) < 3000, "%s: Cin (%d) too large for the slab decode (kt / 9 by multiply-shift, kt < 3000)", who, d->Cin);
-    const int hin = d->H << d->upsample2x, win = d->W << d->upsample2x;
+    const int up = d->upsample2x ? 1 : 0;
+    const int hin = d->H << up, win = d->W << up;
     const int Ho = (hin + 2 - 3) / d->stride + 1, Wo = (win + 2 - 3) / d->stride + 1;
     p = MmaParams{};
     p.A = reinterpret_cast<const f16*>(d->x); p.lda = d->ldx;
-    p.W = reinterpret_cast<const f16*>(d->w); p.ldw = 9L * d->Cin;
+    p.W = reinterpret_cast<const f16*>(d->w); p.ldw = (ph ? 4L : 9L) * d->Cin;
     p.C = d->y; p.ldc = d->ldy;
-    p.M = d->B * Ho * Wo; p.N = d->Cout; p.K = 9 * d->Cin;
+    p.M = d->B * Ho * Wo; p.N = d->Cout; p.K = (ph ? 4 : 9) * d->Cin;
     p.H = d->H; p.Wd = d->W; p.Ho = Ho; p.Wo = Wo; p.cpt = d->Cin / 64; p.stride = d->stride; p.ups = d->upsample2x;
+    if (ph) { p.phase = 1; p.ups = 0; p.Ho = d->H; p.Wo = d->W; }
     p.padded = d->x_padded;
     p.mode = SG_EPI_LINEAR; p.flags = d->flags;
     p.bias = reinterpret_cast<const f16*>(d->bias);
     p.rowbias = d->rowbias; p.rowbias_ld = d->rowbias_ld; p.rows_per_batch = Ho * Wo;
     p.res1 = d->res1; p.ldr1 = d->ldr1;
     SG_REQUIRE(!d->stats || sg_aligned16(d->stats), "%s: stats alignment", who);
-    p.stats = d->stats; p.stats_batch_rows = Ho * Wo;
+    p.stats = d->stats; p.stats_batch_rows = ph ? d->H * d->W : Ho * Wo;
     SG_REQUIRE(d->defer_reduce == 0 || (d->defer_reduce == 1 && !d->stats), "%s: defer_reduce is 0 or 1 and excludes stats", who);
     p.defer = d->defer_reduce;
     return check_tile_hint(who, d->tile_m, d->tile_n, d->tile_waves);
diff --git a/storygen_amd/engine.py b/storygen_amd/engine.py
--- a/storygen_amd/engine.py
+++ b/storygen_amd/engine.py
@@ -7,7 +7,7 @@
 
 from . import ops
 from .arch import BlockSpec, ResnetSpec, UNetArch, XfSpec, feature_shapes
-from .repack import conv1x1_nk, conv3x3_krsc, conv_in_kn, ff_fused_pack, fold_layernorm, interleave_geglu
+from .repack import conv1x1_nk, conv3x3_krsc, conv_in_kn, ff_fused_pack, fold_layernorm, interleave_geglu, upsample_phase_pack
 
 F16 = torch.float16
 GN_EPILOGUE_STATS = True
@@ -20,6 +20,8 @@
 FF_FUSED = True
 FF_SPLIT_MAX_TOKENS = 16384
 FF_PROJ_MERGE = True
+UPSAMPLE_PHASES = True
+UPSAMPLE_PHASES_MIN_ROWS = 1024
 LN_EPS = 1e-5
 
 
@@ -128,6 +130,8 @@
             if blk.sampler_prefix:
                 self.samplers[blk.sampler_prefix] = (conv3x3_krsc(g(f"{blk.sampler_prefix}.weight")),
                                                      g(f"{blk.sampler_prefix}.bias"))
+        self.sampler_phases = {blk.sampler_prefix: upsample_phase_pack(g(f"{blk.sampler_prefix}.weight"))
+                               for blk in arch.up if blk.sampler_prefix}
         self.gn_out = (g("conv_norm_out.weight"), g("conv_norm_out.bias"))
         self.w_conv_out = conv3x3_krsc(g("conv_out.weight"))
         self.b_conv_out = g("conv_out.bias")
@@ -695,6 +699,11 @@
         pbuf = self.padded[(lvl, h.shape[1])]
         ops.pad_cast(self._img(h, lvl), pbuf)
         kw = dict(stride=2 if down else 1, upsample2x=not down, bias=b, workspace=self.ws_split, x_padded=True)
+        if not down and UPSAMPLE_PHASES and self.dev.type == "cuda" and out.shape[0] >= UPSAMPLE_PHASES_MIN_ROWS:
+            kwp = dict(kw, upsample2x=2)
+            wp = self.sampler_phases[prefix]
+            if ops.conv3x3_phases_fit(pbuf, wp, self._img(out, out_lvl), **kwp):
+                w, kw, prefix = wp, kwp, prefix + "#phases"
         return self._produce(prefix, out_lvl, out.shape[1], lambda s: ops.conv3x3(pbuf, w, self._img(out, out_lvl), stats=s, **kw),
                              lambda buf: ops.conv3x3_stats_rows(pbuf, w, self._img(out, out_lvl), stats=buf, **kw))
 
diff --git a/storygen_amd/ops.py b/storygen_amd/ops.py
--- a/storygen_amd/ops.py
+++ b/storygen_amd/ops.py
@@ -13,6 +13,7 @@
 EPI_LINEAR = 0
 EPI_GEGLU = 1
 F_OUT_F32, F_RES1_F32, F_RES2_F32 = 1, 2, 4
+EUNSUP = -2
 
 TILE_TABLE = {}
 TUNE_SINK = None
@@ -262,6 +263,9 @@
         PLAN_SINK.append((_kernel_name(bm1, bn1, pipe1, False), wgs1 * threads1, b1, family, shape + " [2nd]"))
     else:
         bm, bn, _, wgs, threads, pipe = _plan_of(lib.sg_conv3x3_launch_plan if kind == "conv" else lib.sg_gemm_launch_plan, d)
+        if kind == "conv" and d.upsample2x == 2:
+            PLAN_SINK.append((f"mma_phase_kernel<{bm // 64}, {bn // 64}>", wgs * threads, nbytes, family, shape))
+            return
     PLAN_SINK.append((_kernel_name(bm, bn, pipe, kind == "conv"), wgs * threads, nbytes, family, shape))
 
 
@@ -344,9 +348,10 @@
     B, H, W, Cin = x.shape
     if x_padded:
         H, W = H - 2, W - 2
-    Cout = w_krsc.shape[0]
-    if tuple(w_krsc.shape) != (Cout, 3, 3, Cin) or not w_krsc.is_contiguous():
-        raise ValueError(f"conv3x3: w must be contiguous [Cout,3,3,{Cin}], got {tuple(w_krsc.shape)}")
+    phases = upsample2x is not True and int(upsample2x) == 2
+    Cout = w_krsc.shape[1 if phases else 0]
+    if tuple(w_krsc.shape) != ((4, Cout, 2, 2, Cin) if phases else (Cout, 3, 3, Cin)) or not w_krsc.is_contiguous():
+        raise ValueError(f"conv3x3: w must be contiguous {'[4,Cout,2,2,' if phases else '[Cout,3,3,'}{Cin}], got {tuple(w_krsc.shape)}")
     hin, win = (H * 2, W * 2) if upsample2x else (H, W)
     Ho, Wo = (hin - 1) // stride + 1, (win - 1) // stride + 1
     if tuple(out.shape) != (B, Ho, Wo, Cout):
@@ -385,14 +390,14 @@
         TUNE_SINK.append((sig, dict(kind="conv", B=B, H=H, W=W, Cin=Cin, Cout=Cout, stride=stride, ups=bool(upsample2x), padded=bool(x_padded),
                                     out_f32=bool(flags & F_OUT_F32), bias=bias is not None, rowbias=rowbias is not None,
                                     res1=None if res1 is None else str(res1.dtype))))
-    return d, 2.0 * B * Ho * Wo * Cout * 9 * Cin, f"B{B} {Ho}x{Wo} {Cin}->{Cout} s{stride}{' up' if upsample2x else ''}"
+    return d, 2.0 * B * Ho * Wo * Cout * (4 if phases else 9) * Cin, f"B{B} {Ho}x{Wo} {Cin}->{Cout} s{stride}{(' up4' if phases else ' up') if upsample2x else ''}"
 
 
 def conv3x3(x: torch.Tensor, w_krsc: torch.Tensor, out: torch.Tensor, **kw) -> torch.Tensor:
     d, flops, shape = _conv_desc(x, w_krsc, out, **kw)
     if PLAN_SINK is not None:
         Ho, Wo = out.shape[1], out.shape[2]
-        nb = 2.0 * d.B * d.H * d.W * d.Cin + 2.0 * d.Cout * 9 * d.Cin + (4 if d.flags & F_OUT_F32 else 2) * d.B * Ho * Wo * d.Cout
+        nb = 2.0 * d.B * d.H * d.W * d.Cin + 2.0 * d.Cout * (16 if d.upsample2x == 2 else 9) * d.Cin + (4 if d.flags & F_OUT_F32 else 2) * d.B * Ho * Wo * d.Cout
         if d.res1:
             nb += (4 if d.flags & F_RES1_F32 else 2) * d.B * Ho * Wo * d.Cout
         _report_plan("conv", d, nb, "conv3x3", shape)
@@ -403,6 +408,21 @@
         else:
             check(lib.sg_conv3x3_nhwc_f16(C.byref(d), _stream()), "sg_conv3x3_nhwc_f16")
     return out
+
+
+def conv3x3_phases_fit(x: torch.Tensor, w_phases: torch.Tensor, out: torch.Tensor, **kw) -> bool:
+    d, _, _ = _conv_desc(x, w_phases, out, **{**kw, "upsample2x": 2})
+    rc = lib.sg_conv3x3_launch_plan(C.byref(d), (C.c_int32 * 6)())
+    if rc == EUNSUP:
+        return False
+    check(rc, "sg_conv3x3_launch_plan")
+    return True
+
+
+def conv3x3_upsample(x: torch.Tensor, w_krsc: torch.Tensor, w_phases: torch.Tensor, out: torch.Tensor, **kw) -> torch.Tensor:
+    if conv3x3_phases_fit(x, w_phases, out, **kw):
+        return conv3x3(x, w_phases, out, upsample2x=2, **kw)
+    return conv3x3(x, w_krsc, out, upsample2x=True, **kw)
 
 
 def conv3x3_planned_splits(x: torch.Tensor, w_krsc: torch.Tensor, out: torch.Tensor, **kw) -> int:
diff --git a/storygen_amd/repack.py b/storygen_amd/repack.py
--- a/storygen_amd/repack.py
+++ b/storygen_amd/repack.py
@@ -7,6 +7,27 @@
 
 def conv3x3_krsc(w: torch.Tensor) -> torch.Tensor:
     return w.permute(0, 2, 3, 1).contiguous()
+
+
+UPSAMPLE_PHASE_TAPS = (((0,), (1, 2)), ((0, 1), (2,)))
+
+
+def upsample_phase_sums(w: torch.Tensor) -> torch.Tensor:
+    cout, cin = w.shape[:2]
+    out = w.new_zeros(4, cout, 2, 2, cin)
+    for a in range(2):
+        for b in range(2):
+            for ty in range(2):
+                for tx in range(2):
+                    acc = out[2 * a + b, :, ty, tx]
+                    for ky in UPSAMPLE_PHASE_TAPS[a][ty]:
+                        for kx in UPSAMPLE_PHASE_TAPS[b][tx]:
+                            acc += w[:, :, ky, kx]
+    return out
+
+
+def upsample_phase_pack(w: torch.Tensor) -> torch.Tensor:
+    return upsample_phase_sums(w.float()).to(torch.float16).contiguous()
 
 
 def conv_in_kn(w: torch.Tensor) -> torch.Tensor:
```

Result: faster. 80.12 denoising steps/s (median of 6 runs) (+1.8%).
